# maxim2266/csvplus

Measured on AMD Instinct MI355X. Metric: joined rows/sec (IndexOn build + chained Join, 1e8-row 3-col orders), higher is better.
Workload: dtype u32; 1 GPU; BASELINE configs[3]: orders(1e8 x {cust_id,prod_id,qty}).Join(UniqueIndexOn customers.id 1e7).Join(UniqueIndexOn products.prod_id 1e5); rows=100000000, customers=10000000, products=100000, rows_this_rank=100000000, exchange=none (1 GPU), output=sorted positions

## Files before the change

### csvplus_amd/csrc/capi.hip

```cpp
#include <algorithm>
#include <map>
#include <mutex>
#include <new>

#include "cph_internal.hpp"
#include "codec_device.hpp"

namespace cph {

constexpr size_t kGuardBytes = 256;
constexpr uint8_t kGuardByte = 0xA5;

Status DevicePool::alloc(size_t bytes, void** out) {
    std::lock_guard<std::recursive_mutex> lk(mu_);
    const size_t want = (bytes + (guard ? kGuardBytes : 0) + 255) & ~(size_t)255;
    int best = -1;
    for (int i = 0; i < (int)free_.size(); i++) {
        if (free_[i].cap >= want && free_[i].cap <= want * 2 + (1u << 20)) {
            if (best < 0 || free_[i].cap < free_[best].cap) best = i;
        }
    }
    Block b;
    bool from_slab = false;
    for (size_t i = 0; i < slab_free_.size(); i++)
// ... 349 lines not shown
}

Status validate_cols(const cph_strcol* cols, int32_t ncols) {
    if (!cols || ncols <= 0) return {CPH_ERR_INVALID, "no key columns"};
    if (ncols > kMaxKeyCols) return {CPH_ERR_INVALID, "too many key columns"};
    for (int c = 0; c < ncols; c++) {
        if (cols[c].fixed_width == 0 && cols[c].offset_bits != 32 && cols[c].offset_bits != 64)
            return {CPH_ERR_INVALID, "offset_bits must be 32 or 64"};
        if (cols[c].mem != CPH_MEM_HOST && cols[c].mem != CPH_MEM_DEVICE) return {CPH_ERR_INVALID, "bad mem"};
        if (cols[c].nrows != cols[0].nrows) return {CPH_ERR_INVALID, "key columns differ in row count"};
        if (cols[c].nrows && !cols[c].offsets && cols[c].fixed_width == 0) return {CPH_ERR_INVALID, "offsets is NULL"};
        if (cols[c].nrows && cols[c].fixed_width && !cols[c].data) return {CPH_ERR_INVALID, "data is NULL"};
    }
    if (cols[0].nrows > 0xFFFFFFFFull) return {CPH_ERR_TOO_MANY_ROWS, "more than 2^32-1 rows"};
    return {};
}

Status stage_cols(cph_ctx* ctx, const cph_strcol* cols, int32_t ncols, std::vector<DevBuf>* storage,
                         DevCol* out) {
    for (int c = 0; c < ncols; c++) {
        DevCol d;
        d.nrows = cols[c].nrows;
        d.offset_bits = cols[c].offset_bits;
        d.fixed_width = cols[c].fixed_width;
        if (cols[c].mem == CPH_MEM_DEVICE || cols[c].nrows == 0) {
            d.data = cols[c].data;
            d.offsets = cols[c].offsets;
            if (!d.data) {
                if (!ctx->safe_words) {
                    CPH_TRY(ctx->safe_words.alloc(&ctx->pool, 64));
                    CPH_HIP_TRY(hipMemsetAsync(ctx->safe_words.get(), 0, 64, ctx->stream));
                }
                d.data = ctx->safe_words.as<uint8_t>();
            }
        } else if (cols[c].fixed_width) {
            const size_t bytes = (size_t)cols[c].nrows * cols[c].fixed_width;
            DevBuf bd;
            CPH_TRY(bd.alloc(&ctx->pool, bytes + 8));
            CPH_HIP_TRY(hipMemcpyAsync(bd.get(), cols[c].data, bytes, hipMemcpyHostToDevice, ctx->stream));
            d.data = bd.as<uint8_t>();
            d.offsets = nullptr;
            storage->push_back(std::move(bd));
        } else {
            const size_t obytes = (size_t)(cols[c].nrows + 1) * (size_t)(cols[c].offset_bits / 8);
            const uint64_t first = cols[c].offset_bits == 32 ? ((const uint32_t*)cols[c].offsets)[0]
                                                             : ((const uint64_t*)cols[c].offsets)[0];
            const uint64_t last = cols[c].offset_bits == 32 ? ((const uint32_t*)cols[c].offsets)[cols[c].nrows]
                                                            : ((const uint64_t*)cols[c].offsets)[cols[c].nrows];
            if (last < first) return {CPH_ERR_INVALID, "offsets are not monotonic"};
            DevBuf bo, bd;
            CPH_TRY(bo.alloc(&ctx->pool, obytes));
            CPH_TRY(bd.alloc(&ctx->pool, (size_t)last + 8));
            CPH_HIP_TRY(hipMemcpyAsync(bo.get(), cols[c].offsets, obytes, hipMemcpyHostToDevice, ctx->stream));
            if (last) CPH_HIP_TRY(hipMemcpyAsync(bd.get(), cols[c].data, (size_t)last, hipMemcpyHostToDevice, ctx->stream));
            d.data = bd.as<uint8_t>();
            d.offsets = bo.get();
            storage->push_back(std::move(bo));
            storage->push_back(std::move(bd));
        }
        out[c] = d;
    }
    return {};
}

Status check_row_sources(const cph_strcol* cols, const cph_rowsel* sel, int32_t ncols, uint64_t first_row, uint64_t nrows, bool exact) {
    for (int c = 0; c < ncols; c++) {
        CPH_TRY(validate_cols(cols + c, 1));
        const bool ident = !sel || !sel[c].ids;
        if (ident && nrows && (exact ? cols[c].nrows != nrows : cols[c].nrows < first_row + nrows))
            return {CPH_ERR_INVALID, exact ? "a column without row ids must have nrows rows"
                                           : "a column without row ids must have at least first_row + nrows rows"};
        if (!ident && sel[c].bits != 32 && sel[c].bits != 64) return {CPH_ERR_INVALID, "row id bits must be 32 or 64"};
    }
    return {};
}

Status stage_row_sources(cph_ctx* ctx, const cph_strcol* cols, const cph_rowsel* sel, const int* order, int32_t ncols, uint64_t first_row,
                         uint64_t n, std::vector<DevBuf>* staged, ColsArg* arg, ColIds* ids) {
    for (int k = 0; k < ncols; k++) {
        const int c = order ? order[k] : k;
        CPH_TRY(stage_cols(ctx, cols + c, 1, staged, &arg->c[k]));
        if (!sel || !sel[c].ids || !n) continue;
        RowIds& r = ids->ids[k];
        r.bits = sel[c].bits;
        r.base = sel[c].base;
        r.ptr = sel[c].ids;
        if (cols[c].mem == CPH_MEM_HOST) {
            const size_t w = (size_t)(sel[c].bits / 8);
            staged->emplace_back();
            CPH_TRY(staged->back().alloc(&ctx->pool, n * w));
            CPH_HIP_TRY(hipMemcpyAsync(staged->back().get(), static_cast<const uint8_t*>(sel[c].ids) + first_row * w, n * w,
                                       hipMemcpyHostToDevice, ctx->stream));
            r.ptr = reinterpret_cast<const void*>((uintptr_t)staged->back().get() - (uintptr_t)(first_row * w));
        }
    }
    return {};
}

Status deliver(cph_ctx* ctx, ResultOwner* owner, const ResultPart* parts, int nparts, int32_t out_mem) {
    auto show = [](const ResultPart& p, const void* v) { memcpy(p.pub, &v, sizeof v); };
    auto padded = [](const ResultPart& p) { return (p.bytes + 15) & ~(size_t)15; };
    uint8_t* h = nullptr;
    if (out_mem == CPH_MEM_HOST) {
        size_t need = 16;
        for (int i = 0; i < nparts; i++) need += padded(parts[i]);
        CPH_HIP_TRY(hipHostMalloc(&owner->h_block, need, hipHostMallocDefault));
        h = static_cast<uint8_t*>(owner->h_block);
    }
    for (int i = 0; i < nparts; i++) {
        const ResultPart& p = parts[i];
        const void* src = p.src ? p.src : p.dev->get();
        if (h && p.bytes) CPH_HIP_TRY(hipMemcpyAsync(h, src, p.bytes, hipMemcpyDeviceToHost, ctx->stream));
        show(p, h ? h : src);
        if (h) h += padded(p);
    }
    CPH_HIP_TRY(hipStreamSynchronize(ctx->stream));
    if (h)
        for (int i = 0; i < nparts; i++) parts[i].dev->reset();
    return {};
}

static int32_t fail(cph_ctx* ctx, const Status& s) {
    if (ctx) ctx->err = s.msg;
    return s.code;
}

static Status enter(cph_ctx* ctx) {
    if (!ctx) return {CPH_ERR_INVALID, "ctx is NULL"};
    CPH_HIP_TRY(hipSetDevice(ctx->device));
    return {};
}

struct BuildJob {
    cph_index* ix = nullptr;
    int32_t nkeycols = 0;
    std::vector<DevBuf> staged;
    DevCol dcols[kMaxKeyCols];
    DevBuf stats_dev;
    const void* sample_host = nullptr;
    size_t scratch_off = 0;
    GroupSpec spec;
    bool small = false;
    SmallBufs sbufs;
    bool presplit = false;
    bool sampled = false;
    bool no_sample = false;
    bool unique = false;
    bool no_direct = false;
    bool side = false;
    bool spec_split = false;
    bool exact_split = false;
    bool no_split = false;
    uint32_t* miss = nullptr;
    uint32_t* cs_over = nullptr;
    DevBuf cs_codes;
};

static Status build_phase1(cph_ctx* ctx, const cph_strcol* keycols, int32_t nkeycols, BuildJob* job) {
    CPH_TRY(validate_cols(keycols, nkeycols));
    cph_index* ix = job->ix;
    ix->ctx = ctx;
    ix->nrows = keycols[0].nrows;
    ix->table_rows = ix->nrows;
    ix->nkeycols = nkeycols;
    job->nkeycols = nkeycols;
    CPH_TRY(stage_cols(ctx, keycols, nkeycols, &job->staged, job->dcols));
    job->small = small_build_applies(ctx, job->dcols, nkeycols, ix->nrows);
    if (!job->small && !job->no_split && nkeycols == 1 && !job->dcols[0].fixed_width && ix->nrows >= (1ull << 22)) {
        CPH_TRY(codec_try_split(ctx, job->dcols, 1, ix->nrows, nullptr, &ix->codec, !job->exact_split, &job->spec_split));
        job->presplit = ix->codec.has_split();
    }
    job->sampled = !job->small && !job->presplit && !job->no_sample && codec_sample_applies(ctx, job->dcols, nkeycols, ix->nrows);
    if (job->sampled) CPH_TRY(codec_sample_launch(ctx, job->dcols[0], ix->nrows, &job->sample_host));
    else if (!job->small && !job->presplit) CPH_TRY(codec_stats_launch(ctx, job->dcols, nkeycols, &job->stats_dev));
    return {};
}

static Status build_phase2(cph_ctx* ctx, BuildJob* job, const void* stats_host);
static Status job_arm_miss(cph_ctx* ctx, BuildJob* job) {
    job->miss = host_word(ctx);
    return job->miss ? Status{} : Status{CPH_ERR_HIP, "no pinned host memory for the report words of a build"};
}
static Status build_encode_sort(cph_ctx* ctx, BuildJob* job);

static size_t job_readback_bytes(const BuildJob& j) {
    return j.small ? sizeof(SmallResult) : (j.presplit || j.sampled) ? 0 : sizeof(ColStats) * (size_t)j.nkeycols;
}

static void build_run(cph_ctx* ctx, std::vector<BuildJob>& jobs, std::vector<Status>& status) {
    const size_t nj = jobs.size();
    auto fail_all = [&](const Status& s) {
        for (size_t i = 0; i < nj; i++)
            if (status[i].ok()) status[i] = s;
    };
    size_t total = 0;
    bool any_general = false;
    for (size_t i = 0; i < nj; i++) {
        jobs[i].scratch_off = total;
        total += job_readback_bytes(jobs[i]);
        total = (total + 63) & ~(size_t)63;
        if (status[i].ok() && !jobs[i].small) any_general = true;
    }
    Status s = ensure_pinned_scratch(ctx, total > 64 ? total : 64);
    if (!s.ok()) return fail_all(s);
    uint8_t* h = static_cast<uint8_t*>(ctx->pinned_scratch);
    for (size_t i = 0; i < nj; i++) {
        if (!status[i].ok()) continue;
        if (jobs[i].small) {
            SideStream on_side(ctx, jobs[i].side);
            status[i] = small_build_launch(ctx, jobs[i].dcols, jobs[i].nkeycols, jobs[i].ix->nrows, &jobs[i].sbufs,
                                           reinterpret_cast<SmallResult*>(h + jobs[i].scratch_off));
            continue;
        }
        if (jobs[i].presplit || jobs[i].sampled) continue;
        hipError_t e = hipMemcpyAsync(h + jobs[i].scratch_off, jobs[i].stats_dev.get(), job_readback_bytes(jobs[i]),
                                      hipMemcpyDeviceToHost, jobs[i].side ? ctx->side_stream : ctx->stream);
        if (e != hipSuccess) status[i] = {CPH_ERR_HIP, std::string("statistics read-back: ") + hipGetErrorString(e)};
    }
    bool any_side = false;
    for (size_t i = 0; i < nj; i++) any_side = any_side || jobs[i].side;
    auto sync_streams = [&]() {
        return hipStreamSynchronize(ctx->stream) == hipSuccess && (!any_side || hipStreamSynchronize(ctx->side_stream) == hipSuccess);
    };
    if (!sync_streams()) return fail_all({CPH_ERR_HIP, "hipStreamSynchronize failed"});
    ctx->pool.flush_deferred();
    std::vector<std::vector<uint8_t>> stats_host(nj);
    std::vector<size_t> retry;
    for (size_t i = 0; i < nj; i++) {
        if (!status[i].ok()) continue;
        if (jobs[i].small) {
            const SmallResult res = *reinterpret_cast<const SmallResult*>(h + jobs[i].scratch_off);
            bool not_small = false;
            status[i] = small_build_finish(ctx, jobs[i].ix, jobs[i].nkeycols, &jobs[i].sbufs, &res, &not_small);
            jobs[i].sbufs = SmallBufs{};
            if (status[i].ok() && not_small) retry.push_back(i);
            else if (status[i].ok()) index_plan_table(jobs[i].ix);
            continue;
        }
        if (jobs[i].sampled) {
            const uint8_t* sh = static_cast<const uint8_t*>(jobs[i].sample_host);
            stats_host[i].assign(sh, sh + codec_sample_bytes());
        } else if (!jobs[i].presplit) {
            stats_host[i].assign(h + jobs[i].scratch_off, h + jobs[i].scratch_off + job_readback_bytes(jobs[i]));
        }
    }
    for (size_t i = 0; i < nj; i++)
        if (status[i].ok() && !jobs[i].small) {
            SideStream on_side(ctx, jobs[i].side);
            status[i] = build_phase2(ctx, &jobs[i], stats_host[i].data());
        }
    std::vector<size_t> resplit;
    std::vector<size_t> resort;
    if (any_general) {
        s = ensure_pinned_scratch(ctx, 2 * sizeof(uint32_t) * nj + 64);
        if (!s.ok()) return fail_all(s);
        uint32_t* fd = static_cast<uint32_t*>(ctx->pinned_scratch);
        uint32_t* sm = fd + nj;
        for (size_t i = 0; i < nj; i++) {
            if (!status[i].ok() || jobs[i].small) continue;
            hipStream_t js = jobs[i].side ? ctx->side_stream : ctx->stream;
            fd[i] = 0xFFFFFFFFu;
            sm[i] = 0;
            if (!jobs[i].ix->first_dup_dev) continue;
            hipError_t e = hipMemcpyAsync(&fd[i], jobs[i].ix->first_dup_dev.get(), sizeof(uint32_t), hipMemcpyDeviceToHost, js);
            if (e != hipSuccess) status[i] = {CPH_ERR_HIP, std::string("first-duplicate read-back: ") + hipGetErrorString(e)};
        }
        if (!sync_streams()) return fail_all({CPH_ERR_HIP, "hipStreamSynchronize failed"});
        ctx->pool.flush_deferred();
        for (size_t i = 0; i < nj; i++) {
            if (!status[i].ok() || jobs[i].small) continue;
            cph_index* ix = jobs[i].ix;
            if (jobs[i].miss) sm[i] = *(volatile uint32_t*)jobs[i].miss;
            if (sm[i]) { jobs[i].cs_codes.reset(); jobs[i].cs_over = nullptr; resplit.push_back(i); continue; }
            if (jobs[i].cs_over && *(volatile uint32_t*)jobs[i].cs_over) { resort.push_back(i); continue; }
            jobs[i].cs_codes.reset();
            ix->first_dup = fd[i] != 0xFFFFFFFFu ? (uint64_t)fd[i] : UINT64_MAX;
            ix->first_dup_dev.reset();
            index_plan_table(ix);
        }
    }
    for (size_t i : resort) {
        BuildJob& j = jobs[i];
        cph_index* ix = j.ix;
        const uint64_t n = ix->nrows;
        uint32_t* over = j.cs_over;
        j.cs_over = nullptr;
        ix->sorted_codes.reset(); ix->perm.reset(); ix->first_dup_dev.reset();
        DevBuf kb, va, vb;
        Status r = kb.alloc(&ctx->pool, n * sizeof(uint32_t));
        if (r.ok()) r = va.alloc(&ctx->pool, n * sizeof(uint32_t));
        bool sorted_now = false;
        {
            CountedSortPlan first;
            int wb = counted_sort_plan(ctx, n, ix->codec.word_states[0], &first) ? (int)first.wbits : 0;
            for (int attempt = 0; attempt < 2 && r.ok() && !sorted_now && wb > 0; attempt++) {
                wb -= 2;
                CountedSortPlan csp;
                if (!counted_sort_plan(ctx, n, ix->codec.word_states[0], &csp, wb) || (int)csp.wbits != wb) break;
                r = ix->first_dup_dev.alloc(&ctx->pool, sizeof(uint32_t));
                if (r.ok()) r = counted_sort(ctx, csp, j.cs_codes.as<uint32_t>(), n, ix->codec.word_states[0], va.as<uint32_t>(), kb.as<uint32_t>(),
                                             ix->first_dup_dev.as<uint32_t>(), over);
                if (r.ok() && hipStreamSynchronize(ctx->stream) != hipSuccess) r = {CPH_ERR_HIP, "hipStreamSynchronize failed"};
                if (r.ok() && *(volatile uint32_t*)over == 0) {
                    ix->sorted_codes = std::move(kb);
                    ix->perm = std::move(va);
                    ix->sort_passes = 0;
                    r = index_first_dup_read(ctx, ix);
                    sorted_now = true;
                } else {
                    ix->first_dup_dev.reset();
                }
            }
        }
        if (sorted_now) {
            j.cs_codes.reset();
            if (r.ok()) index_plan_table(ix);
            status[i] = r;
            continue;
        }
        if (r.ok()) r = vb.alloc(&ctx->pool, n * sizeof(uint32_t));
        uint32_t *kout = nullptr, *vout = nullptr;
        int passes = 0;
        if (r.ok()) r = radix_sort_pairs<uint32_t>(ctx, j.cs_codes.as<uint32_t>(), kb.as<uint32_t>(), va.as<uint32_t>(), vb.as<uint32_t>(), true, n,
                                                   ix->codec.word_bits[0], &kout, &vout, &passes);
        if (r.ok()) {
            ix->sorted_codes = std::move(kout == j.cs_codes.as<uint32_t>() ? j.cs_codes : kb);
            ix->perm = std::move(vout == va.as<uint32_t>() ? va : vb);
            ix->sort_passes = passes;
            r = index_first_dup_launch(ctx, ix);
        }
        if (r.ok()) r = index_first_dup_read(ctx, ix);
        j.cs_codes.reset();
        if (r.ok()) index_plan_table(ix);
        status[i] = r;
    }
    for (size_t i : resplit) {
        std::vector<BuildJob> one;
        one.push_back(std::move(jobs[i]));
        std::vector<Status> st1(1);
        BuildJob& j = one[0];
        j.side = false;
        const bool again_exact = j.spec_split;
        j.spec_split = false;
        j.exact_split = again_exact;
        j.no_split = !again_exact;
        j.no_sample = true;
        j.sampled = false;
        j.no_direct = true;
        j.presplit = false;
        j.miss = nullptr;
        cph_index* ix = j.ix;
        ix->codec = CodecHost{};
        ix->codec_dev.reset(); ix->sorted_codes.reset(); ix->perm.reset(); ix->first_dup_dev.reset(); ix->ranktab.reset();
        if (again_exact) {
            ctx->n_split_respec++;
            st1[0] = codec_try_split(ctx, j.dcols, 1, ix->nrows, nullptr, &ix->codec, false, nullptr);
            j.presplit = st1[0].ok() && ix->codec.has_split();
        }
        if (st1[0].ok() && !j.presplit) st1[0] = codec_stats_launch(ctx, j.dcols, j.nkeycols, &j.stats_dev);
        if (st1[0].ok()) build_run(ctx, one, st1);
        status[i] = st1[0];
        jobs[i] = std::move(one[0]);
    }
    for (size_t i : retry) {
        std::vector<BuildJob> one;
        one.push_back(std::move(jobs[i]));
        std::vector<Status> st1(1);
        one[0].small = false;
        one[0].side = false;
        st1[0] = codec_stats_launch(ctx, one[0].dcols, one[0].nkeycols, &one[0].stats_dev);
        if (st1[0].ok()) build_run(ctx, one, st1);
        status[i] = st1[0];
        jobs[i] = std::move(one[0]);
    }
}

static Status sort_words_lsd(cph_ctx* ctx, cph_index* ix, const uint64_t* all, int nw, const int* bits, uint64_t n, DevBuf& va,
                             DevBuf& vb) {
    DevBuf ka, kb;
    CPH_TRY(ka.alloc(&ctx->pool, n * sizeof(uint64_t)));
    CPH_TRY(kb.alloc(&ctx->pool, n * sizeof(uint64_t)));
    uint32_t* vcur = va.as<uint32_t>();
    uint32_t* vother = vb.as<uint32_t>();
    uint64_t* kout = ka.as<uint64_t>();
    bool first = true;
    int passes = 0;
    ix->sort_passes = 0;
    for (int w = nw - 1; w >= 0; w--) {
        const uint64_t* word = all + (uint64_t)w * n;
        if (first) {
            if (n) CPH_HIP_TRY(hipMemcpyAsync(ka.get(), word, n * sizeof(uint64_t), hipMemcpyDeviceToDevice, ctx->stream));
        } else {
            CPH_TRY(gather_u64(ctx, word, vcur, ka.as<uint64_t>(), n));
        }
        uint32_t* vout;
        CPH_TRY(radix_sort_pairs<uint64_t>(ctx, ka.as<uint64_t>(), kb.as<uint64_t>(), vcur, vother, first, n, bits[w], &kout, &vout,
                                           &passes));
        ix->sort_passes += passes;
        if (vout != vcur) { vother = vcur; vcur = vout; }
        first = false;
    }
    DevBuf sorted;
    CPH_TRY(sorted.alloc(&ctx->pool, (size_t)nw * n * sizeof(uint64_t)));
    if (n) CPH_HIP_TRY(hipMemcpyAsync(sorted.get(), kout, n * sizeof(uint64_t), hipMemcpyDeviceToDevice, ctx->stream));
    for (int w = 1; w < nw; w++) CPH_TRY(gather_u64(ctx, all + (uint64_t)w * n, vcur, sorted.as<uint64_t>() + (uint64_t)w * n, n));
    ix->sorted_codes = std::move(sorted);
    ix->perm = std::move(vcur == va.as<uint32_t>() ? va : vb);
    return {};
}

static DevCol window_col(const DevCol* cols, const cph_key_window& w, int s) {
    DevCol v = cols[w.seg_col[s]];
    v.skip = w.seg_skip[s];
    v.take = w.seg_take[s];
    return v;
}

static Status build_multi_window(cph_ctx* ctx, BuildJob* job, const std::vector<ColStats>& raw) {
    cph_index* ix = job->ix;
    const uint64_t n = ix->nrows;
    std::vector<cph_key_window>& W = ix->windows;
    W.clear();
    W.emplace_back();
    uint32_t room = kMaxKeyBytes;
    for (int c = 0; c < job->nkeycols; c++) {
        uint32_t left = raw[(size_t)c].maxlen, skip = 0;
        do {
            if (room == 0 || W.back().nseg == kMaxKeyCols) {
                W.emplace_back();
                room = kMaxKeyBytes;
            }
            cph_key_window& w = W.back();
            const uint32_t t = left < room ? left : room;
            w.seg_col[w.nseg] = c;
            w.seg_skip[w.nseg] = skip;
            w.seg_take[w.nseg] = t == left ? 0xFFFFFFFFu : t;
            w.nseg++;
            skip += t;
            left -= t;
            room -= t;
        } while (left > 0);
    }
    int total_words = 0;
    for (auto& w : W) {
        DevCol v[kMaxKeyCols];
        for (int s = 0; s < w.nseg; s++) v[s] = window_col(job->dcols, w, s);
        std::vector<ColStats> st;
        CPH_TRY(codec_collect_stats(ctx, v, w.nseg, &st));
        CPH_TRY(codec_build(st, &w.codec));
        w.codec.key32 = false;
        CPH_TRY(codec_upload(ctx, w.codec, &w.codec_dev));
        w.word_base = total_words;
        total_words += w.codec.nwords;
    }
    ix->codec = W[0].codec;
    DevBuf all, va, vb;
    CPH_TRY(all.alloc(&ctx->pool, (size_t)total_words * n * sizeof(uint64_t)));
    CPH_TRY(va.alloc(&ctx->pool, n * sizeof(uint32_t)));
    CPH_TRY(vb.alloc(&ctx->pool, n * sizeof(uint32_t)));
    std::vector<int> bits((size_t)total_words);
    for (auto& w : W) {
        DevCol v[kMaxKeyCols];
        for (int s = 0; s < w.nseg; s++) v[s] = window_col(job->dcols, w, s);
        CPH_TRY(codec_encode_build(ctx, w.codec, w.codec_dev, v, n, all.as<uint64_t>() + (uint64_t)w.word_base * n));
        for (int k = 0; k < w.codec.nwords; k++) bits[(size_t)(w.word_base + k)] = w.codec.word_bits[k];
    }
    CPH_TRY(sort_words_lsd(ctx, ix, all.as<uint64_t>(), total_words, bits.data(), n, va, vb));
    return index_first_dup_launch(ctx, ix);
}

static Status build_phase2(cph_ctx* ctx, BuildJob* job, const void* stats_host) {
    cph_index* ix = job->ix;
    const uint64_t n = ix->nrows;
    const int32_t nkeycols = job->nkeycols;
    const DevCol* dcols = job->dcols;
    if (job->presplit) {
        CPH_TRY(job_arm_miss(ctx, job));
        CPH_TRY(codec_upload(ctx, ix->codec, &ix->codec_dev));
        return build_encode_sort(ctx, job);
    }
    std::vector<ColStats> stats;
    if (job->sampled) {
        codec_sample_finish(dcols[0], stats_host, &stats);
        CPH_TRY(codec_build(stats, &ix->codec));
        if (codec_sample_checked(ix->codec, dcols)) {
            CPH_TRY(job_arm_miss(ctx, job));
            CPH_TRY(codec_upload(ctx, ix->codec, &ix->codec_dev));
            return build_encode_sort(ctx, job);
        }
        job->sampled = false;
        ix->codec = CodecHost{};
        CPH_TRY(codec_collect_stats(ctx, dcols, nkeycols, &stats));
    } else {
        codec_stats_finish(dcols, nkeycols, stats_host, &stats);
    }
    uint64_t positions = 0;
    for (const auto& s : stats) positions += s.maxlen;
    if (positions > (uint64_t)kMaxKeyBytes) return build_multi_window(ctx, job, stats);
    CPH_TRY(codec_build(stats, &ix->codec));
    if (!job->no_split) CPH_TRY(codec_try_split(ctx, dcols, nkeycols, n, &stats, &ix->codec));
    if (ix->codec.has_split()) {
        CPH_TRY(job_arm_miss(ctx, job));
    } else {
        CPH_TRY(codec_try_groups(ctx, dcols, nkeycols, n, &ix->codec, &job->spec));
    }
    CPH_TRY(codec_upload(ctx, ix->codec, &ix->codec_dev));
    return build_encode_sort(ctx, job);
}

static Status build_encode_sort(cph_ctx* ctx, BuildJob* job) {
    cph_index* ix = job->ix;
    const uint64_t n = ix->nrows;
    const DevCol* dcols = job->dcols;
    const CodecHost& cd = ix->codec;

    DevBuf va, vb;
    CPH_TRY(va.alloc(&ctx->pool, n * sizeof(uint32_t)));
    CPH_TRY(vb.alloc(&ctx->pool, n * sizeof(uint32_t)));
    int passes = 0;

    if (cd.nwords == 1) {
        const size_t kb_ = cd.key32 ? sizeof(uint32_t) : sizeof(uint64_t);
        DevBuf ka, kb, counts;
        CPH_TRY(ka.alloc(&ctx->pool, n * kb_));
        CPH_TRY(kb.alloc(&ctx->pool, n * kb_));
        const RadixPlan plan = radix_plan(ctx, n, cd.word_bits[0]);
        EncodeHist eh;
        const uint64_t states = cd.word_states[0];
        const bool direct = job->unique && !job->no_direct && ctx->direct_sort != 0 && cd.key32 && !job->spec.active && n >= (1ull << 16) &&
                            states >= n && states <= 2 * n && states < 0xFFFFFFFFull;
        if (direct) {
            if (!job->miss) {
                CPH_TRY(job_arm_miss(ctx, job));
            }
            if (states == n && ctx->direct_sort == 3) {
                CPH_HIP_TRY(hipMemsetAsync(va.get(), 0xFF, n * sizeof(uint32_t), ctx->stream));
                eh.slots = va.as<uint32_t>();
                eh.slot_states = (uint32_t)states;
            }
            DevBuf rt;
            uint64_t rt_blocks = 0;
            if (ctx->direct_ranktab && ctx->direct_sort == 1 && states != n && states <= (1ull << 30)) {
                rt_blocks = ranktab_blocks(states);
                if (!rt.alloc(&ctx->pool, rt_blocks * 8).ok()) rt_blocks = 0;
            }
            void* rtp = rt_blocks ? rt.get() : nullptr;
            ArithPlan ap;
            codec_arith_plan(cd, &ap);
            const DevCol& kc = dcols[0];
            if (ctx->direct_sort == 1 && ctx->direct_fused_encode && job->nkeycols == 1 && ap.enabled && ap.keylen == 8 && kc.fixed_width == 8 &&
                !kc.segmented() && ((uintptr_t)kc.data & 15) == 0) {
                CPH_TRY(direct_sort_windows_keys(ctx, reinterpret_cast<const uint64_t*>(kc.data), ap, n, states, va.as<uint32_t>(), ka.as<uint32_t>(),
                                                 job->miss, rtp, rt_blocks));
                ix->sorted_codes = std::move(ka);
                ix->perm = std::move(va);
                ix->sort_passes = 0;
                if (rtp) ix->ranktab = std::move(rt);
                return {};
            }
            CPH_TRY(codec_encode_build(ctx, cd, ix->codec_dev, dcols, n, ka.get(), &eh, nullptr, job->miss));
            if (eh.scattered) CPH_TRY(direct_sort_finish_full(ctx, va.as<uint32_t>(), n, ka.as<uint32_t>(), job->miss));
            else {
                bool rt_written = false;
                CPH_TRY(direct_sort_distinct(ctx, ka.as<uint32_t>(), n, states, va.as<uint32_t>(), ka.as<uint32_t>(), job->miss, rtp, rt_blocks, &rt_written));
                if (rt_written) ix->ranktab = std::move(rt);
            }
            ix->sorted_codes = std::move(ka);
            ix->perm = std::move(va);
            ix->sort_passes = 0;
            return {};
        }
        CountedSortPlan csp;
        if (cd.key32 && !job->spec.active && counted_sort_plan(ctx, n, states, &csp)) {
            uint32_t* over = host_word(ctx);
            if (!over) return {CPH_ERR_HIP, "no pinned host memory for the report words of a build"};
            vb.reset();
            CountedSort cs;
            CPH_TRY(cs.begin(ctx, csp, n));
            CPH_TRY(codec_encode_build(ctx, cd, ix->codec_dev, dcols, n, ka.get(), &eh, &job->spec, job->miss));
            CPH_TRY(ix->first_dup_dev.alloc(&ctx->pool, sizeof(uint32_t)));
            CPH_TRY(cs.run(ctx, ka.as<uint32_t>(), n, states, va.as<uint32_t>(), kb.as<uint32_t>(), ix->first_dup_dev.as<uint32_t>(), over, false));
            job->cs_over = over;
            job->cs_codes = std::move(ka);
            ix->sorted_codes = std::move(kb);
            ix->perm = std::move(va);
            ix->sort_passes = 0;
            return {};
        }
        if (plan.npass > 0) {
            CPH_TRY(counts.alloc(&ctx->pool, plan.count_words() * sizeof(uint32_t)));
            eh.tile_rows = plan.tile;
            eh.digit_mask = (1u << plan.nb0) - 1u;
            eh.bins = 1u << plan.rbits;
            eh.counts = counts.as<uint32_t>();
        }
        CPH_TRY(codec_encode_build(ctx, cd, ix->codec_dev, dcols, n, ka.get(), &eh, &job->spec, job->miss));
        if (job->spec.active) {
            uint32_t miss = 0;
            CPH_TRY(read_device_value(ctx, job->spec.miss.as<uint32_t>(), &miss));
            job->spec.active = false;
            if (miss) {
                const int bits_before = cd.word_bits[0];
                CPH_TRY(codec_groups_complete(ctx, dcols, job->nkeycols, n, miss, &job->spec, &ix->codec));
                CPH_TRY(codec_upload(ctx, ix->codec, &ix->codec_dev));
                if (cd.nwords != 1 || cd.word_bits[0] != bits_before || radix_plan(ctx, n, cd.word_bits[0]).npass != plan.npass) {
                    ka.reset(); kb.reset(); counts.reset(); va.reset(); vb.reset();
                    return build_encode_sort(ctx, job);
                }
                CPH_TRY(codec_encode_build(ctx, cd, ix->codec_dev, dcols, n, ka.get(), &eh, nullptr));
            }
        }
        uint32_t* vout;
        if (cd.key32) {
            uint32_t* kout;
            CPH_TRY(radix_sort_pairs<uint32_t>(ctx, ka.as<uint32_t>(), kb.as<uint32_t>(), va.as<uint32_t>(), vb.as<uint32_t>(),
                                               true, n, cd.word_bits[0], &kout, &vout, &passes, eh.counts, eh.done));
            ix->sorted_codes = std::move(kout == ka.as<uint32_t>() ? ka : kb);
        } else {
            uint64_t* kout;
            CPH_TRY(radix_sort_pairs<uint64_t>(ctx, ka.as<uint64_t>(), kb.as<uint64_t>(), va.as<uint32_t>(), vb.as<uint32_t>(),
                                               true, n, cd.word_bits[0], &kout, &vout, &passes, eh.counts, eh.done));
            ix->sorted_codes = std::move(kout == ka.as<uint64_t>() ? ka : kb);
        }
        ix->sort_passes = passes;
        ix->perm = std::move(vout == va.as<uint32_t>() ? va : vb);
    } else {
        DevBuf all;
        CPH_TRY(all.alloc(&ctx->pool, (size_t)cd.nwords * n * sizeof(uint64_t)));
        CPH_TRY(codec_encode_build(ctx, cd, ix->codec_dev, dcols, n, all.get(), nullptr, nullptr, job->miss));
        CPH_TRY(sort_words_lsd(ctx, ix, all.as<uint64_t>(), cd.nwords, cd.word_bits, n, va, vb));
    }

    CPH_TRY(index_first_dup_launch(ctx, ix));
    return {};
}

static Status index_build_impl(cph_ctx* ctx, const cph_strcol* keycols, int32_t nkeycols, cph_index* ix, bool unique) {
    if (nkeycols == 1 && keycols && keycols[0].mem == CPH_MEM_HOST && validate_cols(keycols, nkeycols).ok()) {
        bool taken = false;
        CPH_TRY(build_from_host_codes(ctx, keycols, nkeycols, ix, unique, &taken));
        if (taken) return {};
    }
    std::vector<BuildJob> jobs(1);
    std::vector<Status> st(1);
    jobs[0].ix = ix;
    jobs[0].unique = unique;
    st[0] = build_phase1(ctx, keycols, nkeycols, &jobs[0]);
    if (st[0].ok()) build_run(ctx, jobs, st);
    return st[0];
}

}

using namespace cph;

extern "C" {

CPH_API const char* cph_version(void) { return "csvplus_hip 0.1 (gfx950)"; }

CPH_API int32_t cph_ctx_create(int32_t device_id, cph_ctx** out) {
    if (!out) return CPH_ERR_INVALID;
    *out = nullptr;
    int count = 0;
    hipError_t e = hipGetDeviceCount(&count);
    if (e != hipSuccess || count <= 0) {
        (void)hipGetLastError();
        return CPH_ERR_NO_DEVICE;
    }
    if (device_id < 0 || device_id >= count) return CPH_ERR_NO_DEVICE;
    if (hipSetDevice(device_id) != hipSuccess) return CPH_ERR_NO_DEVICE;
    cph_ctx* ctx = new (std::nothrow) cph_ctx();
    if (!ctx) return CPH_ERR_NOMEM;
    ctx->device = device_id;
    if (hipStreamCreateWithFlags(&ctx->stream, hipStreamNonBlocking) != hipSuccess) {
        delete ctx;
        return CPH_ERR_HIP;
    }
    ctx->own_stream = true;
    warm_keycodec();
    warm_radix_sort();
    warm_probe();
    warm_chain();
    warm_materialize();
    warm_csv_ingest();
    warm_index_ops();
    warm_small_build();
    warm_window_sort();
    warm_counted_sort();
    (void)ensure_pinned_scratch(ctx, 1 << 16);
    void* ring = nullptr;
    (void)pinned_upload(ctx, 64, &ring);
    (void)host_word(ctx);
    *out = ctx;
    return CPH_OK;
}

CPH_API void cph_ctx_destroy(cph_ctx* ctx) {
    if (!ctx) return;
    (void)hipSetDevice(ctx->device);
    (void)hipStreamSynchronize(ctx->stream);
    if (ctx->pinned_scratch) (void)hipHostFree(ctx->pinned_scratch);
    if (ctx->upload_ring) (void)hipHostFree(ctx->upload_ring);
    if (ctx->host_words) (void)hipHostFree(ctx->host_words);
    for (void* p : ctx->pinned_user) (void)hipHostFree(p);
    for (auto& b : ctx->pinned_user_free) (void)hipHostFree(b.first);
    for (auto& b : ctx->pinned_cache) (void)hipHostFree(b.first);
    for (auto& p : ctx->prof_pending) { (void)hipEventDestroy(p.start); (void)hipEventDestroy(p.stop); }
    for (hipEvent_t e : ctx->prof_free_events) (void)hipEventDestroy(e);
    hipStream_t own = ctx->own_stream ? ctx->stream : nullptr;
    if (ctx->side_stream) {
        (void)hipStreamSynchronize(ctx->side_stream);
        (void)hipStreamDestroy(ctx->side_stream);
    }
    if (ctx->side_fork) (void)hipEventDestroy(ctx->side_fork);
    for (auto& sc : ctx->scan) sc.words.reset();
    for (auto& sc : ctx->self_clean) { sc.sum.reset(); sc.sample.reset(); sc.win.reset(); }
    host_pool_destroy(ctx);
    ctx->pool.trim();
    if (own) (void)hipStreamDestroy(own);
    delete ctx;
}

CPH_API int32_t cph_ctx_set_option(cph_ctx* ctx, const char* name, int64_t value) {
    if (!ctx || !name) return CPH_ERR_INVALID;
    const std::string k(name);
    if (k == "chain_debug") ctx->chain_debug = (int)value;
    else if (k == "sort_threads") ctx->sort_threads = (int)value;
    else if (k == "sort_rbits") ctx->sort_rbits = (int)value;
    else if (k == "sort_digit_stream") ctx->sort_digit_stream = value != 0;
    else if (k == "sort_xcd_tiles") ctx->sort_xcd_tiles = value != 0;
    else if (k == "codec_debug") ctx->codec_debug = (int)value;
    else if (k == "join_hash") ctx->join_hash = value != 0;
    else if (k == "stream_role_streams") ctx->stream_role_streams = value != 0;
    else if (k == "stream_zero_copy_out") ctx->stream_zero_copy_out = value != 0;
    else if (k == "chain_nt_streams") ctx->chain_nt_streams = value < 0 || value > 2 ? 0 : (int)value;
    else if (k == "chain_rank_lds") ctx->chain_rank_lds = value != 0;
    else if (k == "chain_rows4") ctx->chain_rows4 = value < 0 || value > 2 ? 1 : (int)value;
    else if (k == "codec_split") ctx->codec_split = value != 0;
    else if (k == "split_speculative") ctx->split_speculative = value != 0;
    else if (k == "scan_lookback") ctx->scan_lookback = value != 0;
    else if (k == "build_side_stream") ctx->build_side_stream = value != 0;
    else if (k == "stats_sample") ctx->stats_sample = value != 0;
    else if (k == "host_build") ctx->host_build = value != 0;
    else if (k == "host_threads") { ctx->host_threads = value < 0 || value > 256 ? 0 : (int)value; host_pool_destroy(ctx); }
    else if (k == "host_split") ctx->host_split = value < 0 || value > 2 ? 1 : (int)value;
    else if (k == "host_numa") ctx->host_numa = value != 0;
    else if (k == "sample_lean") ctx->sample_lean = value != 0;
    else if (k == "hash_partitioned") ctx->hash_partitioned = value < 0 || value > 2 ? 1 : (int)value;
    else if (k == "host_split_threads") { ctx->host_split_threads = value < 0 || value > 256 ? 0 : (int)value; host_pool_destroy(ctx); }
    else if (k == "counted_sort") ctx->counted_sort = value != 0;
    else if (k == "csv_fast") ctx->csv_fast = value != 0;
    else if (k == "csv_onepass_debug") ctx->csv_onepass_debug = (int)value;
    else if (k == "csv_onepass") ctx->csv_onepass = value < 0 ? 0 : value > (1 << 20) ? (1 << 20) : (int)value;
    else if (k == "direct_sort") ctx->direct_sort = value < 0 || value > 4 ? 1 : (int)value;
    else if (k == "chain_arith") ctx->chain_arith = value != 0;
    else if (k == "chain_identity") ctx->chain_identity = value != 0;
    else if (k == "chain_prejoin") ctx->chain_prejoin = value != 0;
    else if (k == "direct_fused_encode") ctx->direct_fused_encode = value != 0;
    else if (k == "direct_ranktab") ctx->direct_ranktab = value != 0;
    else if (k == "hash_load_pct") ctx->hash_load_pct = value < 25 ? 25 : value > 90 ? 90 : (int)value;
    else if (k == "probe_hash_rows") ctx->probe_hash_rows = value == 4 ? 4 : 2;
    else if (k == "small_build_rows") ctx->small_build_rows = value < 0 ? 0 : value > (1 << 20) ? (1 << 20) : (int)value;
    else if (k == "plan_threads") ctx->plan_threads = (int)value;
    else if (k == "gstats_threads") ctx->gstats_threads = (int)value;
    else if (k == "speculative_groups") ctx->speculative_groups = value < 0 || value > 2 ? 1 : (int)value;
    else if (k == "pool_guard") ctx->pool.guard = value != 0;
    else if (k == "pool_reserve_mb") {
        if (value <= 0) return fail_with(ctx, {CPH_ERR_INVALID, "pool_reserve_mb must be positive"});
        if (hipSetDevice(ctx->device) != hipSuccess) return fail_with(ctx, {CPH_ERR_HIP, "hipSetDevice failed"});
        Status rs = ctx->pool.reserve((size_t)value << 20);
        if (!rs.ok()) return fail_with(ctx, rs);
    }
    else if (k == "pool_guard_check") {
        ctx->pool.check_live();
        if (ctx->pool.guard_violations) {
            char b[64];
            snprintf(b, sizeof b, " (%llu blocks)", (unsigned long long)ctx->pool.guard_violations);
            return fail_with(ctx, {CPH_ERR_INVALID, ctx->pool.first_violation + b});
        }
    }
    else return fail_with(ctx, {CPH_ERR_INVALID, "unknown option: " + k});
    return CPH_OK;
}

CPH_API const char* cph_last_error(const cph_ctx* ctx) { return ctx ? ctx->err.c_str() : "ctx is NULL"; }

CPH_API int32_t cph_ctx_set_stream(cph_ctx* ctx, void* hip_stream) {
    Status s = enter(ctx);
    if (!s.ok()) return fail(ctx, s);
    (void)hipStreamSynchronize(ctx->stream);
    if (ctx->side_stream) (void)hipStreamSynchronize(ctx->side_stream);
    for (auto& sc : ctx->scan) { sc.words.reset(); sc.tiles = 0; sc.tickets = 0; sc.epoch = 0; }
    if (hip_stream) {
        if (ctx->own_stream) (void)hipStreamDestroy(ctx->stream);
        ctx->stream = reinterpret_cast<hipStream_t>(hip_stream);
        ctx->own_stream = false;
    } else if (!ctx->own_stream) {
        if (hipStreamCreateWithFlags(&ctx->stream, hipStreamNonBlocking) != hipSuccess)
            return fail(ctx, {CPH_ERR_HIP, "hipStreamCreate failed"});
        ctx->own_stream = true;
    }
    return CPH_OK;
}

CPH_API int32_t cph_ctx_synchronize(cph_ctx* ctx) {
    Status s = enter(ctx);
    if (!s.ok()) return fail(ctx, s);
    hipError_t e = hipStreamSynchronize(ctx->stream);
    if (e != hipSuccess) return fail(ctx, {CPH_ERR_HIP, std::string("hipStreamSynchronize: ") + hipGetErrorString(e)});
    return CPH_OK;
}

CPH_API int32_t cph_ctx_profile(cph_ctx* ctx, int32_t enable) {
    Status s = enter(ctx);
    if (!s.ok()) return fail(ctx, s);
    ctx->profiling = enable != 0;
    ctx->prof_only.clear();
    return CPH_OK;
}

CPH_API int32_t cph_ctx_profile_only(cph_ctx* ctx, const char* kernel_name) {
    Status s = enter(ctx);
    if (!s.ok()) return fail(ctx, s);
    ctx->profiling = kernel_name != nullptr;
    ctx->prof_only = kernel_name ? kernel_name : "";
    return CPH_OK;
}

CPH_API int32_t cph_ctx_profile_read(cph_ctx* ctx, cph_kernel_stat* out, int32_t cap, int32_t* n, int32_t reset) {
    Status s = enter(ctx);
    if (!s.ok()) return fail(ctx, s);
    if (!n || (cap > 0 && !out)) return fail(ctx, {CPH_ERR_INVALID, "bad argument"});
    hipError_t e = hipStreamSynchronize(ctx->stream);
    if (e != hipSuccess) return fail(ctx, {CPH_ERR_HIP, std::string("hipStreamSynchronize: ") + hipGetErrorString(e)});
    for (auto& p : ctx->prof_pending) {
        float ms = 0;
        if (hipEventElapsedTime(&ms, p.start, p.stop) == hipSuccess) {
            ProfStat& st = ctx->prof_stats[(size_t)p.name_idx];
            st.launches++;
            st.total_ms += ms;
            st.bytes += p.bytes;
        } else {
            (void)hipGetLastError();
        }
        ctx->prof_free_events.push_back(p.start);
        ctx->prof_free_events.push_back(p.stop);
    }
    ctx->prof_pending.clear();
    const int32_t total = (int32_t)ctx->prof_stats.size();
    *n = total;
    for (int32_t i = 0; i < total && i < cap; i++) {
        const ProfStat& st = ctx->prof_stats[(size_t)i];
        memset(&out[i], 0, sizeof out[i]);
        snprintf(out[i].name, sizeof out[i].name, "%s", st.name.c_str());
        out[i].launches = st.launches;
        out[i].total_ms = st.total_ms;
        out[i].algo_bytes = st.bytes;
    }
    if (reset) ctx->prof_stats.clear();
    return CPH_OK;
}

CPH_API int32_t cph_pinned_alloc(cph_ctx* ctx, size_t bytes, void** out) {
    Status s = enter(ctx);
    if (!s.ok()) return fail(ctx, s);
    if (!out) return fail(ctx, {CPH_ERR_INVALID, "out is NULL"});
    void* p = nullptr;
    constexpr size_t kRecycleMax = 4u << 20;
    size_t cap = bytes ? bytes : 1;
    if (cap <= kRecycleMax) {
        size_t c2 = 4096;
        while (c2 < cap) c2 <<= 1;
        cap = c2;
        for (size_t i = 0; i < ctx->pinned_user_free.size(); i++)
            if (ctx->pinned_user_free[i].second == cap) {
                p = ctx->pinned_user_free[i].first;
                ctx->pinned_user_free.erase(ctx->pinned_user_free.begin() + (long)i);
                break;
            }
    }
    if (!p) {
        hipError_t e = hipHostMalloc(&p, cap, hipHostMallocDefault);
        if (e != hipSuccess) {
            (void)hipGetLastError();
            for (auto& b : ctx->pinned_user_free) (void)hipHostFree(b.first);
            ctx->pinned_user_free.clear();
            e = hipHostMalloc(&p, cap, hipHostMallocDefault);
        }
        if (e != hipSuccess) return fail(ctx, {CPH_ERR_NOMEM, std::string("hipHostMalloc: ") + hipGetErrorString(e)});
    }
    ctx->pinned_user.push_back(p);
    if (cap <= kRecycleMax) ctx->pinned_user_cap.push_back({p, cap});
    *out = p;
    return CPH_OK;
}

CPH_API int32_t cph_pinned_free(cph_ctx* ctx, void* p) {
    Status s = enter(ctx);
    if (!s.ok()) return fail(ctx, s);
    auto it = std::find(ctx->pinned_user.begin(), ctx->pinned_user.end(), p);
    if (it == ctx->pinned_user.end()) return fail(ctx, {CPH_ERR_INVALID, "not a cph_pinned_alloc block"});
    ctx->pinned_user.erase(it);
    for (size_t i = 0; i < ctx->pinned_user_cap.size(); i++)
        if (ctx->pinned_user_cap[i].first == p) {
            const size_t cap = ctx->pinned_user_cap[i].second;
            ctx->pinned_user_cap.erase(ctx->pinned_user_cap.begin() + (long)i);
            if (ctx->pinned_user_free.size() < 32) {
                ctx->pinned_user_free.push_back({p, cap});
                return CPH_OK;
            }
            break;
        }
    (void)hipHostFree(p);
    return CPH_OK;
}

CPH_API int32_t cph_index_build(cph_ctx* ctx, const cph_strcol* keycols, int32_t nkeycols, int32_t unique,
                                cph_index** out, uint64_t* first_dup_pos) {
    Status s = enter(ctx);
    if (!s.ok()) return fail(ctx, s);
    if (!out) return fail(ctx, {CPH_ERR_INVALID, "out is NULL"});
    *out = nullptr;
    if (first_dup_pos) *first_dup_pos = UINT64_MAX;
    cph_index* ix = new (std::nothrow) cph_index();
    if (!ix) return fail(ctx, {CPH_ERR_NOMEM, "out of host memory"});
    s = index_build_impl(ctx, keycols, nkeycols, ix, unique != 0);
    if (!s.ok()) {
        delete ix;
        return fail(ctx, s);
    }
    if (first_dup_pos) *first_dup_pos = ix->first_dup;
    *out = ix;
    if (unique && ix->first_dup != UINT64_MAX) {
        char b[128];
        snprintf(b, sizeof b, "duplicate value while creating unique index (sorted position %llu)",
                 (unsigned long long)ix->first_dup);
        return fail(ctx, {CPH_ERR_DUPLICATE, b});
    }
    return CPH_OK;
}

CPH_API int32_t cph_index_build_many(cph_ctx* ctx, const cph_index_spec* specs, int32_t nspecs, cph_index** out,
                                     uint64_t* first_dup_pos, int32_t* status) {
    Status s = enter(ctx);
    if (!s.ok()) return fail(ctx, s);
    if (!specs || !out || nspecs < 1 || nspecs > 64) return fail(ctx, {CPH_ERR_INVALID, "bad cph_index_build_many arguments"});
    std::vector<BuildJob> jobs((size_t)nspecs);
    std::vector<Status> st((size_t)nspecs);
    if (!host_words_reserve(ctx, (uint32_t)nspecs * (uint32_t)(codec_sample_bytes() / 4 + 16)))
        return fail(ctx, {CPH_ERR_INVALID, "cph_index_build_many: the batch needs more report words than the ctx holds"});
    bool two_streams = nspecs >= 2 && ctx->build_side_stream != 0;
    if (two_streams && !ctx->side_stream && hipStreamCreateWithFlags(&ctx->side_stream, hipStreamNonBlocking) != hipSuccess) {
        (void)hipGetLastError();
        ctx->side_stream = nullptr;
        two_streams = false;
    }
    struct DeferGuard {
        cph_ctx* c;
        ~DeferGuard() {
            if (!c) return;
            (void)hipStreamSynchronize(c->stream);
            (void)hipStreamSynchronize(c->side_stream);
            c->pool.end_defer();
        }
    } defer{two_streams ? ctx : nullptr};
    if (two_streams) {
        hipError_t fe = ctx->side_fork ? hipSuccess : hipEventCreateWithFlags(&ctx->side_fork, hipEventDisableTiming);
        if (fe == hipSuccess) fe = hipEventRecord(ctx->side_fork, ctx->stream);
        if (fe == hipSuccess) fe = hipStreamWaitEvent(ctx->side_stream, ctx->side_fork, 0);
        if (fe != hipSuccess) {
            (void)hipGetLastError();
            two_streams = false;
            defer.c = nullptr;
        }
    }
    if (two_streams) ctx->pool.begin_defer();
    for (int i = 0; i < nspecs; i++) {
        out[i] = nullptr;
        if (first_dup_pos) first_dup_pos[i] = UINT64_MAX;
        jobs[i].ix = new (std::nothrow) cph_index();
        jobs[i].side = two_streams && (i & 1);
        jobs[i].unique = specs[i].unique != 0;
        SideStream on_side(ctx, jobs[i].side);
        if (!jobs[i].ix) st[i] = {CPH_ERR_NOMEM, "out of host memory"};
        else st[i] = build_phase1(ctx, specs[i].keycols, specs[i].nkeycols, &jobs[i]);
    }
    build_run(ctx, jobs, st);
    int32_t rc = CPH_OK;
    std::string msg;
    for (int i = 0; i < nspecs; i++) {
        cph_index* ix = jobs[i].ix;
        if (st[i].ok() && specs[i].unique && ix->first_dup != UINT64_MAX) {
            char b[160];
            snprintf(b, sizeof b, "index %d: duplicate value while creating unique index (sorted position %llu)", i,
                     (unsigned long long)ix->first_dup);
            st[i] = {CPH_ERR_DUPLICATE, b};
        }
        const bool keep = st[i].ok() || st[i].code == CPH_ERR_DUPLICATE;
        if (keep) {
            out[i] = ix;
            if (first_dup_pos) first_dup_pos[i] = ix->first_dup;
        } else {
            delete ix;
        }
        if (status) status[i] = st[i].code;
        if (!st[i].ok() && rc == CPH_OK) { rc = st[i].code; msg = st[i].msg; }
    }
    if (rc != CPH_OK) return fail(ctx, {rc, msg});
    return CPH_OK;
}

CPH_API void cph_index_destroy(cph_index* ix) {
    if (!ix) return;
    if (ix->ctx) (void)hipSetDevice(ix->ctx->device);
    if (ix->perm_host) {
        if (ix->ctx) pinned_cache_put(ix->ctx, ix->perm_host, ix->perm_host_cap);
        else (void)hipHostFree(ix->perm_host);
    }
    delete ix;
}

CPH_API uint64_t cph_index_nrows(const cph_index* ix) { return ix ? ix->nrows : 0; }
CPH_API int32_t cph_index_nkeycols(const cph_index* ix) { return ix ? ix->nkeycols : 0; }

CPH_API int32_t cph_index_perm(cph_index* ix, int32_t mem, const uint32_t** perm, uint64_t* n) {
    if (!ix || !perm) return CPH_ERR_INVALID;
    cph_ctx* ctx = ix->ctx;
    Status s = enter(ctx);
    if (!s.ok()) return fail(ctx, s);
    if (n) *n = ix->nrows;
    if (mem == CPH_MEM_DEVICE) {
        *perm = ix->perm.as<uint32_t>();
        return CPH_OK;
    }
    if (!ix->perm_host) {
        const size_t bytes = (size_t)ix->nrows * sizeof(uint32_t);
        void* p = nullptr;
        size_t cap = 0;
        s = pinned_cache_get(ctx, bytes, &p, &cap);
        if (!s.ok()) return fail(ctx, s);
        if (bytes) {
            hipError_t e = hipMemcpyAsync(p, ix->perm.get(), bytes, hipMemcpyDeviceToHost, ctx->stream);
            if (e == hipSuccess) e = hipStreamSynchronize(ctx->stream);
            if (e != hipSuccess) {
                (void)hipHostFree(p);
                return fail(ctx, {CPH_ERR_HIP, std::string("perm read-back: ") + hipGetErrorString(e)});
            }
        }
        ix->perm_host = static_cast<uint32_t*>(p);
        ix->perm_host_cap = cap;
    }
    *perm = ix->perm_host;
    return CPH_OK;
}

CPH_API int32_t cph_join_probe(cph_ctx* ctx, const cph_index* ix, const cph_strcol* probecols, int32_t nprobecols,
                               const void* row_sel, int32_t sel_bits, uint64_t sel_base, uint64_t nsel,
                               uint64_t probe_base, int32_t want_pairs, int32_t out_mem, cph_matches** out) {
    Status s = enter(ctx);
    if (!s.ok()) return fail(ctx, s);
    if (!ix || !out) return fail(ctx, {CPH_ERR_INVALID, "index/out is NULL"});
    *out = nullptr;
    if (nprobecols > ix->nkeycols) return fail(ctx, {CPH_ERR_TOO_MANY_COLS, "too many source columns in Join()"});
    s = validate_cols(probecols, nprobecols);
    if (!s.ok()) return fail(ctx, s);
    if (out_mem != CPH_MEM_HOST && out_mem != CPH_MEM_DEVICE) return fail(ctx, {CPH_ERR_INVALID, "bad out_mem"});
    if (row_sel && sel_bits != 32 && sel_bits != 64) return fail(ctx, {CPH_ERR_INVALID, "sel_bits must be 32 or 64"});
    if (row_sel && nsel > 0xFFFFFFFFull) return fail(ctx, {CPH_ERR_TOO_MANY_ROWS, "more than 2^32-1 selected rows"});

    cph_matches_impl* m = new (std::nothrow) cph_matches_impl();
    if (!m) return fail(ctx, {CPH_ERR_NOMEM, "out of host memory"});
    m->ctx = ctx;
    auto run = [&]() -> Status {
        std::vector<DevBuf> staged;
        DevCol dcols[kMaxKeyCols];
        CPH_TRY(stage_cols(ctx, probecols, nprobecols, &staged, dcols));
        RowSel dsel;
        dsel.ptr = row_sel;
        dsel.bits = sel_bits;
        dsel.base = sel_base;
        DevBuf selbuf;
        const bool cols_on_host = probecols[0].mem == CPH_MEM_HOST;
        if (row_sel && cols_on_host && nsel) {
            const size_t sb = nsel * (size_t)(sel_bits / 8);
            CPH_TRY(selbuf.alloc(&ctx->pool, sb));
            CPH_HIP_TRY(hipMemcpyAsync(selbuf.get(), row_sel, sb, hipMemcpyHostToDevice, ctx->stream));
            dsel.ptr = selbuf.get();
        }
        const uint64_t nprobe = row_sel ? nsel : probecols[0].nrows;
        ProbeOut po;
        CPH_TRY(probe_run(ctx, ix, dcols, nprobecols, dsel, nprobe, probe_base, want_pairs != 0, &po));
        m->pub.nprobe = nprobe;
        m->pub.nmatches = po.nmatches;
        m->pub.mem = out_mem;
        const bool pairs = want_pairs && po.nmatches;
        if (out_mem == CPH_MEM_DEVICE) {
            m->d_lo = std::move(po.lo);
            m->d_cnt = std::move(po.cnt);
            m->d_pidx = std::move(po.pidx);
            m->d_brow = std::move(po.brow);
            m->pub.lo = m->d_lo.as<uint32_t>();
            m->pub.cnt = m->d_cnt.as<uint32_t>();
            m->pub.probe_idx = pairs ? m->d_pidx.as<uint64_t>() : nullptr;
            m->pub.build_row = pairs ? m->d_brow.as<uint32_t>() : nullptr;
            CPH_HIP_TRY(hipStreamSynchronize(ctx->stream));
        } else {
            auto a16 = [](size_t x) { return (x + 15) & ~(size_t)15; };
            const size_t b_lo = a16(nprobe * sizeof(uint32_t));
            const size_t b_pi = pairs ? a16(po.nmatches * sizeof(uint64_t)) : 0;
            const size_t b_br = pairs ? a16(po.nmatches * sizeof(uint32_t)) : 0;
            const size_t total = 2 * b_lo + b_pi + b_br + 16;
            CPH_TRY(pinned_cache_get(ctx, result_block_bytes(total), &m->h_block, &m->h_cap));
            uint8_t* h = static_cast<uint8_t*>(m->h_block);
            uint8_t* h_pidx = h;
            uint8_t* h_lo = h + b_pi;
            uint8_t* h_cnt = h_lo + b_lo;
            uint8_t* h_brow = h_cnt + b_lo;
            if (nprobe) {
                CPH_HIP_TRY(hipMemcpyAsync(h_lo, po.lo.get(), nprobe * sizeof(uint32_t), hipMemcpyDeviceToHost, ctx->stream));
                CPH_HIP_TRY(hipMemcpyAsync(h_cnt, po.cnt.get(), nprobe * sizeof(uint32_t), hipMemcpyDeviceToHost, ctx->stream));
            }
            if (pairs) {
                CPH_HIP_TRY(hipMemcpyAsync(h_pidx, po.pidx.get(), po.nmatches * sizeof(uint64_t), hipMemcpyDeviceToHost, ctx->stream));
                CPH_HIP_TRY(hipMemcpyAsync(h_brow, po.brow.get(), po.nmatches * sizeof(uint32_t), hipMemcpyDeviceToHost, ctx->stream));
            }
            CPH_HIP_TRY(hipStreamSynchronize(ctx->stream));
            m->pub.lo = reinterpret_cast<const uint32_t*>(h_lo);
            m->pub.cnt = reinterpret_cast<const uint32_t*>(h_cnt);
            m->pub.probe_idx = pairs ? reinterpret_cast<const uint64_t*>(h_pidx) : nullptr;
            m->pub.build_row = pairs ? reinterpret_cast<const uint32_t*>(h_brow) : nullptr;
        }
        return {};
    };
    s = run();
    if (!s.ok()) {
        (void)hipStreamSynchronize(ctx->stream);
        if (m->h_block) pinned_cache_put(ctx, m->h_block, m->h_cap);
        delete m;
// ... 270 lines not shown
```

### csvplus_amd/csrc/codec_device.hpp

```cpp
#pragma once

#include "cph_internal.hpp"
#include "device_utils.hpp"

namespace cph {

__device__ __forceinline__ uint64_t find_first_byte(const uint8_t* data, uint64_t begin, uint64_t len, uint32_t d) {
    const uint64_t dv = 0x0101010101010101ull * (uint64_t)(d & 0xFFu);
    for (uint64_t j = 0; 8 * j < len; j++) {
        const uint64_t x = load_value_chunk(data, begin, len, (int)j) ^ dv;
        const uint64_t t = (x - 0x0101010101010101ull) & ~x & 0x8080808080808080ull;
        if (t) {
            const uint64_t pos = 8 * j + (uint64_t)((__ffsll((long long)t) - 1) >> 3);
            return pos < len ? pos : len;
        }
    }
    return len;
}

__device__ __forceinline__ void value_span_whole(const DevCol& col, uint64_t row, uint64_t* begin, uint64_t* len);
__device__ __forceinline__ void value_span(const DevCol& col, uint64_t row, uint64_t* begin, uint64_t* len) {
    value_span_whole(col, row, begin, len);
    if (col.split) {
        const uint64_t b = *begin, l = *len;
// ... 218 lines not shown
        uint32_t b[R], e[R];
#pragma unroll
        for (int k = 0; k < R; k++) {
            b[k] = NT ? __builtin_nontemporal_load(&off[wr.rel[k]]) : off[wr.rel[k]];
            e[k] = NT ? __builtin_nontemporal_load(&off[wr.rel[k] + 1]) : off[wr.rel[k] + 1];
        }
#pragma unroll
        for (int k = 0; k < R; k++) {
            sp->x[k] = b[k];
            sp->len[k] = e[k] - b[k];
        }
    } else if constexpr (sizeof(B) == 8) {
        const uint64_t* off = reinterpret_cast<const uint64_t*>(c.offsets) + wr.rbase;
        uint64_t b[R], e[R];
#pragma unroll
        for (int k = 0; k < R; k++) {
            b[k] = off[wr.rel[k]];
            e[k] = off[wr.rel[k] + 1];
        }
#pragma unroll
        for (int k = 0; k < R; k++) {
            sp->x[k] = b[k];
            const uint64_t l = e[k] - b[k];
            sp->len[k] = l > 0xFFFFFFFFull ? 0xFFFFFFFFu : (uint32_t)l;
        }
    } else {
#pragma unroll
        for (int k = 0; k < R; k++) { sp->x[k] = 0; sp->len[k] = 0; }
    }
}
template <int R, class B>
__device__ __forceinline__ void gather_spans(const DevCol& c, const uint32_t (&row)[R], WaveSpans<R, B>* sp) {
    const uint64_t p = (uint64_t)(uintptr_t)c.data;
    sp->base8 = (const uint8_t*)(uintptr_t)(p & ~7ull);
    sp->delta = (uint32_t)(p & 7ull);
    if (c.fixed_width) {
#pragma unroll
        for (int k = 0; k < R; k++) {
            sp->x[k] = (B)row[k] * (B)c.fixed_width;
            sp->len[k] = c.fixed_width;
        }
        return;
    }
    if (c.offset_bits == 32) {
        const uint32_t* off = reinterpret_cast<const uint32_t*>(c.offsets);
        uint32_t b[R], e[R];
#pragma unroll
        for (int k = 0; k < R; k++) {
            b[k] = off[row[k]];
            e[k] = off[(uint64_t)row[k] + 1];
        }
#pragma unroll
        for (int k = 0; k < R; k++) {
            sp->x[k] = b[k];
            sp->len[k] = e[k] - b[k];
        }
    } else if constexpr (sizeof(B) == 8) {
        const uint64_t* off = reinterpret_cast<const uint64_t*>(c.offsets);
        uint64_t b[R], e[R];
#pragma unroll
        for (int k = 0; k < R; k++) {
            b[k] = off[row[k]];
            e[k] = off[(uint64_t)row[k] + 1];
        }
#pragma unroll
        for (int k = 0; k < R; k++) {
            sp->x[k] = b[k];
            const uint64_t l = e[k] - b[k];
            sp->len[k] = l > 0xFFFFFFFFull ? 0xFFFFFFFFu : (uint32_t)l;
        }
    } else {
#pragma unroll
        for (int k = 0; k < R; k++) { sp->x[k] = 0; sp->len[k] = 0; }
    }
}
inline bool col_is_narrow(const DevCol& c) { return c.fixed_width ? c.fixed_width <= 0xFFFFu : c.offset_bits == 32; }

template <int R, class W, class B, bool FIXED>
__device__ __forceinline__ void encode_position(const CPH_LDS W* lp, int b, uint32_t pos, const WaveSpans<R, B>& sp, const uint64_t (&cur)[R],
                                                W (&acc)[R], W (&bad)[R]) {
#pragma unroll
    for (int k = 0; k < R; k++) {
        const uint32_t half = b < 4 ? (uint32_t)cur[k] : (uint32_t)(cur[k] >> 32);
        const uint32_t byte = (half >> (8 * (b & 3))) & 0xFFu;
        const uint32_t sym = FIXED ? byte + 1u : (pos < sp.len[k] ? byte + 1u : 0u);
        const W v = lp[b * kLutStride + sym];
        if constexpr (sizeof(W) == 4) {
            acc[k] = __builtin_elementwise_add_sat(acc[k], v);
        } else {
            bad[k] |= v;
            acc[k] += v;
        }
    }
}

template <int R, class W, class B, class CW, bool LONG>
__device__ __forceinline__ void encode_rows(const CodecView& cv, const WaveSpans<R, B>& sp, const uint64_t (&c0)[R],
                                            const uint64_t (&c1)[R], CW (&code)[R], uint32_t* okmask, bool fixed = false) {
    const int maxlen = cv.hdr->col_maxlen[0];
    const CPH_LDS W* lutw = (const CPH_LDS W*)cv.lutw;
    W acc[R], bad[R];
#pragma unroll
    for (int k = 0; k < R; k++) { acc[k] = 0; bad[k] = 0; }
    const int nchunks = (maxlen + 7) >> 3;
#pragma unroll 1
    for (int j = 0; j < nchunks; j++) {
        uint64_t cur[R];
        if (j == 0) {
#pragma unroll
            for (int k = 0; k < R; k++) cur[k] = c0[k];
        } else if (LONG && j == 1) {
#pragma unroll
            for (int k = 0; k < R; k++) cur[k] = c1[k];
        } else {
#pragma unroll
            for (int k = 0; k < R; k++) cur[k] = sp.chunk(k, (uint32_t)j);
        }
        const int qn = maxlen - 8 * j < 8 ? maxlen - 8 * j : 8;
        const CPH_LDS W* lp = lutw + (8 * j) * kLutStride;
        if (fixed) {
#pragma unroll
            for (int b = 0; b < 8; b++)
                if (b < qn) encode_position<R, W, B, true>(lp, b, (uint32_t)(8 * j + b), sp, cur, acc, bad);
        } else {
#pragma unroll
            for (int b = 0; b < 8; b++)
                if (b < qn) encode_position<R, W, B, false>(lp, b, (uint32_t)(8 * j + b), sp, cur, acc, bad);
        }
    }
    uint32_t m = *okmask;
#pragma unroll
    for (int k = 0; k < R; k++) {
        code[k] = (CW)acc[k];
        const W flag = sizeof(W) == 4 ? acc[k] : bad[k];
        const bool good = sp.len[k] <= (uint32_t)maxlen && !(flag >> (sizeof(W) * 8 - 1));
        if (!good) m &= ~(1u << k);
    }
    *okmask = m;
}

struct ArithPlan {
    uint32_t enabled;
    uint32_t mul24;
    uint32_t keylen;
    uint32_t keep[2];
    uint32_t lo[2];
    uint32_t rngc[2];
    uint32_t wa[2], wb[2];
    uint32_t ma[2];
    uint32_t s1;
};

void codec_arith_plan(const CodecHost& codec, ArithPlan* ap);

template <int R, class CW>
__device__ __forceinline__ void encode_rows_arith(const ArithPlan& ap, const uint64_t (&c0)[R], CW (&code)[R], uint32_t* okmask) {
    uint32_t m = *okmask;
    uint32_t zl[R], zh[R];
#pragma unroll
    for (int k = 0; k < R; k++) {
        const uint32_t xl = (uint32_t)c0[k], xh = (uint32_t)(c0[k] >> 32);
        zl[k] = xl - ap.lo[0];
        zh[k] = xh - ap.lo[1];
        const uint32_t tl = zl[k] + ap.rngc[0], th = zh[k] + ap.rngc[1];
        const uint32_t bad = ((xl | zl[k] | tl) | (xh | zh[k] | th)) & 0x80808080u;
        if (bad) m &= ~(1u << k);
    }
    if (ap.mul24) {
#pragma unroll
        for (int k = 0; k < R; k++) {
            const uint32_t pa0 = __builtin_amdgcn_udot4(zl[k], ap.wa[0], 0u, false);
            const uint32_t pa1 = __builtin_amdgcn_udot4(zh[k], ap.wa[1], 0u, false);
            const uint32_t w0 = __builtin_amdgcn_udot4(zl[k], ap.wb[0], __umul24(pa0, ap.ma[0]), false);
            code[k] = (CW)__builtin_amdgcn_udot4(zh[k], ap.wb[1], __umul24(pa1, ap.ma[1]) + __umul24(w0, ap.s1), false);
        }
    } else {
#pragma unroll
        for (int k = 0; k < R; k++) {
            const uint32_t pa0 = __builtin_amdgcn_udot4(zl[k], ap.wa[0], 0u, false);
            const uint32_t pa1 = __builtin_amdgcn_udot4(zh[k], ap.wa[1], 0u, false);
            const uint32_t w0 = __builtin_amdgcn_udot4(zl[k], ap.wb[0], pa0 * ap.ma[0], false);
            code[k] = (CW)__builtin_amdgcn_udot4(zh[k], ap.wb[1], pa1 * ap.ma[1] + w0 * ap.s1, false);
        }
    }
    *okmask = m;
}

template <bool LONGV = true>
struct ValueHeadT {
    uint64_t begin = 0, len = 0, c0 = 0, c1 = 0, c2 = 0;
    __device__ __forceinline__ void span(const DevCol& col, uint64_t row) { value_span(col, row, &begin, &len); }
    __device__ __forceinline__ void chunks(const DevCol& col) {
        c0 = len > 0 ? load_value_chunk(col.data, begin, len, 0) : 0;
        c1 = len > 8 ? load_value_chunk(col.data, begin, len, 1) : 0;
        c2 = len > 16 ? load_value_chunk(col.data, begin, len, 2) : 0;
    }
    __device__ __forceinline__ void chunks_nobranch(const DevCol& col) {
        const uint64_t p = (uint64_t)(uintptr_t)col.data;
        const uint8_t* base8 = (const uint8_t*)(uintptr_t)(p & ~7ull);
        const uint32_t delta = (uint32_t)(p & 7ull);
        const uint32_t l32 = len > 0xFFFFFFFFull ? 0xFFFFFFFFu : (uint32_t)len;
        const uint64_t a = load_chunk_nobranch<uint64_t>(base8, delta, begin, l32, 0);
        const uint64_t b = load_chunk_nobranch<uint64_t>(base8, delta, begin, l32, 1);
        const uint64_t c = load_chunk_nobranch<uint64_t>(base8, delta, begin, l32, 2);
        c0 = l32 > 0 ? a : 0;
        c1 = l32 > 8 ? b : 0;
        c2 = l32 > 16 ? c : 0;
    }
    __device__ __forceinline__ void load(const DevCol& col, uint64_t row) {
        span(col, row);
        chunks(col);
    }
    __device__ __forceinline__ uint64_t chunk(const DevCol& col, int j) const {
        if constexpr (LONGV) {
            if (8ull * (uint64_t)j >= len) return 0;
            return j == 0 ? c0 : j == 1 ? c1 : j == 2 ? c2 : load_value_chunk(col.data, begin, len, j);
        } else {
            return j == 0 ? c0 : j == 1 ? c1 : j == 2 ? c2 : 0;
        }
    }
    __device__ __forceinline__ uint32_t sym(const DevCol& col, int q) const {
        const uint32_t b = ((uint32_t)(chunk(col, q >> 3) >> (8 * (q & 7))) & 0xFFu) + 1u;
        return (uint64_t)q < len ? b : 0u;
    }
    __device__ __forceinline__ uint64_t window(const DevCol& col, int q) const {
        const int sh = (q & 7) * 8;
        const uint64_t lo = chunk(col, q >> 3);
        if (sh == 0) return lo;
        return (lo >> sh) | (chunk(col, (q >> 3) + 1) << (64 - sh));
    }
    __device__ __forceinline__ uint64_t raw(const DevCol& col, int q, int span) const {
        const uint64_t nvalid = len > (uint64_t)q ? (len - (uint64_t)q < (uint64_t)span ? len - (uint64_t)q : (uint64_t)span) : 0;
        return group_raw(window(col, q), nvalid);
    }
    template <int J>
    __device__ __forceinline__ uint64_t ck() const {
        if constexpr (J == 0) return c0;
        else if constexpr (J == 1) return c1;
        else if constexpr (J == 2) return c2;
        else return 0;
    }
    template <int J>
    __device__ __forceinline__ uint32_t sym_j(int q) const {
        const uint32_t b = ((uint32_t)(ck<J>() >> (8 * (q & 7))) & 0xFFu) + 1u;
        return (uint64_t)q < len ? b : 0u;
    }
    template <int J>
    __device__ __forceinline__ uint64_t window_j(int q) const {
        const int sh = (q & 7) * 8;
        return sh == 0 ? ck<J>() : (ck<J>() >> sh) | (ck<J + 1>() << (64 - sh));
    }
    template <int J>
    __device__ __forceinline__ uint64_t raw_j(int q, int span) const {
        const uint32_t l32 = len > 0xFFFFFFFFull ? 0xFFFFFFFFu : (uint32_t)len;
        const uint32_t left = l32 > (uint32_t)q ? l32 - (uint32_t)q : 0u;
        return group_raw(window_j<J>(q), (uint64_t)(left < (uint32_t)span ? left : (uint32_t)span));
    }
};
using ValueHead = ValueHeadT<true>;

template <class Emit>
__device__ __forceinline__ bool encode_key_groups(const CodecView& cv, const ColsArg& cols, int ncols_used, uint64_t row,
                                                  Emit&& emit) {
    const int p_end = cv.hdr->col_start[ncols_used];
    uint64_t acc = 0;
    bool valid = true;
    for (int c = 0; c < ncols_used; c++) {
        const DevCol& col = cols.c[c];
        uint64_t begin, len;
        value_span(col, row, &begin, &len);
        const int maxlen = cv.hdr->col_maxlen[c];
        const int p0 = cv.hdr->col_start[c];
        if (len > (uint64_t)maxlen) valid = false;
        ValueHead v;
        v.begin = begin;
        v.len = len;
        v.chunks(col);
        for (int q = 0; q < maxlen; q++) {
            const int p = p0 + q;
            const uint32_t kind = cv.unit[p];
            uint64_t r = 0;
            if (kind == kUnitWide) {
                int rank = -1;
                if (len <= (uint64_t)kWideBytes) {
                    uint64_t w[4];
                    wide_words(col.data, begin, len, w);
                    rank = wide_lookup(cv, w[0], w[1], w[2], w[3], (uint32_t)len);
                }
                if (rank < 0) valid = false;
                r = rank < 0 ? 0ull : (uint64_t)rank;
            } else if (kind == kUnitHead) {
                int span = 1;
                while (span < kGroupSpan && q + span < maxlen && cv.unit[p + span] == kUnitAbsorbed) span++;
                const uint64_t joint = v.raw(col, q, span);
                const CPH_LDS uint64_t* d = cv.dict + cv.dict_off[p];
                const CPH_LDS uint16_t* ht = cv.hash + cv.hash_off[p];
                const int bits = cv.hash_bits[p];
                const uint32_t mask = (1u << bits) - 1u;
                uint32_t sl = bits ? group_slot(joint, bits) : 0u;
                bool found = false;
                for (;;) {
                    const uint32_t e = ht[sl];
                    if (e == 0) break;
                    if (d[e - 1] == joint) { r = (uint64_t)(e - 1); found = true; break; }
                    sl = (sl + 1) & mask;
                }
// ... 56 lines not shown
```

### csvplus_amd/csrc/cph_internal.hpp

```cpp
#pragma once

#include <hip/hip_runtime.h>

#include <cstdint>
#include <cstdio>
#include <cstring>
#include <mutex>
#include <string>
#include <utility>
#include <vector>

#include "../../include/csvplus_hip.h"

namespace cph {

constexpr int kMaxKeyBytes = 128;
constexpr int kMaxKeyCols  = CPH_MAX_KEY_COLS;
constexpr int kLutStride   = 257;
constexpr uint16_t kLutInvalid = 0xFFFF;
constexpr int kMaxWords    = 20;

struct Status {
    int32_t code = CPH_OK;
    std::string msg;
// ... 102 lines not shown
CPH_HD2 inline uint32_t wide_rotl(uint32_t v, int r) { return (v << r) | (v >> (32 - r)); }
CPH_HD2 inline void wide_fold(uint64_t w0, uint64_t w1, uint64_t w2, uint64_t w3, uint32_t len, uint32_t* x, uint32_t* y) {
    *x = (uint32_t)w0 ^ wide_rotl((uint32_t)w1, 9) ^ wide_rotl((uint32_t)w2, 18) ^ wide_rotl((uint32_t)w3, 27) ^ (len * 0x01000193u);
    *y = (uint32_t)(w0 >> 32) ^ wide_rotl((uint32_t)(w1 >> 32), 7) ^ wide_rotl((uint32_t)(w2 >> 32), 14) ^ wide_rotl((uint32_t)(w3 >> 32), 21);
}
CPH_HD2 inline uint32_t wide_hash_lo(uint64_t w0, uint64_t w1, uint64_t w2, uint64_t w3, uint32_t len) {
    uint32_t x, y;
    wide_fold(w0, w1, w2, w3, len, &x, &y);
    uint32_t h1 = (x * 0x9E3779B1u) ^ (y * 0x85EBCA6Bu);
    h1 ^= h1 >> 15;
    return h1;
}
CPH_HD2 inline uint64_t wide_hash(uint64_t w0, uint64_t w1, uint64_t w2, uint64_t w3, uint32_t len) {
    uint32_t x, y;
    wide_fold(w0, w1, w2, w3, len, &x, &y);
    const uint32_t h1 = wide_hash_lo(w0, w1, w2, w3, len);
    uint32_t h2 = (x * 0xCC9E2D51u + wide_rotl(y, 13)) * 0x1B873593u;
    h2 ^= h2 >> 16;
    h2 *= 0xC2B2AE35u;
    h2 ^= h2 >> 13;
    const uint64_t h = (uint64_t)h1 | ((uint64_t)h2 << 32);
    return h ? h : 1ull;
}

struct CodecHost {
    int32_t ncols = 0;
    int32_t npos = 0;
    int32_t nwords = 1;
    bool    key32 = false;
    int32_t col_start[kMaxKeyCols + 1] = {0};
    int32_t col_maxlen[kMaxKeyCols] = {0};
    int32_t col_minlen[kMaxKeyCols] = {0};
    int32_t word_bits[kMaxWords] = {0};
    uint64_t word_states[kMaxWords] = {0};
    std::vector<uint16_t> radix;
    std::vector<uint64_t> mult;
    std::vector<int32_t>  word_of;
    std::vector<uint16_t> lut;
    std::vector<uint8_t>  unit;
    std::vector<int32_t>  dict_off;
    std::vector<int32_t>  dict_len;
    std::vector<uint64_t> dict;
    bool has_groups() const { return !unit.empty(); }
    int32_t split_col = -1;
    uint8_t split_byte = 0;
    bool spec_checked = false;
    int32_t split_maxlen = 0;
    std::vector<WideKey> wdict;
    std::vector<uint16_t> wide_disp, wide_slots;
    bool has_split() const { return split_col >= 0; }
    int32_t virtual_cols(int32_t real_cols) const { return real_cols + (has_split() && split_col < real_cols ? 1 : 0); }
};
constexpr int kGroupSpan = 7;
constexpr int kGroupDictMax = 4096;
enum : uint8_t { kUnitPos = 0, kUnitHead = 1, kUnitAbsorbed = 2, kUnitWide = 3 };

struct CodecDevHeader {
    int32_t ncols;
    int32_t npos;
    int32_t nwords;
    int32_t key32;
    int32_t col_start[kMaxKeyCols + 1];
    int32_t col_maxlen[kMaxKeyCols];
    int32_t mult_off;
    int32_t wordof_off;
    int32_t lut_off;
    int32_t total_bytes;
    int32_t lutw_off;
    int32_t lutw_bits;
    int32_t ngroups;
    int32_t unit_off;
    int32_t dictoff_off;
    int32_t dictlen_off;
    int32_t dict_off;
    int32_t hashoff_off;
    int32_t hashbits_off;
    int32_t hash_off;
    int32_t wide_pos;
    int32_t wide_n;
    int32_t wide_off;
    int32_t wide_hash_off;
    int32_t wide_hash_bits;
    int32_t split_vcol;
    int32_t split_byte;
    int32_t wide_disp_off;
    int32_t wide_disp_bits;
    int32_t pad_[3];
};
#if defined(__HIPCC__)
#define CPH_HD __host__ __device__
#else
#define CPH_HD
#endif
CPH_HD inline uint32_t group_slot(uint64_t raw, int bits) { return (uint32_t)((raw * 0x9E3779B97F4A7C15ull) >> (64 - bits)); }
CPH_HD inline uint64_t group_raw(uint64_t window, uint64_t nvalid) {
    return (window & ((1ull << (8 * nvalid)) - 1ull)) | (nvalid << 56);
}
CPH_HD inline uint64_t group_order_key(uint64_t raw, int span) {
    const int nvalid = (int)(raw >> 56);
    uint64_t k = 0;
    for (int i = 0; i < span && i < nvalid; i++) k |= (((raw >> (8 * i)) & 0xFFull) + 1ull) << (9 * (kGroupSpan - 1 - i));
    return k;
}

}

namespace cph {
struct ProfPending { int name_idx; hipEvent_t start, stop; double bytes; };
struct ProfStat { std::string name; uint64_t launches = 0; double total_ms = 0, bytes = 0; };
}

struct cph_ctx {
    int device = 0;
    hipStream_t stream = nullptr;
    bool own_stream = false;
    std::string err;
    cph::DevicePool pool;
    void* pinned_scratch = nullptr;
    size_t pinned_scratch_bytes = 0;
    void* upload_ring = nullptr;
    size_t upload_cap = 0, upload_pos = 0;
    std::vector<void*> pinned_user;
    std::vector<std::pair<void*, size_t>> pinned_user_free;
    std::vector<std::pair<void*, size_t>> pinned_user_cap;
    std::vector<std::pair<void*, size_t>> pinned_cache;
    uint32_t* host_words = nullptr;
    uint32_t host_words_pos = 0;
    struct SelfClean {
        cph::DevBuf sum;
        cph::DevBuf sample;
        cph::DevBuf win;
        uint64_t win_words = 0;
    } self_clean[2];
    cph::DevBuf safe_words;
    int cus = 0;
    int chain_debug = 0;
    int sort_threads = 0, sort_rbits = 0;
    int sort_digit_stream = 1;
    int sort_xcd_tiles = 1;
    int small_build_rows = 8192;
    int stream_role_streams = 0;
    int stream_zero_copy_out = 0;
    int chain_nt_streams = 0;
    int chain_arith = 1;
    int chain_identity = 1;
    int chain_rows4 = 1;
    int chain_rank_lds = 1;
    int probe_hash_rows = 2;
    int join_hash = 1;
    int codec_debug = 0;
    uint64_t n_split_respec = 0;
    int hash_load_pct = 50;
    int direct_fused_encode = 1;
    int direct_ranktab = 1;
    int chain_prejoin = 1;
    int split_speculative = 1;
    int codec_split = 1;
    int scan_lookback = 1;
    struct ScanState {
        cph::DevBuf words;
        uint64_t tiles = 0, epoch = 0;
        uint32_t tickets = 0;
    } scan[2];
    int csv_fast = 1;
    int csv_onepass = 1;
    int csv_onepass_debug = 0;
    int sample_lean = 1;
    int hash_partitioned = 1;
    int counted_sort = 1;
    int direct_sort = 1;
    int stats_sample = 1;
    int host_build = 1;
    int host_threads = 0;
    void* host_pool = nullptr;
    int host_split = 1;
    int host_split_threads = 0;
    void* host_pool_wide = nullptr;
    int host_numa = 0;
    int build_side_stream = 1;
    hipStream_t side_stream = nullptr;
    hipEvent_t side_fork = nullptr;
    int stream_slot = 0;
    hipStream_t swapped_main = nullptr;
    hipStream_t other_stream() const { return stream_slot ? swapped_main : side_stream; }
    int plan_threads = 0, gstats_threads = 0;
    int speculative_groups = 1;
    struct KernelCfg { const void* fn; size_t lds; int blocks_per_cu; };
    std::vector<KernelCfg> kernel_cfg;
    bool profiling = false;
    std::string prof_only;
    std::vector<cph::ProfPending> prof_pending;
    std::vector<cph::ProfStat> prof_stats;
    std::vector<hipEvent_t> prof_free_events;
};

namespace cph {
constexpr uint32_t kHostWords = 65536;
uint32_t* host_word(cph_ctx* ctx, uint32_t n = 1);
bool host_words_reserve(cph_ctx* ctx, uint32_t n);
Status self_clean_block(cph_ctx* ctx, cph::DevBuf* b, size_t bytes);
struct SideStream {
    cph_ctx* ctx;
    hipStream_t saved;
    SideStream(cph_ctx* c, bool on) : ctx(on ? c : nullptr), saved(c->stream) {
        if (ctx) {
            ctx->swapped_main = saved;
            ctx->stream = ctx->side_stream;
            ctx->stream_slot = 1;
        }
    }
    ~SideStream() {
        if (ctx) {
            ctx->stream = saved;
            ctx->stream_slot = 0;
            ctx->swapped_main = nullptr;
        }
    }
    SideStream(const SideStream&) = delete;
    SideStream& operator=(const SideStream&) = delete;
};
}

struct cph_key_window {
    cph::CodecHost codec;
    cph::DevBuf codec_dev;
    int32_t nseg = 0;
    int32_t seg_col[CPH_MAX_KEY_COLS] = {0};
    uint32_t seg_skip[CPH_MAX_KEY_COLS] = {0}, seg_take[CPH_MAX_KEY_COLS] = {0};
    int32_t word_base = 0;
};

struct cph_index {
    cph_ctx* ctx = nullptr;
    uint64_t nrows = 0;
    uint64_t table_rows = 0;
    int32_t nkeycols = 0;
    cph::CodecHost codec;
    cph::DevBuf codec_dev;
    std::vector<cph_key_window> windows;
    int32_t total_words() const {
        if (windows.empty()) return codec.nwords;
        int32_t t = 0;
        for (const auto& w : windows) t += w.codec.nwords;
        return t;
    }
    cph::DevBuf sorted_codes;
    cph::DevBuf perm;
    cph::DevBuf table;
    cph::DevBuf rowtab;
    cph::DevBuf ranktab;
    uint64_t table_entries = 0;
    cph::DevBuf hash;
    uint32_t hash_sectors = 0;
    uint32_t hash_slice_mask = 0;
    int32_t hash_mode = 0;
    bool accel_failed = false;
    std::mutex accel_mu;
    hipEvent_t accel_ready = nullptr;
    ~cph_index() {
        if (accel_ready) (void)hipEventDestroy(accel_ready);
    }
    int32_t sort_passes = 0;
    bool small_built = false;
    bool host_coded = false;
    uint64_t first_dup = UINT64_MAX;
    uint32_t* perm_host = nullptr;
    size_t perm_host_cap = 0;
    cph::DevBuf first_dup_dev;
};

struct cph_chain_impl {
    cph_chain pub;
    cph_ctx* ctx = nullptr;
    cph::DevBuf d_stream;
    cph::DevBuf d_rows[CPH_MAX_CHAIN];
    void* h_block = nullptr;
    size_t h_cap = 0;
};

struct cph_matches_impl {
    cph_matches pub;
    cph_ctx* ctx = nullptr;
    cph::DevBuf d_lo, d_cnt, d_pidx, d_brow;
    void* h_block = nullptr;
    size_t h_cap = 0;
};

namespace cph {

struct DevCol {
    const uint8_t* data = nullptr;
    const void* offsets = nullptr;
    uint64_t nrows = 0;
    int32_t offset_bits = 32;
    uint32_t fixed_width = 0;
    uint32_t skip = 0, take = 0xFFFFFFFFu;
    bool segmented() const { return skip != 0 || take != 0xFFFFFFFFu; }
    uint16_t split = 0;
    uint16_t part = 0;
};
struct ColsArg {
    DevCol c[kMaxKeyCols];
};
struct RowIds {
    const void* ptr = nullptr;
    int32_t bits = 32;
    uint64_t base = 0;
    uint64_t* stash = nullptr;
};
struct ColIds {
    RowIds ids[kMaxKeyCols];
};
int codec_virtual_cols(const CodecHost& codec, const DevCol* real, int nreal, DevCol* out);
bool codec_wide_perfect_hash(CodecHost* codec);

struct ColStats {
    uint32_t minlen, maxlen;
    uint32_t mask[kMaxKeyBytes][8];
};
Status codec_collect_stats(cph_ctx* ctx, const DevCol* cols, int32_t ncols, std::vector<ColStats>* out);
Status codec_stats_launch(cph_ctx* ctx, const DevCol* cols, int32_t ncols, DevBuf* dev_stats);
void codec_stats_finish(const DevCol* cols, int32_t ncols, const void* host_copy, std::vector<ColStats>* out);
Status codec_build(const std::vector<ColStats>& stats, CodecHost* codec);
bool codec_sample_applies(const cph_ctx* ctx, const DevCol* cols, int32_t ncols, uint64_t n);
size_t codec_sample_bytes();
Status codec_sample_launch(cph_ctx* ctx, const DevCol& col, uint64_t n, const void** host_copy);
void codec_sample_finish(const DevCol& col, const void* host_copy, std::vector<ColStats>* out);
bool codec_sample_checked(const CodecHost& codec, const DevCol* cols);
struct GroupChoice { int t, p0, span; double saved; uint32_t count; uint32_t tab; };
struct GroupSpec {
    bool active = false;
    DevBuf slots, counts, miss;
    std::vector<GroupChoice> chosen;
    CodecHost plain;
};
Status codec_try_groups(cph_ctx* ctx, const DevCol* cols, int32_t ncols, uint64_t n, CodecHost* codec, GroupSpec* spec = nullptr);
constexpr uint32_t kSpecGiveUp = 1u << 16;
Status codec_groups_complete(cph_ctx* ctx, const DevCol* cols, int32_t ncols, uint64_t n, uint32_t missed, GroupSpec* spec, CodecHost* codec);
Status codec_upload(cph_ctx* ctx, const CodecHost& codec, DevBuf* dev);
int codec_premultiplied_bits(const CodecHost& codec);
struct EncodeHist {
    uint32_t tile_rows = 0;
    uint32_t digit_mask = 0;
    uint32_t bins = 0;
    uint32_t* counts = nullptr;
    bool done = false;
    uint32_t* slots = nullptr;
    uint32_t slot_states = 0;
    bool scattered = false;
};
Status codec_encode_build(cph_ctx* ctx, const CodecHost& codec, const DevBuf& codec_dev, const DevCol* cols,
                          uint64_t n, void* out_codes, const EncodeHist* hist = nullptr, const GroupSpec* spec = nullptr,
                          uint32_t* miss = nullptr);
Status codec_try_split(cph_ctx* ctx, const DevCol* cols, int32_t ncols, uint64_t n, const std::vector<ColStats>* stats, CodecHost* codec,
                       bool speculate = false, bool* speculated = nullptr);
Status codec_split_from_host(cph_ctx* ctx, const cph_host::HostCol& hc, uint64_t n, cph_host::BlockPool& pool, CodecHost* codec);
bool codec_encode_values_host(const CodecHost& codec, const cph_strval* values, int32_t nvalues,
                              uint64_t* q_exact, int32_t* nq, uint64_t* qlo, uint64_t* qhi);

struct RadixPlan {
    int npass = 0, threads = 256, rbits = 8;
    uint32_t tile = 4096, ntiles = 0;
    int nb0 = 0;
    size_t count_words() const { return ((size_t)1 << rbits) * ntiles; }
};
RadixPlan radix_plan(const cph_ctx* ctx, uint64_t n, int bits);
template <class K>
Status radix_sort_pairs(cph_ctx* ctx, K* keys_a, K* keys_b, uint32_t* vals_a, uint32_t* vals_b, bool vals_iota,
                        uint64_t n, int bits, K** keys_out, uint32_t** vals_out, int* passes,
                        uint32_t* counts = nullptr, bool first_hist_done = false);
struct CountedSortPlan {
    uint32_t wbits = 0, k2 = 0, nb1 = 0, nwt = 0;
    bool two = false;
};
bool counted_sort_plan(const cph_ctx* ctx, uint64_t n, uint64_t states, CountedSortPlan* p, int max_wbits = 31, uint64_t min_rows = 1ull << 21);
struct CountedSort {
    CountedSortPlan p;
    DevBuf words, ent1, ent2;
    uint32_t* counts = nullptr;
    Status begin(cph_ctx* ctx, const CountedSortPlan& plan, uint64_t n);
    Status partition(cph_ctx* ctx, const uint32_t* codes, uint64_t n, uint64_t states, uint32_t* over_host, bool hist_done);
    const uint64_t* entries() const { return p.two ? ent2.as<uint64_t>() : ent1.as<uint64_t>(); }
    const uint32_t* flag() const { return counts + p.nwt; }
    const uint32_t* wbase() const { return counts + p.nwt + 1; }
    Status run(cph_ctx* ctx, const uint32_t* codes, uint64_t n, uint64_t states, uint32_t* perm_out, uint32_t* sorted_out, uint32_t* first_dup_dev,
               uint32_t* over_host, bool hist_done);
};
Status counted_sort(cph_ctx* ctx, const CountedSortPlan& p, const uint32_t* codes, uint64_t n, uint64_t states, uint32_t* perm_out,
                    uint32_t* sorted_out, uint32_t* first_dup_dev, uint32_t* over_host);
void warm_counted_sort();
Status direct_sort_distinct(cph_ctx* ctx, const uint32_t* codes, uint64_t n, uint64_t states, uint32_t* perm_out, uint32_t* sorted_out,
                            uint32_t* flag, void* ranktab = nullptr, uint64_t rank_blocks = 0, bool* ranktab_written = nullptr);
struct ArithPlan;
Status direct_sort_windows_keys(cph_ctx* ctx, const uint64_t* keys, const ArithPlan& ap, uint64_t n, uint64_t states, uint32_t* perm_out,
                                uint32_t* sorted_out, uint32_t* flag, void* ranktab = nullptr, uint64_t rank_blocks = 0);
Status direct_sort_windows(cph_ctx* ctx, const uint32_t* codes, uint64_t n, uint64_t states, uint32_t* perm_out, uint32_t* sorted_out,
                           uint32_t* flag, void* ranktab = nullptr, uint64_t rank_blocks = 0);
struct WindowSort {
    Status begin(cph_ctx* ctx, uint64_t n, uint64_t states);
    Status add(cph_ctx* ctx, const uint32_t* codes, uint64_t row0, uint64_t m, uint32_t* flag, const uint64_t* keys = nullptr, const ArithPlan* ap = nullptr);
    Status finish(cph_ctx* ctx, uint32_t* perm_out, uint32_t* sorted_out, uint32_t* flag, void* ranktab = nullptr, uint64_t rank_blocks = 0);
    ~WindowSort();
    WindowSort() = default;
    WindowSort(const WindowSort&) = delete;
    WindowSort& operator=(const WindowSort&) = delete;
    uint64_t n = 0, states = 0, nb1 = 0, nwin_total = 0;
    uint32_t nb2 = 1, shift1 = 0;
    bool two = false, started = false, finished = false;
    DevBuf ent1, ent2;
    DevBuf* words = nullptr;
    uint32_t *cur1 = nullptr, *cur2 = nullptr;
};
Status direct_sort_finish_full(cph_ctx* ctx, const uint32_t* slots, uint64_t n, uint32_t* sorted_out, uint32_t* flag);
Status exclusive_scan_u32(cph_ctx* ctx, uint32_t* data, uint64_t n);
Status exclusive_scan_u32_total(cph_ctx* ctx, uint32_t* data, uint64_t n, uint32_t* total_out);
Status exclusive_scan_u64(cph_ctx* ctx, uint64_t* data, uint64_t n, uint64_t* total_out);
Status gather_u64(cph_ctx* ctx, const uint64_t* src, const uint32_t* idx, uint64_t* dst, uint64_t n);
Status fill_iota_u32(cph_ctx* ctx, uint32_t* dst, uint64_t n);

Status index_first_dup_launch(cph_ctx* ctx, cph_index* ix);
Status index_first_dup_read(cph_ctx* ctx, cph_index* ix);
void index_plan_table(cph_index* ix);
Status index_ensure_table(cph_ctx* ctx, const cph_index* ix);
Status index_ensure_rowtab(cph_ctx* ctx, const cph_index* ix);
Status index_ensure_ranktab(cph_ctx* ctx, const cph_index* ix);
inline uint64_t ranktab_blocks(uint64_t table_entries) { return ((table_entries + 31) / 32 + 1) & ~1ull; }
Status index_ensure_hash(cph_ctx* ctx, const cph_index* ix);
bool index_wants_hash(const cph_index* ix);
struct ProbeOut {
    DevBuf lo, cnt, pidx, brow;
    uint64_t nprobe = 0, nmatches = 0;
};
struct RowSel {
    const void* ptr = nullptr;
    int32_t bits = 32;
    uint64_t base = 0;
};
Status probe_run(cph_ctx* ctx, const cph_index* ix, const DevCol* cols, int32_t ncols, RowSel sel,
                 uint64_t nprobe, uint64_t probe_base, bool want_pairs, ProbeOut* out, bool positions = false);
Status index_find_device(cph_ctx* ctx, const cph_index* ix, const uint64_t* q_exact, int32_t nq, uint64_t qlo,
                         uint64_t qhi, uint64_t* lower, uint64_t* upper);
Status index_find_many_device(cph_ctx* ctx, const cph_index* ix, const uint64_t* queries, size_t stride, uint64_t nkeys,
                              uint64_t* lower, uint64_t* upper);

void index_desc_serialize(const cph_index* ix, std::vector<uint8_t>* out);
size_t index_desc_header_bytes();
bool index_desc_size(const uint8_t* p, size_t n, size_t* need);
bool index_desc_parse(const uint8_t* p, size_t n, cph_index* ix);
Status index_adopt_payload(cph_ctx* ctx, cph_index* ix);
size_t index_code_bytes(const cph_index* ix);

struct ChainStep {
    const cph_index* index = nullptr;
    DevCol cols[kMaxKeyCols];
    int32_t ncols = 0;
    int32_t source = 0;
};
struct ChainOut {
    DevBuf stream_row;
    DevBuf build_row[CPH_MAX_CHAIN];
    uint64_t nrows = 0;
    int32_t nsteps = 0;
    bool identity = false;
};
Status chain_run(cph_ctx* ctx, const ChainStep* steps, int nsteps, uint64_t probe_base, ChainOut* out, bool positions = false);
bool chain_fast_path_ok(const ChainStep* steps, int nsteps);
Status chain_enqueue_dense(cph_ctx* ctx, const ChainStep* steps, int nsteps, uint64_t nprobe, uint64_t probe_base,
                           uint32_t* const* d_rows, uint64_t* d_masks, uint32_t* d_counts, uint64_t* d_total, bool positions = false);
Status chain_enqueue_codes(cph_ctx* ctx, const cph_index* const* idx, const uint32_t* const* d_codes, int nsteps, uint64_t nprobe,
                           uint32_t* const* d_rows, uint64_t* d_masks, uint32_t* d_counts, uint64_t* d_total, bool positions);
uint64_t chain_dense_mask_words(uint64_t nprobe);
uint64_t chain_dense_count_words(uint64_t nprobe);

void warm_keycodec();
void warm_radix_sort();
void warm_probe();
void warm_chain();
void warm_materialize();
void warm_csv_ingest();
void warm_index_ops();
void warm_small_build();
void warm_window_sort();
Status build_from_host_codes(cph_ctx* ctx, const cph_strcol* keycols, int32_t nkeycols, cph_index* ix, bool unique, bool* taken);
void host_pool_destroy(cph_ctx* ctx);

constexpr int kSmallMaxPos = 64;
enum : uint32_t { kSmallBuilt = 0, kSmallNotSmall = 1, kSmallPending = 0xFFFFFFFFu };
struct SmallResult {
    uint32_t status;
    uint32_t first_dup;
    uint32_t bits, key32, passes;
    uint32_t minlen[kMaxKeyCols], maxlen[kMaxKeyCols];
    uint32_t mask[kSmallMaxPos][8];
    uint64_t t[10];
    uint64_t codec_check;
};
CPH_HD inline uint64_t small_codec_check(uint64_t h, uint64_t radix, uint64_t mult) {
    h = (h ^ radix) * 0x9E3779B97F4A7C15ull;
    return (h ^ mult) * 0xC2B2AE3D27D4EB4Full + 1;
}
struct SmallBufs {
    DevBuf ka, kb, va, vb, sorted, perm;
};
bool small_build_applies(const cph_ctx* ctx, const DevCol* cols, int32_t ncols, uint64_t n);
Status small_build_launch(cph_ctx* ctx, const DevCol* cols, int32_t ncols, uint64_t n, SmallBufs* bufs, SmallResult* res);
Status small_build_finish(cph_ctx* ctx, cph_index* ix, int32_t ncols, SmallBufs* bufs, const SmallResult* res, bool* not_small);

Status ensure_pinned_scratch(cph_ctx* ctx, size_t bytes);
Status pinned_cache_get(cph_ctx* ctx, size_t bytes, void** out, size_t* cap);
void pinned_cache_put(cph_ctx* ctx, void* p, size_t cap);
Status pinned_upload(cph_ctx* ctx, size_t bytes, void** out);
Status validate_cols(const cph_strcol* cols, int32_t ncols);
Status stage_cols(cph_ctx* ctx, const cph_strcol* cols, int32_t ncols, std::vector<DevBuf>* storage, DevCol* out);
Status check_row_sources(const cph_strcol* cols, const cph_rowsel* sel, int32_t ncols, uint64_t first_row, uint64_t nrows, bool exact);
Status stage_row_sources(cph_ctx* ctx, const cph_strcol* cols, const cph_rowsel* sel, const int* order, int32_t ncols, uint64_t first_row,
                         uint64_t n, std::vector<DevBuf>* staged, ColsArg* arg, ColIds* ids);

inline int32_t fail_with(cph_ctx* ctx, const Status& s) {
    if (ctx) ctx->err = s.msg;
    return s.code;
}

struct ResultOwner {
    cph_ctx* ctx = nullptr;
    void* h_block = nullptr;
    ResultOwner() = default;
    ResultOwner(const ResultOwner&) = delete;
    ResultOwner& operator=(const ResultOwner&) = delete;
    ~ResultOwner() {
        if (h_block) (void)hipHostFree(h_block);
    }
};
struct ResultPart {
    DevBuf* dev;
    size_t bytes;
    void* pub;
    const void* src = nullptr;
};
Status deliver(cph_ctx* ctx, ResultOwner* owner, const ResultPart* parts, int nparts, int32_t out_mem);

template <class Impl, class Pub>
int32_t finish_call(cph_ctx* ctx, Impl* r, const Status& s, Pub** out) {
    if (!s.ok()) {
        (void)hipStreamSynchronize(ctx->stream);
        delete r;
        return fail_with(ctx, s);
    }
    *out = &r->pub;
    return CPH_OK;
}
template <class Impl, class Pub>
void release_result(Pub* pub) {
    if (!pub) return;
    auto* r = reinterpret_cast<Impl*>(pub);
    if (r->own.ctx) (void)hipSetDevice(r->own.ctx->device);
    delete r;
}

template <class T>
Status read_device_value(cph_ctx* ctx, const T* dev, T* host) {
    CPH_TRY(ensure_pinned_scratch(ctx, sizeof(T)));
    CPH_HIP_TRY(hipMemcpyAsync(ctx->pinned_scratch, dev, sizeof(T), hipMemcpyDeviceToHost, ctx->stream));
    CPH_HIP_TRY(hipStreamSynchronize(ctx->stream));
    memcpy(host, ctx->pinned_scratch, sizeof(T));
    return {};
}

Status kernel_setup(cph_ctx* ctx, const void* fn, int threads, size_t lds, int* blocks_per_cu);
Status device_cus(cph_ctx* ctx, int* cus);

inline unsigned grid_for_items(uint64_t n, unsigned cap = 8192) {
    uint64_t b = (n + 255) / 256;
    if (b > cap) b = cap;
    return (unsigned)(b ? b : 1);
}

class ProfScope {
public:
    ProfScope(cph_ctx* ctx, const char* name, double bytes);
// ... 10 lines not shown
```

### csvplus_amd/csrc/keycodec.hip

```cpp
#include <algorithm>
#include <cmath>
#include <mutex>

#include "codec_device.hpp"
#include "host_encode_kernels.hpp"

namespace cph {

constexpr int kStatsThreads = 256;
constexpr int kStatsRows = 8;

template <class B, bool SEG>
__global__ __launch_bounds__(kStatsThreads) void k_col_stats(DevCol col, uint32_t* __restrict__ g_minmax,
                                                            uint32_t* __restrict__ g_mask) {
    __shared__ __attribute__((aligned(16))) uint8_t s_flag[kMaxKeyBytes * 256];
    __shared__ uint32_t s_min, s_max;
    {
        uint4* z = reinterpret_cast<uint4*>(s_flag);
        for (int i = threadIdx.x; i < kMaxKeyBytes * 256 / 16; i += kStatsThreads) z[i] = make_uint4(0, 0, 0, 0);
    }
    if (threadIdx.x == 0) { s_min = 0xFFFFFFFFu; s_max = 0; }
    __syncthreads();

    uint32_t mn = 0xFFFFFFFFu, mx = 0;
// ... 895 lines not shown
            s_flag[q * 256u + byte] = 1;
            if (v.find(0x0101010101010101ull * (uint64_t)byte) == q) atomicAdd(&s_cnt[byte], 1u);
        }
    }
    mx = wave_max(mx);
    mn = wave_min(mn);
    if (lane_id() == 0) { atomicMax(&s_max, mx); atomicMin(&s_min, mn); }
    lds_atomics_barrier();
    for (int i = threadIdx.x; i < 256; i += kSplitThreads)
        if (s_cnt[i]) atomicAdd(&out->cnt[i], s_cnt[i]);
    for (int i = threadIdx.x; i < kSplitMaxValue * 8; i += kSplitThreads) {
        const uint32_t* f = reinterpret_cast<const uint32_t*>(s_flag + 32 * i);
        uint32_t bits = 0;
#pragma unroll
        for (int x = 0; x < 8; x++) {
            const uint32_t q = f[x];
            bits |= ((q & 1u) | ((q >> 7) & 2u) | ((q >> 14) & 4u) | ((q >> 21) & 8u)) << (4 * x);
        }
        uint32_t* gm = &out->mask[0][0] + i;
        if (bits && (__hip_atomic_load(gm, __ATOMIC_RELAXED, __HIP_MEMORY_SCOPE_AGENT) & bits) != bits) atomicOr(gm, bits);
    }
    if (threadIdx.x == 0) { atomicMax(&out->maxlen, s_max); atomicMax(&out->minlen_inv, ~s_min); }
    if (host_out) {
        __shared__ uint32_t s_last;
        uint32_t* ticket = reinterpret_cast<uint32_t*>(out + 1);
        __threadfence();
        __syncthreads();
        if (threadIdx.x == 0) s_last = atomicAdd(ticket, 1u) == gridDim.x - 1u ? 1u : 0u;
        __syncthreads();
        if (s_last) {
            uint32_t* src = reinterpret_cast<uint32_t*>(out);
            uint32_t* dst = reinterpret_cast<uint32_t*>(host_out);
            for (uint32_t i = threadIdx.x; i < (uint32_t)(sizeof(SplitSample) / 4); i += kSplitThreads) dst[i] = atomicExch(&src[i], 0u);
            if (threadIdx.x == 0) atomicExch(ticket, 0u);
            __threadfence_system();
        }
    }
}

template <class OUT, int NCH, bool PLAIN32 = false>
__global__ __launch_bounds__(kSplitThreads) void k_encode_split(DevCol col, const uint8_t* __restrict__ g_codec, uint64_t n,
                                                               OUT* __restrict__ out, uint32_t tile_rows, uint32_t ntiles,
                                                               uint32_t* __restrict__ counts, uint32_t digit_mask, uint32_t bins,
                                                               int codec_bytes, uint32_t* __restrict__ miss, OUT inv, uint32_t vmax) {
    extern __shared__ __attribute__((aligned(16))) uint8_t smem[];
    const CodecView cv = codec_load_to_lds(g_codec, smem);
    const uint64_t dv = 0x0101010101010101ull * (uint64_t)((uint32_t)cv.hdr->split_byte & 0xFFu);
    const int vp = cv.hdr->split_vcol;
    const int ps = cv.hdr->col_start[vp + 1];
    const uint32_t smaxlen = (uint32_t)cv.hdr->col_maxlen[vp + 1];
    const OUT pmult = (OUT)cv.mult[cv.hdr->wide_pos];
    CPH_LDS OUT* s_lutw = (CPH_LDS OUT*)(smem + codec_bytes);
    uint32_t* s_hist = reinterpret_cast<uint32_t*>(smem + codec_bytes + (size_t)smaxlen * kLutStride * sizeof(OUT));
    for (uint32_t i = threadIdx.x; i < smaxlen * (uint32_t)kLutStride; i += kSplitThreads) {
        const uint32_t r = cv.lut[(uint32_t)ps * kLutStride + i];
        s_lutw[i] = r == kLutInvalid ? inv : (OUT)r * (OUT)cv.mult[ps + (int)(i / kLutStride)];
    }
    __syncthreads();
    const uint32_t hmask = (1u << cv.hdr->wide_hash_bits) - 1u, dmask = (1u << cv.hdr->wide_disp_bits) - 1u;
    const uint32_t per_xcd = (ntiles + 7) / 8, xcd = blockIdx.x & 7u;
    const uint32_t t_end = (xcd + 1) * per_xcd < ntiles ? (xcd + 1) * per_xcd : ntiles;
    uint32_t missed = 0;
    for (uint32_t tile = xcd * per_xcd + (blockIdx.x >> 3); tile < t_end; tile += gridDim.x >> 3) {
        if (counts) {
            for (uint32_t x = threadIdx.x; x < bins; x += kSplitThreads) s_hist[x] = 0;
            __syncthreads();
        }
        const uint64_t tile_end = (uint64_t)(tile + 1) * tile_rows < n ? (uint64_t)(tile + 1) * tile_rows : n;
        for (uint64_t base = (uint64_t)tile * tile_rows; base < tile_end; base += (uint64_t)kSplitThreads * kSplitRows) {
            ValueRegs<NCH> v[kSplitRows];
            {
                uint64_t b[kSplitRows], l[kSplitRows];
                if constexpr (PLAIN32) {
                    const uint32_t* __restrict__ offs = reinterpret_cast<const uint32_t*>(col.offsets);
                    uint32_t o0[kSplitRows], o1[kSplitRows];
#pragma unroll
                    for (int k = 0; k < kSplitRows; k++) {
                        const uint64_t i = base + (uint64_t)k * kSplitThreads + threadIdx.x;
                        const uint64_t r = i < n ? i : n - 1;
                        o0[k] = offs[r];
                        o1[k] = offs[r + 1];
                    }
#pragma unroll
                    for (int k = 0; k < kSplitRows; k++) v[k].load32(col, o0[k], o1[k] - o0[k]);
                } else {
#pragma unroll
                    for (int k = 0; k < kSplitRows; k++) {
                        const uint64_t i = base + (uint64_t)k * kSplitThreads + threadIdx.x;
                        value_span_whole(col, i < n ? i : n - 1, &b[k], &l[k]);
                    }
#pragma unroll
                    for (int k = 0; k < kSplitRows; k++) v[k].load(col, b[k], l[k]);
                }
            }
            uint32_t plen[kSplitRows], slen[kSplitRows], hh[kSplitRows], disp[kSplitRows], e[kSplitRows];
            uint64_t w[kSplitRows][4];
#pragma unroll
            for (int k = 0; k < kSplitRows; k++) {
                split_lengths(v[k], dv, &plen[k], &slen[k]);
                v[k].head_words(plen[k] < (uint32_t)kWideBytes ? plen[k] : (uint32_t)kWideBytes, w[k]);
                hh[k] = wide_hash_lo(w[k][0], w[k][1], w[k][2], w[k][3], plen[k]);
            }
#pragma unroll
            for (int k = 0; k < kSplitRows; k++) disp[k] = cv.wide_disp[hh[k] & dmask];
#pragma unroll
            for (int k = 0; k < kSplitRows; k++) e[k] = cv.wide_hash[((hh[k] >> 16) + disp[k]) & hmask];
            bool hit[kSplitRows];
#pragma unroll
            for (int k = 0; k < kSplitRows; k++) {
                const CPH_LDS WideKey* key = cv.wide + (e[k] ? e[k] - 1 : 0);
                const uint32_t klen = key->len;
                const uint64_t k0 = key->w[0], k1 = key->w[1], k2 = key->w[2];
                uint64_t diff = (k0 ^ w[k][0]) | (k1 ^ w[k][1]) | (k2 ^ w[k][2]);
                if constexpr (NCH > 3) diff |= key->w[3] ^ w[k][3];
                hit[k] = (e[k] != 0) & (klen == plen[k]) & (diff == 0);
            }
            OUT acc[kSplitRows];
            uint64_t w0[kSplitRows], w1[kSplitRows];
#pragma unroll
            for (int k = 0; k < kSplitRows; k++) {
                const bool ok = hit[k] && v[k].len <= vmax && plen[k] <= (uint32_t)kWideBytes && slen[k] <= smaxlen;
                if (!ok && base + (uint64_t)k * kSplitThreads + threadIdx.x < tile_end) missed = 1;
                acc[k] = (OUT)(hit[k] ? e[k] - 1 : 0u) * pmult;
                v[k].window(plen[k], &w0[k], &w1[k]);
            }
            for (uint32_t q = 0; q < smaxlen; q++) {
                const CPH_LDS OUT* lp = s_lutw + q * (uint32_t)kLutStride;
#pragma unroll
                for (int k = 0; k < kSplitRows; k++) {
                    const uint64_t src = q < 8u ? w0[k] : w1[k];
                    const uint32_t sym = q < slen[k] ? ((uint32_t)(src >> (8u * (q & 7u))) & 0xFFu) + 1u : 0u;
                    acc[k] += lp[sym];
                }
            }
#pragma unroll
            for (int k = 0; k < kSplitRows; k++) {
                const uint64_t i = base + (uint64_t)k * kSplitThreads + threadIdx.x;
                if (i < tile_end) {
                    if (inv && acc[k] >= inv) missed = 1;
                    out[i] = acc[k];
                    if (counts) atomicAdd(&s_hist[(uint32_t)acc[k] & digit_mask], 1u);
                }
            }
        }
        if (counts) {
            lds_atomics_barrier();
            for (uint32_t x = threadIdx.x; x < bins; x += kSplitThreads) counts[(uint64_t)x * ntiles + tile] = s_hist[x];
            __syncthreads();
        }
    }
    if (__ballot(missed) && lane_id() == 0) *miss = 1u;
}

__global__ __launch_bounds__(kSplitThreads) void k_sample_fixed8(DevCol col, uint64_t step, uint64_t n, SplitSample* __restrict__ out,
                                                                SplitSample* __restrict__ host_out) {
    __shared__ uint32_t s_mask[8 * 8];
    __shared__ uint32_t s_last;
    const uint32_t W = col.fixed_width;
    if (threadIdx.x < 64) s_mask[threadIdx.x] = 0;
    __syncthreads();
    const uint64_t stride = (uint64_t)gridDim.x * kSplitThreads;
    for (uint64_t i = (uint64_t)blockIdx.x * kSplitThreads + threadIdx.x; i < n; i += stride) {
        uint64_t b, l;
        value_span_whole(col, i * step, &b, &l);
        ValueRegs<1> v;
        v.load(col, b, l);
        for (uint32_t q = 0; q < W; q++) {
            const uint32_t byte = (uint32_t)(v.c[0] >> (8u * q)) & 0xFFu, bit = 1u << (byte & 31u);
            uint32_t* w = &s_mask[q * 8u + (byte >> 5)];
            if (!(*(volatile uint32_t*)w & bit)) atomicOr(w, bit);
        }
    }
    lds_atomics_barrier();
    if (threadIdx.x < 64) {
        const uint32_t bits = s_mask[threadIdx.x];
        uint32_t* gm = &out->mask[0][0] + threadIdx.x;
        if (bits && (__hip_atomic_load(gm, __ATOMIC_RELAXED, __HIP_MEMORY_SCOPE_AGENT) & bits) != bits) atomicOr(gm, bits);
    }
    uint32_t* ticket = reinterpret_cast<uint32_t*>(out + 1);
    __threadfence();
    __syncthreads();
    if (threadIdx.x == 0) s_last = atomicAdd(ticket, 1u) == gridDim.x - 1u ? 1u : 0u;
    __syncthreads();
    if (s_last) {
        uint32_t* src = &out->mask[0][0];
        uint32_t* dst = &host_out->mask[0][0];
        for (uint32_t i = threadIdx.x; i < (uint32_t)(kSplitMaxValue * 8); i += kSplitThreads) dst[i] = i < 64u ? atomicExch(&src[i], 0u) : 0u;
        if (threadIdx.x == 0) {
            host_out->maxlen = W;
            host_out->minlen_inv = ~W;
            atomicExch(ticket, 0u);
        }
        __threadfence_system();
    }
}

int codec_virtual_cols(const CodecHost& cd, const DevCol* real, int nreal, DevCol* out) {
    int nv = 0;
    for (int c = 0; c < nreal; c++) {
        if (cd.has_split() && c == cd.split_col) {
            DevCol a = real[c], b = real[c];
            a.split = b.split = (uint16_t)(0x100u | cd.split_byte);
            a.part = 0;
            b.part = 1;
            out[nv++] = a;
            out[nv++] = b;
        } else {
            out[nv++] = real[c];
        }
    }
    return nv;
}

bool codec_wide_perfect_hash(CodecHost* codec) {
    CodecHost& cd = *codec;
    const size_t n = cd.wdict.size();
    cd.wide_disp.clear();
    cd.wide_slots.clear();
    if (n == 0 || n > (size_t)kWideDictMax) return false;
    std::vector<uint32_t> h(n);
    for (size_t i = 0; i < n; i++) h[i] = wide_hash_lo(cd.wdict[i].w[0], cd.wdict[i].w[1], cd.wdict[i].w[2], cd.wdict[i].w[3], cd.wdict[i].len);
    size_t nslots = 4;
    while (nslots < 2 * n) nslots <<= 1;
    for (int attempt = 0; attempt < 3; attempt++, nslots <<= 1) {
        const size_t nbuckets = nslots / 4 > 0 ? nslots / 4 : 1;
        std::vector<std::vector<uint32_t>> bucket(nbuckets);
        for (size_t i = 0; i < n; i++) bucket[h[i] & (nbuckets - 1)].push_back((uint32_t)i);
        std::vector<size_t> order(nbuckets);
        for (size_t b = 0; b < nbuckets; b++) order[b] = b;
        std::sort(order.begin(), order.end(), [&](size_t a, size_t b) { return bucket[a].size() > bucket[b].size(); });
        std::vector<uint16_t> slots(nslots, 0), disp(nbuckets, 0);
        bool ok = true;
        for (size_t b : order) {
            if (bucket[b].empty()) break;
            bool placed = false;
            for (uint32_t d = 0; d < 65536u && !placed; d++) {
                std::vector<uint32_t> at;
                bool free_ = true;
                for (uint32_t i : bucket[b]) {
                    const uint32_t sl = ((h[i] >> 16) + d) & (uint32_t)(nslots - 1);
                    if (slots[sl] || std::find(at.begin(), at.end(), sl) != at.end()) { free_ = false; break; }
                    at.push_back(sl);
                }
                if (!free_) continue;
                for (size_t j = 0; j < at.size(); j++) slots[at[j]] = (uint16_t)(bucket[b][j] + 1);
                disp[b] = (uint16_t)d;
                placed = true;
            }
            if (!placed) { ok = false; break; }
        }
        if (ok) {
            cd.wide_disp = std::move(disp);
            cd.wide_slots = std::move(slots);
            return true;
        }
    }
    return false;
}

static bool wide_less(const WideKey& a, const WideKey& b) {
    const uint32_t m = a.len < b.len ? a.len : b.len;
    for (uint32_t i = 0; i < m; i++) {
        const uint8_t x = (uint8_t)(a.w[i >> 3] >> (8 * (i & 7))), y = (uint8_t)(b.w[i >> 3] >> (8 * (i & 7)));
        if (x != y) return x < y;
    }
    return a.len < b.len;
}

static double codec_sort_cost(const CodecHost& c) {
    if (c.nwords == 1) return (double)((c.word_bits[0] + 7) / 8) * (c.key32 ? 8.0 : 12.0);
    double cost = 0;
    for (int w = 0; w < c.nwords; w++) cost += (double)((c.word_bits[w] + 7) / 8) * 12.0 + 16.0;
    return cost;
}
static double radix_bits(const ColStats& st, uint32_t q) {
    int cnt = q >= st.minlen ? 1 : 0;
    for (int w = 0; w < 8; w++) cnt += __builtin_popcount(st.mask[q][w]);
    return std::log2((double)(cnt > 1 ? cnt : 1));
}

template <int NCH>
static void launch_split_stats(cph_ctx* ctx, const DevCol& col, const SplitCands& cands, uint64_t step, uint64_t rows, SplitSlot* slots, SplitStats* out) {
    uint64_t nblk = (rows + (uint64_t)kSplitThreads * kSplitRows - 1) / ((uint64_t)kSplitThreads * kSplitRows);
    if (nblk > 2048) nblk = 2048;
    if (nblk < 1) nblk = 1;
    hipLaunchKernelGGL((k_split_stats<NCH>), dim3((unsigned)nblk, cands.n), dim3(kSplitThreads), 0, ctx->stream, col, cands, step, rows, slots, out);
}
static double bits_sort_cost(double bits) {
    if (bits <= 32.0) return std::ceil(bits / 8.0) * 8.0;
    if (bits <= 63.0) return std::ceil(bits / 8.0) * 12.0;
    const double words = std::ceil(bits / 63.0);
    return std::ceil(bits / 8.0) * 12.0 + 16.0 * words;
}

static int split_pick(const cph_ctx* ctx, int c, const std::vector<int>& cand, const std::vector<SplitStats>& hs, uint64_t step, double most,
                      double plain_bits) {
    auto split_bits = [&](const SplitStats& st) {
        double bits = std::log2((double)(st.count > 1 ? st.count : 1));
        ColStats tmp{};
        tmp.minlen = ~st.smin_inv;
        memcpy(tmp.mask, st.mask, sizeof st.mask);
        for (uint32_t q = 0; q < st.smax && q < (uint32_t)kSplitMaxSuffix; q++) bits += radix_bits(tmp, q);
        return bits;
    };
    int best = -1;
    double best_bits = 1e30;
    for (size_t k = 0; k < cand.size(); k++) {
        const SplitStats& st = hs[k];
        if (st.flags || st.count == 0 || st.count > (uint32_t)kWideDictMax / (step > 1 ? 2 : 1) || st.smax > (uint32_t)kSplitMaxSuffix) continue;
        const double bits = split_bits(st);
        if (ctx->codec_debug) fprintf(stderr, "codec_try_split: column %d, byte 0x%02x: %u prefixes, suffix %u..%u bytes, %.1f bits (plain %.1f)\n", c, cand[k], st.count, ~st.smin_inv, st.smax, bits, most);
        if (bits < best_bits) { best_bits = bits; best = (int)k; }
    }
    if (best < 0 || bits_sort_cost(plain_bits - most + best_bits) >= bits_sort_cost(plain_bits)) return -1;
    return best;
}

static std::vector<int> split_candidates(const SplitSample& hsm, uint64_t nsel) {
    std::vector<int> cand;
    for (int b = 0; b < 256; b++)
        if ((double)hsm.cnt[b] >= 0.99 * (double)nsel) cand.push_back(b);
    auto alnum = [](int b) { return (b >= '0' && b <= '9') || (b >= 'a' && b <= 'z') || (b >= 'A' && b <= 'Z'); };
    std::sort(cand.begin(), cand.end(), [&](int a, int b) { return alnum(a) != alnum(b) ? !alnum(a) : hsm.cnt[a] > hsm.cnt[b]; });
    if (cand.size() > 8) cand.resize(8);
    return cand;
}

static Status split_assemble(const cph_ctx* ctx, int c, int ncols, const std::vector<ColStats>* stats, uint32_t d, const SplitStats& st,
                             std::vector<WideKey>* dict_io, double plain_bits, CodecHost* out, bool* usable) {
    *usable = false;
    std::vector<WideKey>& dict = *dict_io;
    const uint32_t pmin = ~st.pmin_inv, smin = ~st.smin_inv;
    std::sort(dict.begin(), dict.end(), wide_less);

    std::vector<ColStats> vstats;
    for (int k = 0; k < ncols; k++) {
        if (k != c) { vstats.push_back((*stats)[(size_t)k]); continue; }
        ColStats pre{}, suf{};
        pre.minlen = pmin;
        pre.maxlen = st.pmax;
        for (uint32_t q = 0; q < st.pmax; q++) pre.mask[q][0] = 1u;
        suf.minlen = smin;
        suf.maxlen = st.smax;
        memcpy(suf.mask, st.mask, sizeof st.mask);
        vstats.push_back(pre);
        vstats.push_back(suf);
    }
    uint64_t positions = 0;
    for (const auto& v : vstats) positions += v.maxlen;
    if (positions > (uint64_t)kMaxKeyBytes || st.pmax == 0) return {};
    CodecHost trial;
    CPH_TRY(codec_build(vstats, &trial));
    const int p0 = trial.col_start[c];
    trial.unit.assign((size_t)trial.npos, kUnitPos);
    trial.dict_off.assign((size_t)trial.npos, 0);
    trial.dict_len.assign((size_t)trial.npos, 0);
    trial.unit[(size_t)p0] = kUnitWide;
    trial.radix[(size_t)p0] = (uint16_t)dict.size();
    for (int sym = 0; sym < kLutStride; sym++) trial.lut[(size_t)p0 * kLutStride + (size_t)sym] = kLutInvalid;
    for (uint32_t i = 1; i < st.pmax; i++) {
        trial.unit[(size_t)p0 + i] = kUnitAbsorbed;
        trial.radix[(size_t)p0 + i] = 1;
        for (int sym = 0; sym < kLutStride; sym++) trial.lut[((size_t)p0 + i) * kLutStride + (size_t)sym] = 0;
    }
    trial.split_col = c;
    trial.split_byte = (uint8_t)d;
    trial.split_maxlen = (int32_t)st.vmax;
    trial.wdict = std::move(dict);
    if (!codec_wide_perfect_hash(&trial)) return {};
    CPH_TRY(codec_split_words(&trial));
    if (ctx->codec_debug)
        fprintf(stderr, "codec_try_split: column %d cut at 0x%02x: %zu prefixes (<= %u bytes), suffix %u..%u bytes: %d word(s), %d bits, sort cost %.0f (plain: %.1f bits%s)\n",
                c, d, trial.wdict.size(), st.pmax, smin, st.smax, trial.nwords, trial.word_bits[0], codec_sort_cost(trial), plain_bits,
                stats ? "" : " by the sample");
    *out = std::move(trial);
    *usable = true;
    return {};
}

bool codec_sample_applies(const cph_ctx* ctx, const DevCol* cols, int32_t ncols, uint64_t n) {
    return ctx->stats_sample != 0 && ncols == 1 && cols[0].fixed_width >= 1 && cols[0].fixed_width <= (uint32_t)kSplitMaxValue &&
           !cols[0].segmented() && n >= (1ull << 20);
}
size_t codec_sample_bytes() { return sizeof(SplitSample); }
Status codec_sample_launch(cph_ctx* ctx, const DevCol& col, uint64_t n, const void** host_copy) {
    const uint64_t step = n >> 16;
    const uint64_t nsel = (n + step - 1) / step;
    DevBuf& acc = ctx->self_clean[ctx->stream_slot].sample;
    CPH_TRY(self_clean_block(ctx, &acc, sizeof(SplitSample) + 16));
    uint32_t* hw = host_word(ctx, (uint32_t)(sizeof(SplitSample) / 4));
    if (!hw) return {CPH_ERR_HIP, "no pinned host memory for the sample's statistics"};
    ProfScope ps(ctx, "k_split_count", 0);
    uint64_t nblk = (nsel + kSplitThreads - 1) / kSplitThreads;
    if (nblk > 1024) nblk = 1024;
    if (col.fixed_width <= 8 && ctx->sample_lean)
        hipLaunchKernelGGL(k_sample_fixed8, dim3((unsigned)nblk), dim3(kSplitThreads), 0, ctx->stream, col, step, nsel, acc.as<SplitSample>(),
                           reinterpret_cast<SplitSample*>(hw));
    else
        hipLaunchKernelGGL(k_split_count, dim3((unsigned)nblk), dim3(kSplitThreads), 0, ctx->stream, col, step, nsel, acc.as<SplitSample>(),
                           reinterpret_cast<SplitSample*>(hw));
    if (hipGetLastError() != hipSuccess) {
        acc.reset();
        return {CPH_ERR_HIP, "k_split_count launch failed"};
    }
    *host_copy = hw;
    return {};
}
void codec_sample_finish(const DevCol& col, const void* host_copy, std::vector<ColStats>* out) {
    const SplitSample* sm = static_cast<const SplitSample*>(host_copy);
    out->assign(1, ColStats{});
    ColStats& st = (*out)[0];
    st.minlen = st.maxlen = col.fixed_width;
    static_assert(sizeof(sm->mask) <= sizeof(st.mask), "the sample's positions must fit ColStats");
    memcpy(st.mask, sm->mask, sizeof sm->mask);
}
bool codec_sample_checked(const CodecHost& cd, const DevCol* cols) {
    return !cd.has_split() && !cd.has_groups() && cd.ncols == 1 && cd.nwords == 1 && codec_premultiplied_bits(cd) != 0 && !cols[0].segmented();
}

Status codec_try_split(cph_ctx* ctx, const DevCol* cols, int32_t ncols, uint64_t n, const std::vector<ColStats>* stats, CodecHost* codec,
                       bool speculate, bool* speculated) {
    if (speculated) *speculated = false;
    if (!ctx->codec_split || n < (1ull << 16) || ncols >= kMaxKeyCols) return {};
    if (stats && (codec->key32 || codec->has_groups())) return {};
    if (!stats && ncols != 1) return {};
    int c = -1;
    double most = 0, plain_bits = 0;
    if (stats) {
        for (int k = 0; k < ncols; k++) {
            double bits = 0;
            for (uint32_t q = 0; q < (*stats)[(size_t)k].maxlen; q++) bits += radix_bits((*stats)[(size_t)k], q);
            plain_bits += bits;
            if (cols[k].fixed_width || cols[k].segmented() || (*stats)[(size_t)k].maxlen > (uint32_t)kSplitMaxValue || (*stats)[(size_t)k].maxlen < 4) continue;
            if (bits > most) { most = bits; c = k; }
        }
        if (c < 0 || most < 24.0) return {};
    } else {
        if (cols[0].fixed_width || cols[0].segmented()) return {};
        c = 0;
    }
    const DevCol& col = cols[c];
    const uint64_t step = n > (1ull << 19) ? n >> 18 : 1;
    const uint64_t nsel = (n + step - 1) / step;

    DevBuf sample;
    CPH_TRY(sample.alloc(&ctx->pool, sizeof(SplitSample)));
    CPH_HIP_TRY(hipMemsetAsync(sample.get(), 0, sizeof(SplitSample), ctx->stream));
    {
        ProfScope ps(ctx, "k_split_count", 0);
        uint64_t nblk = (nsel + kSplitThreads - 1) / kSplitThreads;
        if (nblk > 1024) nblk = 1024;
        hipLaunchKernelGGL(k_split_count, dim3((unsigned)nblk), dim3(kSplitThreads), 0, ctx->stream, col, step, nsel, sample.as<SplitSample>(), (SplitSample*)nullptr);
        CPH_HIP_TRY(hipGetLastError());
    }
    CPH_TRY(ensure_pinned_scratch(ctx, sizeof(SplitSample)));
    CPH_HIP_TRY(hipMemcpyAsync(ctx->pinned_scratch, sample.get(), sizeof(SplitSample), hipMemcpyDeviceToHost, ctx->stream));
    CPH_HIP_TRY(hipStreamSynchronize(ctx->stream));
    std::vector<SplitSample> hsv(1);
    SplitSample& hsm = hsv[0];
    memcpy(&hsm, ctx->pinned_scratch, sizeof hsm);
    if (hsm.maxlen > (uint32_t)kSplitMaxValue || hsm.maxlen < 4) return {};
    if (!stats) {
        ColStats tmp{};
        tmp.minlen = ~hsm.minlen_inv;
        memcpy(tmp.mask, hsm.mask, sizeof hsm.mask);
        for (uint32_t q = 0; q < hsm.maxlen; q++) most += radix_bits(tmp, q);
        plain_bits = most;
        if (most <= 32.0) return {};
    }
    const bool small_values = (stats ? (*stats)[(size_t)c].maxlen : hsm.maxlen) <= 24;
    const std::vector<int> cand = split_candidates(hsm, nsel);
    if (cand.empty()) return {};

    const size_t set_bytes = (size_t)kSplitSetSlots * sizeof(SplitSlot);
    DevBuf sets, sstats;
    CPH_TRY(sets.alloc(&ctx->pool, cand.size() * set_bytes));
    CPH_TRY(sstats.alloc(&ctx->pool, cand.size() * sizeof(SplitStats)));
    CPH_HIP_TRY(hipMemsetAsync(sets.get(), 0, cand.size() * set_bytes, ctx->stream));
    CPH_HIP_TRY(hipMemsetAsync(sstats.get(), 0, cand.size() * sizeof(SplitStats), ctx->stream));
    SplitCands all{};
    all.n = (uint32_t)cand.size();
    for (size_t k = 0; k < cand.size(); k++) all.d[k] = (uint8_t)cand[k];
    {
        ProfScope ps(ctx, "k_split_sample", 0);
        if (small_values) launch_split_stats<3>(ctx, col, all, step, nsel, sets.as<SplitSlot>(), sstats.as<SplitStats>());
        else launch_split_stats<5>(ctx, col, all, step, nsel, sets.as<SplitSlot>(), sstats.as<SplitStats>());
        CPH_HIP_TRY(hipGetLastError());
    }
    std::vector<SplitStats> hs(cand.size());
    CPH_TRY(ensure_pinned_scratch(ctx, cand.size() * sizeof(SplitStats)));
    CPH_HIP_TRY(hipMemcpyAsync(ctx->pinned_scratch, sstats.get(), cand.size() * sizeof(SplitStats), hipMemcpyDeviceToHost, ctx->stream));
    CPH_HIP_TRY(hipStreamSynchronize(ctx->stream));
    memcpy(hs.data(), ctx->pinned_scratch, cand.size() * sizeof(SplitStats));
    const int best = split_pick(ctx, c, cand, hs, step, most, plain_bits);
    if (best < 0) return {};

    SplitSlot* slots = sets.as<SplitSlot>() + (size_t)best * kSplitSetSlots;
    SplitStats* dstat = sstats.as<SplitStats>() + best;
    const uint32_t d = (uint32_t)cand[(size_t)best];
    const bool spec = speculate && step > 1 && ctx->split_speculative != 0;
    if (step > 1 && !spec) {
        ProfScope ps(ctx, "k_split_stats", 0);
        SplitCands one{};
        one.n = 1;
        one.d[0] = (uint8_t)d;
        if (small_values) launch_split_stats<3>(ctx, col, one, 1, n, slots, dstat);
        else launch_split_stats<5>(ctx, col, one, 1, n, slots, dstat);
        CPH_HIP_TRY(hipGetLastError());
    }
    CPH_TRY(ensure_pinned_scratch(ctx, sizeof(SplitStats) + set_bytes));
    uint8_t* hp = static_cast<uint8_t*>(ctx->pinned_scratch);
    CPH_HIP_TRY(hipMemcpyAsync(hp, dstat, sizeof(SplitStats), hipMemcpyDeviceToHost, ctx->stream));
    CPH_HIP_TRY(hipMemcpyAsync(hp + sizeof(SplitStats), slots, set_bytes, hipMemcpyDeviceToHost, ctx->stream));
    CPH_HIP_TRY(hipStreamSynchronize(ctx->stream));
    SplitStats st;
    memcpy(&st, hp, sizeof st);
    if (st.flags || st.count == 0 || st.count > (uint32_t)kWideDictMax || st.pmax > (uint32_t)kWideBytes || st.smax > (uint32_t)kSplitMaxSuffix ||
        st.vmax > (uint32_t)kSplitMaxValue)
        return {};
    std::vector<WideKey> dict;
    const SplitSlot* hsl = reinterpret_cast<const SplitSlot*>(hp + sizeof(SplitStats));
    for (int i = 0; i < kSplitSetSlots; i++)
        if (hsl[i].tag) {
            WideKey k{};
            for (int j = 0; j < 4; j++) k.w[j] = hsl[i].w[j];
            k.len = hsl[i].len;
            dict.push_back(k);
        }
    if (dict.size() != st.count) return {};
    CodecHost trial;
    bool usable = false;
    CPH_TRY(split_assemble(ctx, c, ncols, stats, d, st, &dict, plain_bits, &trial, &usable));
    if (!usable) return {};
    if (spec) {
        trial.spec_checked = true;
        if (trial.nwords != 1 || trial.word_states[0] > (trial.key32 ? (1ull << 27) : (1ull << 58)))
            return codec_try_split(ctx, cols, ncols, n, stats, codec, false, nullptr);
    }
    const double plain_cost = stats ? codec_sort_cost(*codec) : bits_sort_cost(plain_bits);
    if (codec_sort_cost(trial) < plain_cost) {
        *codec = std::move(trial);
        if (speculated) *speculated = spec;
    }
    return {};
}

Status codec_split_from_host(cph_ctx* ctx, const cph_host::HostCol& hc, uint64_t n, cph_host::BlockPool& pool, CodecHost* codec) {
    if (!ctx->codec_split || !ctx->split_speculative || hc.fixed_width || !hc.offsets || n < (1ull << 22)) return {};
    const uint64_t step = n >> 18;
    const uint64_t nsel = (n + step - 1) / step;
// ... 21 lines not shown
            const uint64_t b = bb[(i - i0) % kBatch], l = ll[(i - i0) % kBatch];
            const uint32_t l32 = l > 0xFFFFFFFFull ? 0xFFFFFFFFu : (uint32_t)l;
            loc.maxlen = l32 > loc.maxlen ? l32 : loc.maxlen;
            loc.minlen_inv = ~l32 > loc.minlen_inv ? ~l32 : loc.minlen_inv;
            uint32_t seen[8] = {0};
            const uint64_t m = l < (uint64_t)kSplitMaxValue ? l : (uint64_t)kSplitMaxValue;
            for (uint64_t q = 0; q < m; q++) {
                const uint8_t v = hc.data[b + q];
                if (!((seen[v >> 5] >> (v & 31)) & 1u)) {
                    seen[v >> 5] |= 1u << (v & 31);
                    loc.cnt[v]++;
                }
                loc.mask[q][v >> 5] |= 1u << (v & 31);
            }
        }
        std::lock_guard<std::mutex> lk(mu);
        for (int b = 0; b < 256; b++) hsm.cnt[b] += loc.cnt[b];
        hsm.maxlen = loc.maxlen > hsm.maxlen ? loc.maxlen : hsm.maxlen;
        hsm.minlen_inv = loc.minlen_inv > hsm.minlen_inv ? loc.minlen_inv : hsm.minlen_inv;
        for (int q = 0; q < kSplitMaxValue; q++)
            for (int w = 0; w < 8; w++) hsm.mask[q][w] |= loc.mask[q][w];
    }, 2048);
    if (hsm.maxlen > (uint32_t)kSplitMaxValue || hsm.maxlen < 4) return {};
    double most = 0;
    {
        ColStats tmp{};
        tmp.minlen = ~hsm.minlen_inv;
        memcpy(tmp.mask, hsm.mask, sizeof hsm.mask);
        for (uint32_t q = 0; q < hsm.maxlen; q++) most += radix_bits(tmp, q);
    }
    const double plain_bits = most;
    if (most <= 32.0) return {};
    const std::vector<int> cand = split_candidates(hsm, nsel);
    if (cand.empty()) return {};

    std::vector<SplitStats> hs(cand.size());
    std::vector<std::vector<WideKey>> dicts(cand.size());
    std::vector<std::vector<uint64_t>> dtags(cand.size());
    for (auto& x : hs) memset(&x, 0, sizeof x);
    pool.run(nsel, [&](uint64_t i0, uint64_t i1) {
        const size_t nc = cand.size();
        std::vector<SplitStats> loc(nc);
        for (auto& x : loc) memset(&x, 0, sizeof x);
        constexpr size_t kSlots = 4096;
        std::vector<uint64_t> tags(nc * kSlots, 0ull);
        std::vector<WideKey> keys(nc * kSlots);
        std::vector<uint32_t> nkeys(nc, 0);
        constexpr uint64_t kBatch = 32;
        uint64_t bb[kBatch], ll[kBatch];
        for (uint64_t i = i0; i < i1; i++) {
            if ((i - i0) % kBatch == 0) {
                const uint64_t m2 = i1 - i < kBatch ? i1 - i : kBatch;
                for (uint64_t k = 0; k < m2; k++) __builtin_prefetch(static_cast<const uint8_t*>(hc.offsets) + (i + k) * step * (uint64_t)(hc.offset_bits / 8));
                for (uint64_t k = 0; k < m2; k++) {
                    span((i + k) * step, &bb[k], &ll[k]);
                    __builtin_prefetch(hc.data + bb[k]);
                }
            }
            const uint64_t b = bb[(i - i0) % kBatch], l = ll[(i - i0) % kBatch];
            const uint8_t* p = hc.data + b;
            for (size_t k = 0; k < nc; k++) {
                SplitStats& st = loc[k];
                const void* f = l ? memchr(p, cand[k], (size_t)l) : nullptr;
                const uint64_t plen = f ? (uint64_t)((const uint8_t*)f - p) + 1 : l, slen = l - plen;
                const bool usable = l <= (uint64_t)kSplitMaxValue && plen <= (uint64_t)kWideBytes;
                if (!usable) st.flags |= 1u;
                if (slen > (uint64_t)kSplitMaxSuffix) st.flags |= 2u;
                st.rows_with += f ? 1u : 0u;
                const uint32_t pl = plen > 0xFFFFFFFFull ? 0xFFFFFFFFu : (uint32_t)plen, sl = slen > 0xFFFFFFFFull ? 0xFFFFFFFFu : (uint32_t)slen;
                const uint32_t vl = l > 0xFFFFFFFFull ? 0xFFFFFFFFu : (uint32_t)l;
                st.pmin_inv = ~pl > st.pmin_inv ? ~pl : st.pmin_inv;
                st.pmax = pl > st.pmax ? pl : st.pmax;
                st.smin_inv = ~sl > st.smin_inv ? ~sl : st.smin_inv;
                st.smax = sl > st.smax ? sl : st.smax;
                st.vmax = vl > st.vmax ? vl : st.vmax;
                if (usable && !(st.flags & 4u)) {
                    WideKey key{};
                    memcpy(key.w, p, (size_t)plen);
                    key.len = pl;
                    const uint64_t tag = wide_hash(key.w[0], key.w[1], key.w[2], key.w[3], pl);
                    uint64_t* tg = &tags[k * kSlots];
                    WideKey* ky = &keys[k * kSlots];
                    size_t h = (size_t)(tag >> 32) & (kSlots - 1);
                    while (tg[h] != 0ull && !(tg[h] == tag && ky[h].len == pl && memcmp(ky[h].w, key.w, sizeof key.w) == 0)) h = (h + 1) & (kSlots - 1);
                    if (tg[h] == 0ull) {
                        if (nkeys[k] >= (uint32_t)kWideDictMax) st.flags |= 4u;
                        else { tg[h] = tag; ky[h] = key; nkeys[k]++; }
                    }
                }
                const uint64_t lim = slen < (uint64_t)kSplitMaxSuffix ? slen : (uint64_t)kSplitMaxSuffix;
                for (uint64_t q = 0; q < lim; q++) {
                    const uint8_t v = p[plen + q];
                    st.mask[q][v >> 5] |= 1u << (v & 31);
                }
            }
        }
        std::lock_guard<std::mutex> lk(mu);
        for (size_t k = 0; k < nc; k++) {
            SplitStats& g = hs[k];
            const SplitStats& st = loc[k];
            g.flags |= st.flags;
            g.rows_with += st.rows_with;
            g.pmin_inv = st.pmin_inv > g.pmin_inv ? st.pmin_inv : g.pmin_inv;
            g.pmax = st.pmax > g.pmax ? st.pmax : g.pmax;
            g.smin_inv = st.smin_inv > g.smin_inv ? st.smin_inv : g.smin_inv;
            g.smax = st.smax > g.smax ? st.smax : g.smax;
            g.vmax = st.vmax > g.vmax ? st.vmax : g.vmax;
            for (int q = 0; q < kSplitMaxSuffix; q++)
                for (int w = 0; w < 8; w++) g.mask[q][w] |= st.mask[q][w];
            if (dtags[k].empty()) { dtags[k].assign(kSlots, 0ull); dicts[k].assign(kSlots, WideKey{}); }
            for (size_t s2 = 0; s2 < kSlots && !(g.flags & 4u); s2++) {
                const uint64_t tag = tags[k * kSlots + s2];
                if (!tag) continue;
                const WideKey& key = keys[k * kSlots + s2];
                size_t h = (size_t)(tag >> 32) & (kSlots - 1);
                while (dtags[k][h] != 0ull && !(dtags[k][h] == tag && dicts[k][h].len == key.len && memcmp(dicts[k][h].w, key.w, sizeof key.w) == 0)) h = (h + 1) & (kSlots - 1);
                if (dtags[k][h] == 0ull) {
                    if (g.count >= (uint32_t)kWideDictMax) g.flags |= 4u;
                    else { dtags[k][h] = tag; dicts[k][h] = key; g.count++; }
                }
            }
        }
    }, 2048);
    const int best = split_pick(ctx, 0, cand, hs, step, most, plain_bits);
    if (best < 0) return {};
    const SplitStats& st = hs[(size_t)best];
    if (st.flags || st.count == 0 || st.count > (uint32_t)kWideDictMax || st.pmax > (uint32_t)kWideBytes || st.smax > (uint32_t)kSplitMaxSuffix ||
        st.vmax > (uint32_t)kSplitMaxValue)
        return {};
    std::vector<WideKey> dict;
    for (size_t s2 = 0; s2 < dtags[(size_t)best].size(); s2++)
        if (dtags[(size_t)best][s2]) dict.push_back(dicts[(size_t)best][s2]);
    if (dict.size() != st.count) return {};
    CodecHost trial;
    bool usable = false;
    CPH_TRY(split_assemble(ctx, 0, 1, nullptr, (uint32_t)cand[(size_t)best], st, &dict, plain_bits, &trial, &usable));
    if (!usable) return {};
    trial.spec_checked = true;
    if (trial.nwords != 1 || !trial.key32 || trial.word_states[0] > (1ull << 27)) return {};
    if (codec_sort_cost(trial) < bits_sort_cost(plain_bits)) *codec = std::move(trial);
    return {};
}

int codec_premultiplied_bits(const CodecHost& cd) {
    if (cd.nwords != 1 || cd.npos <= 0 || cd.has_groups()) return 0;
    const int bits = cd.word_states[0] <= (1ull << 31) ? 32 : 64;
    return (size_t)cd.npos * kLutStride * (size_t)(bits / 8) <= 48 * 1024 ? bits : 0;
}

void codec_arith_plan(const CodecHost& cd, ArithPlan* ap) {
    *ap = ArithPlan{};
    if (cd.ncols != 1 || cd.nwords != 1 || cd.has_groups() || cd.npos < 1 || cd.npos > 8) return;
    if (cd.col_minlen[0] != cd.col_maxlen[0] || cd.word_states[0] > (1ull << 31)) return;
    uint32_t lo[8] = {0}, rng[8] = {0}, radix[8] = {1, 1, 1, 1, 1, 1, 1, 1};
    for (int p = 0; p < cd.npos; p++) {
        const uint16_t* lut = &cd.lut[(size_t)p * kLutStride];
        if (lut[0] != kLutInvalid) return;
        int first = -1, last = -1, count = 0;
        for (int b = 0; b < 256; b++)
            if (lut[1 + b] != kLutInvalid) { if (first < 0) first = b; last = b; count++; }
        if (first < 0 || last >= 0x80 || last - first + 1 != count || count > 255 || count != (int)cd.radix[(size_t)p]) return;
        for (int b = first; b <= last; b++)
            if (lut[1 + b] != (uint16_t)(b - first)) return;
        lo[p] = (uint32_t)first;
        rng[p] = (uint32_t)(last - first);
        radix[p] = (uint32_t)count;
    }
    ap->keylen = (uint32_t)cd.npos;
    for (int w = 0; w < 2; w++) {
        for (int i = 0; i < 4; i++) {
            const int p = 4 * w + i;
            if (p < cd.npos) ap->keep[w] |= 0xFFu << (8 * i);
            ap->lo[w] |= lo[p] << (8 * i);
            ap->rngc[w] |= (0x7Fu - rng[p]) << (8 * i);
        }
        ap->wa[w] = radix[4 * w + 1] | 1u << 8;
        ap->wb[w] = radix[4 * w + 3] << 16 | 1u << 24;
        ap->ma[w] = radix[4 * w + 2] * radix[4 * w + 3];
    }
    const uint64_t s0 = (uint64_t)radix[0] * radix[1] * radix[2] * radix[3];
    const uint64_t s1 = (uint64_t)radix[4] * radix[5] * radix[6] * radix[7];
    ap->s1 = (uint32_t)s1;
    ap->mul24 = s0 <= (1ull << 24) && s1 < (1ull << 24) ? 1u : 0u;
    ap->enabled = 1;
}

Status codec_upload(cph_ctx* ctx, const CodecHost& cd, DevBuf* dev) {
    CodecDevHeader h{};
    h.ncols = cd.ncols;
    h.npos = cd.npos;
    h.nwords = cd.nwords;
    h.key32 = cd.key32 ? 1 : 0;
    for (int c = 0; c <= cd.ncols; c++) h.col_start[c] = cd.col_start[c];
    for (int c = cd.ncols + 1; c <= kMaxKeyCols; c++) h.col_start[c] = cd.npos;
    for (int c = 0; c < cd.ncols; c++) h.col_maxlen[c] = cd.col_maxlen[c];
    auto align16 = [](size_t x) { return (x + 15) & ~(size_t)15; };
    size_t off = align16(sizeof(CodecDevHeader));
    h.mult_off = (int32_t)off;
    off = align16(off + sizeof(uint64_t) * (size_t)cd.npos);
    h.wordof_off = (int32_t)off;
    off = align16(off + (size_t)cd.npos + 1);
    const int lutw_bits = codec_premultiplied_bits(cd);
    h.lutw_bits = lutw_bits;
    if (lutw_bits) {
        h.lut_off = 0;
        h.lutw_off = (int32_t)off;
        off = align16(off + (size_t)(lutw_bits / 8) * (size_t)cd.npos * kLutStride);
    } else {
        h.lutw_off = 0;
        h.lut_off = (int32_t)off;
        off = align16(off + sizeof(uint16_t) * (size_t)cd.npos * kLutStride);
    }
    if (cd.has_groups()) {
        h.ngroups = 0;
        for (int p = 0; p < cd.npos; p++) h.ngroups += cd.unit[(size_t)p] == kUnitHead || cd.unit[(size_t)p] == kUnitWide;
        h.unit_off = (int32_t)off;
        off = align16(off + (size_t)cd.npos);
        h.dictoff_off = (int32_t)off;
        off = align16(off + sizeof(int32_t) * (size_t)cd.npos);
        h.dictlen_off = (int32_t)off;
        off = align16(off + sizeof(int32_t) * (size_t)cd.npos);
        h.dict_off = (int32_t)off;
        off = align16(off + sizeof(uint64_t) * cd.dict.size());
        h.hashoff_off = (int32_t)off;
        off = align16(off + sizeof(int32_t) * (size_t)cd.npos);
        h.hashbits_off = (int32_t)off;
        off = align16(off + sizeof(int32_t) * (size_t)cd.npos);
        h.hash_off = (int32_t)off;
        size_t slots = 0;
        for (int p = 0; p < cd.npos; p++)
            if (cd.unit[(size_t)p] == kUnitHead) slots += (size_t)1 << (bits_needed((uint64_t)cd.dict_len[(size_t)p] * 2) + 0);
        off = align16(off + sizeof(uint16_t) * slots);
    }
    h.wide_pos = -1;
    h.split_vcol = -1;
    int wide_bits = 0;
    if (cd.has_split()) {
        h.split_vcol = cd.split_col;
        h.split_byte = cd.split_byte;
        h.wide_pos = cd.col_start[cd.split_col];
        h.wide_n = (int32_t)cd.wdict.size();
        h.wide_off = (int32_t)off;
        off = align16(off + sizeof(WideKey) * cd.wdict.size());
        if (cd.wide_slots.empty() || cd.wide_disp.empty()) return {CPH_ERR_INVALID, "internal: split codec without its perfect hash"};
        wide_bits = bits_needed((uint64_t)cd.wide_slots.size());
        h.wide_hash_bits = wide_bits;
        h.wide_hash_off = (int32_t)off;
        off = align16(off + sizeof(uint16_t) * cd.wide_slots.size());
        h.wide_disp_bits = bits_needed((uint64_t)cd.wide_disp.size());
        h.wide_disp_off = (int32_t)off;
        off = align16(off + sizeof(uint16_t) * cd.wide_disp.size());
    }
    h.total_bytes = (int32_t)off;

    std::vector<uint8_t> blob(off, 0);
    memcpy(blob.data(), &h, sizeof h);
    if (cd.has_split()) {
        memcpy(blob.data() + h.wide_off, cd.wdict.data(), sizeof(WideKey) * cd.wdict.size());
        memcpy(blob.data() + h.wide_hash_off, cd.wide_slots.data(), sizeof(uint16_t) * cd.wide_slots.size());
        memcpy(blob.data() + h.wide_disp_off, cd.wide_disp.data(), sizeof(uint16_t) * cd.wide_disp.size());
    }
    if (cd.has_groups()) {
        memcpy(blob.data() + h.unit_off, cd.unit.data(), (size_t)cd.npos);
        memcpy(blob.data() + h.dictoff_off, cd.dict_off.data(), sizeof(int32_t) * (size_t)cd.npos);
        memcpy(blob.data() + h.dictlen_off, cd.dict_len.data(), sizeof(int32_t) * (size_t)cd.npos);
        memcpy(blob.data() + h.dict_off, cd.dict.data(), sizeof(uint64_t) * cd.dict.size());
        int32_t* hoff = reinterpret_cast<int32_t*>(blob.data() + h.hashoff_off);
        int32_t* hbits = reinterpret_cast<int32_t*>(blob.data() + h.hashbits_off);
        uint16_t* hash = reinterpret_cast<uint16_t*>(blob.data() + h.hash_off);
        size_t base = 0;
        for (int p = 0; p < cd.npos; p++) {
            if (cd.unit[(size_t)p] != kUnitHead) continue;
            const int bits = bits_needed((uint64_t)cd.dict_len[(size_t)p] * 2);
            const uint32_t mask = (1u << bits) - 1u;
            hoff[p] = (int32_t)base;
            hbits[p] = bits;
            for (int32_t r = 0; r < cd.dict_len[(size_t)p]; r++) {
                uint32_t sl = bits ? group_slot(cd.dict[(size_t)(cd.dict_off[(size_t)p] + r)], bits) : 0u;
                while (hash[base + sl]) sl = (sl + 1) & mask;
                hash[base + sl] = (uint16_t)(r + 1);
            }
            base += (size_t)1 << bits;
        }
    }
    if (cd.npos) {
        memcpy(blob.data() + h.mult_off, cd.mult.data(), sizeof(uint64_t) * (size_t)cd.npos);
        for (int p = 0; p < cd.npos; p++) blob[(size_t)h.wordof_off + (size_t)p] = (uint8_t)cd.word_of[(size_t)p];
        blob[(size_t)h.wordof_off + (size_t)cd.npos] = 0xFF;
        if (lutw_bits == 32) {
            uint32_t* w = reinterpret_cast<uint32_t*>(blob.data() + h.lutw_off);
            for (size_t i = 0; i < (size_t)cd.npos * kLutStride; i++) {
                const uint16_t r = cd.lut[i];
                w[i] = r == kLutInvalid ? 0x80000000u : (uint32_t)((uint64_t)r * cd.mult[i / kLutStride]);
            }
        } else if (lutw_bits == 64) {
            uint64_t* w = reinterpret_cast<uint64_t*>(blob.data() + h.lutw_off);
            for (size_t i = 0; i < (size_t)cd.npos * kLutStride; i++) {
                const uint16_t r = cd.lut[i];
                w[i] = r == kLutInvalid ? 0x8000000000000000ull : (uint64_t)r * cd.mult[i / kLutStride];
            }
        } else {
            memcpy(blob.data() + h.lut_off, cd.lut.data(), sizeof(uint16_t) * (size_t)cd.npos * kLutStride);
        }
    }
    CPH_TRY(dev->alloc(&ctx->pool, off));
    void* slot = nullptr;
    CPH_TRY(pinned_upload(ctx, off, &slot));
    memcpy(slot, blob.data(), off);
    CPH_HIP_TRY(hipMemcpyAsync(dev->get(), slot, off, hipMemcpyHostToDevice, ctx->stream));
    return {};
}

constexpr int kEncodeThreads = 256;

template <bool KEY32>
__global__ __launch_bounds__(kEncodeThreads) void k_encode_build(ColsArg cols, const uint8_t* __restrict__ g_codec,
                                                                uint64_t n, void* __restrict__ out, uint32_t* __restrict__ miss) {
    extern __shared__ __attribute__((aligned(16))) uint8_t smem[];
    const CodecView cv = codec_load_to_lds(g_codec, smem);
    const int ncols = cv.hdr->ncols;
    const uint64_t stride = (uint64_t)gridDim.x * kEncodeThreads;
    bool all_valid = true;
    for (uint64_t row = (uint64_t)blockIdx.x * kEncodeThreads + threadIdx.x; row < n; row += stride) {
        if constexpr (KEY32) {
            uint32_t code = 0;
            all_valid &= encode_key(cv, cols, ncols, row, [&](int, uint64_t v, int) { code = (uint32_t)v; });
            reinterpret_cast<uint32_t*>(out)[row] = code;
        } else {
            uint64_t* o = reinterpret_cast<uint64_t*>(out);
            if (cv.hdr->npos == 0) o[row] = 0;
            all_valid &= encode_key(cv, cols, ncols, row, [&](int word, uint64_t v, int) { o[(uint64_t)word * n + row] = v; });
        }
    }
    if (miss && !all_valid) *miss = 1u;
}

constexpr int kEncodeRows = 4;
// ... 471 lines not shown
```

### csvplus_amd/csrc/window_sort.hip

```cpp
#include "cph_internal.hpp"
#include "codec_device.hpp"
#include "device_utils.hpp"

namespace cph {

constexpr int kWpThreads = 512;
constexpr int kWpItems = 16;
constexpr int kWpTile = kWpThreads * kWpItems;
constexpr int kWpMaxBuckets = 2048;
constexpr int kWinBits = 14;
constexpr uint32_t kWinSlots = 1u << kWinBits;
constexpr uint32_t kWinEmpty = 0xFFFFFFFFu;
constexpr int kPlaceThreads = 512;

struct WpArgs {
    const uint64_t* keys;
    ArithPlan ap;
    const uint32_t* codes;
    const uint64_t* entries;
    const uint32_t* src_count;
    uint64_t n;
    uint32_t src_cap;
    uint32_t tiles_per_src;
    uint32_t shift;
    uint32_t nb;
    uint64_t* dst;
    uint32_t* dst_count;
    uint32_t states;
    uint32_t row_base;
    uint32_t* flag;
};

template <int SRC>
__global__ __launch_bounds__(kWpThreads) void k_win_partition(WpArgs a) {
    constexpr bool FROM_CODES = SRC != 0;
    extern __shared__ __attribute__((aligned(16))) uint8_t smem[];
    __shared__ uint32_t s_tmp[kWpThreads / kWave + 1];
    const uint32_t nbp = (a.nb + (uint32_t)kWpThreads - 1u) & ~((uint32_t)kWpThreads - 1u);
    uint64_t* s_ent = reinterpret_cast<uint64_t*>(smem);
    uint32_t* s_hist = reinterpret_cast<uint32_t*>(s_ent + kWpTile);
    uint32_t* s_start = s_hist + nbp;
    uint32_t* s_delta = s_start + nbp;
    const uint32_t sb = blockIdx.x / a.tiles_per_src, tl = blockIdx.x % a.tiles_per_src;
    uint64_t cnt = a.n;
    if constexpr (!FROM_CODES) {
        const uint32_t c = a.src_count[sb];
        cnt = c < a.src_cap ? c : a.src_cap;
    }
    const uint64_t t0 = (uint64_t)tl * kWpTile;
    if (t0 >= cnt) return;
    const uint32_t m = cnt - t0 < (uint64_t)kWpTile ? (uint32_t)(cnt - t0) : (uint32_t)kWpTile;
    const uint64_t src0 = FROM_CODES ? t0 : (uint64_t)sb * a.src_cap + t0;
    const uint32_t t = threadIdx.x;
    for (uint32_t i = t; i < nbp; i += kWpThreads) s_hist[i] = 0;
    __syncthreads();
    typedef unsigned int u32x4 __attribute__((ext_vector_type(4)));
    uint32_t code[kWpItems], row[kWpItems], rank[kWpItems];
    if constexpr (SRC == 2) {
        uint64_t c0[kWpItems];
        uint32_t okm = 0;
#pragma unroll
        for (int j = 0; j < kWpItems / 4; j++) {
            const uint32_t i4 = 4u * ((uint32_t)j * kWpThreads + t);
            if (i4 + 3 < m) {
                const u32x4 v0 = reinterpret_cast<const u32x4*>(a.keys + src0 + i4)[0], v1 = reinterpret_cast<const u32x4*>(a.keys + src0 + i4)[1];
                c0[4 * j] = (uint64_t)v0.x | ((uint64_t)v0.y << 32);
                c0[4 * j + 1] = (uint64_t)v0.z | ((uint64_t)v0.w << 32);
                c0[4 * j + 2] = (uint64_t)v1.x | ((uint64_t)v1.y << 32);
                c0[4 * j + 3] = (uint64_t)v1.z | ((uint64_t)v1.w << 32);
                okm |= 0xFu << (4 * j);
            } else {
#pragma unroll
                for (int c = 0; c < 4; c++) {
                    c0[4 * j + c] = i4 + c < m ? a.keys[src0 + i4 + c] : 0ull;
                    okm |= (i4 + c < m ? 1u : 0u) << (4 * j + c);
                }
            }
#pragma unroll
            for (int c = 0; c < 4; c++) row[4 * j + c] = a.row_base + (uint32_t)(t0 + i4 + c);
        }
        const uint32_t have = okm;
        encode_rows_arith<kWpItems, uint32_t>(a.ap, c0, code, &okm);
        bool bad = false;
#pragma unroll
        for (int k = 0; k < kWpItems; k++) {
            const bool ok = ((okm >> k) & 1u) && code[k] < a.states;
            bad |= ((have >> k) & 1u) && !ok;
            code[k] = ok ? code[k] : kWinEmpty;
        }
        if (__ballot(bad) && lane_id() == 0) *a.flag = 1u;
    } else if constexpr (SRC == 1) {
        const bool vec = m == (uint32_t)kWpTile && (((uintptr_t)(a.codes + src0)) & 15) == 0;
#pragma unroll
        for (int j = 0; j < kWpItems / 4; j++) {
            const uint32_t i4 = 4u * ((uint32_t)j * kWpThreads + t);
            uint32_t w[4];
            if (vec) {
                const u32x4 v = reinterpret_cast<const u32x4*>(a.codes + src0)[i4 >> 2];
                w[0] = v.x; w[1] = v.y; w[2] = v.z; w[3] = v.w;
            } else {
#pragma unroll
                for (int c = 0; c < 4; c++) w[c] = i4 + c < m ? a.codes[src0 + i4 + c] : kWinEmpty;
            }
#pragma unroll
            for (int c = 0; c < 4; c++) {
                const bool ok = i4 + c < m && w[c] < a.states;
                code[4 * j + c] = ok ? w[c] : kWinEmpty;
                row[4 * j + c] = a.row_base + (uint32_t)(t0 + i4 + c);
            }
        }
    } else {
        const bool vec = m == (uint32_t)kWpTile;
#pragma unroll
        for (int j = 0; j < kWpItems / 2; j++) {
            const uint32_t i2 = 2u * ((uint32_t)j * kWpThreads + t);
            if (vec) {
                const u32x4 v = reinterpret_cast<const u32x4*>(a.entries + src0)[i2 >> 1];
                row[2 * j] = v.x; code[2 * j] = v.y; row[2 * j + 1] = v.z; code[2 * j + 1] = v.w;
            } else {
#pragma unroll
                for (int c = 0; c < 2; c++) {
                    const uint64_t e = i2 + c < m ? a.entries[src0 + i2 + c] : ~0ull;
                    row[2 * j + c] = (uint32_t)e;
                    code[2 * j + c] = i2 + c < m ? (uint32_t)(e >> 32) : kWinEmpty;
                }
            }
        }
    }
#pragma unroll
    for (int k = 0; k < kWpItems; k++) rank[k] = code[k] != kWinEmpty ? atomicAdd(&s_hist[code[k] >> a.shift], 1u) : 0u;
    lds_atomics_barrier();
    uint32_t tot;
    {
        const uint32_t per = nbp / kWpThreads;
        uint32_t h[kWpMaxBuckets / kWpThreads], sum = 0;
#pragma unroll
        for (int k = 0; k < kWpMaxBuckets / kWpThreads; k++) {
            h[k] = (uint32_t)k < per ? s_hist[t * per + k] : 0u;
            sum += h[k];
        }
        uint32_t run = block_exclusive_sum<uint32_t, kWpThreads>(sum, s_tmp, &tot);
#pragma unroll
        for (int k = 0; k < kWpMaxBuckets / kWpThreads; k++) {
            if ((uint32_t)k < per) {
                const uint32_t b = t * per + k;
                s_start[b] = run;
                if (h[k]) s_delta[b] = atomicAdd(&a.dst_count[(uint64_t)sb * a.nb + b], h[k]) - run;
                run += h[k];
            }
        }
    }
    __syncthreads();
#pragma unroll
    for (int k = 0; k < kWpItems; k++)
        if (code[k] != kWinEmpty) s_ent[s_start[code[k] >> a.shift] + rank[k]] = ((uint64_t)code[k] << 32) | row[k];
    __syncthreads();
    const uint32_t cap = 1u << a.shift, mask = cap - 1u;
    bool over = false;
    uint64_t e[kWpItems];
    uint32_t pos[kWpItems];
#pragma unroll
    for (int k = 0; k < kWpItems; k++) {
        const uint32_t i = (uint32_t)k * kWpThreads + t;
        e[k] = s_ent[i < tot ? i : 0u];
    }
#pragma unroll
    for (int k = 0; k < kWpItems; k++) {
        const uint32_t i = (uint32_t)k * kWpThreads + t;
        pos[k] = s_delta[i < tot ? (uint32_t)(e[k] >> 32) >> a.shift : 0u] + i;
    }
#pragma unroll
    for (int k = 0; k < kWpItems; k++) {
        const uint32_t i = (uint32_t)k * kWpThreads + t;
        if (i < tot) {
            const uint32_t w = (uint32_t)(e[k] >> 32), b = w >> a.shift;
            if (pos[k] < cap) a.dst[(((uint64_t)sb * a.nb + b) << a.shift) + pos[k]] = ((uint64_t)(w & mask) << 32) | (uint32_t)e[k];
            else over = true;
        }
    }
    if (__ballot(over) && lane_id() == 0) *a.flag = 1u;
}

__global__ __launch_bounds__(1024) void k_win_offsets(const uint32_t* __restrict__ counts, uint32_t nwin, uint32_t* __restrict__ off) {
    __shared__ uint32_t s_tmp[1024 / kWave + 1];
    uint32_t carry = 0;
    for (uint32_t base = 0; base < nwin; base += 1024) {
        const uint32_t i = base + threadIdx.x;
        uint32_t v = i < nwin ? counts[i] : 0u;
        v = v < kWinSlots ? v : kWinSlots;
        uint32_t total;
        const uint32_t ex = block_exclusive_sum<uint32_t, 1024>(v, s_tmp, &total);
        if (i < nwin) off[i] = carry + ex;
        carry += total;
    }
}

__global__ __launch_bounds__(kPlaceThreads) void k_win_place(const uint64_t* __restrict__ entries, uint32_t* __restrict__ counts,
                                                            const uint32_t* __restrict__ off, uint64_t n, uint32_t* __restrict__ perm,
                                                            uint32_t* __restrict__ sorted, uint32_t* __restrict__ flag,
                                                            uint32_t* __restrict__ clear_also, uint32_t nclear, uint2* __restrict__ ranktab,
                                                            uint32_t rank_blocks) {
    extern __shared__ __attribute__((aligned(16))) uint8_t smem[];
    __shared__ uint32_t s_wcount[kPlaceThreads / kWave];
    typedef unsigned int u32x4 __attribute__((ext_vector_type(4)));
    uint32_t* win = reinterpret_cast<uint32_t*>(smem);
    const uint32_t g = blockIdx.x, t = threadIdx.x;
    const uint32_t craw = counts[g], cnt = craw < kWinSlots ? craw : kWinSlots;
    {
        u32x4 e;
        e.x = e.y = e.z = e.w = kWinEmpty;
        for (uint32_t i = t; i < kWinSlots / 4; i += kPlaceThreads) reinterpret_cast<u32x4*>(win)[i] = e;
    }
    __syncthreads();
    if (t == 0) {
        counts[g] = 0u;
        if (g < nclear) clear_also[g] = 0u;
    }
    const uint64_t* src = entries + ((uint64_t)g << kWinBits);
    for (uint32_t i = t; i < cnt; i += kPlaceThreads) {
        const uint64_t e = src[i];
        win[(uint32_t)(e >> 32) & (kWinSlots - 1u)] = (uint32_t)e;
    }
    __syncthreads();
    constexpr uint32_t kWaves = kPlaceThreads / kWave, kPerWave = kWinSlots / kWaves, kIters = kPerWave / kWave;
    const uint32_t wave = (uint32_t)wave_id(), lane = (uint32_t)lane_id();
    const uint32_t s0 = wave * kPerWave;
    uint32_t c = 0;
#pragma unroll 4
    for (uint32_t it = 0; it < kIters; it++) c += (uint32_t)__popcll(__ballot(win[s0 + it * kWave + lane] != kWinEmpty));
    if (lane == 0) s_wcount[wave] = c;
    __syncthreads();
    uint32_t before = 0, filled = 0;
#pragma unroll
    for (uint32_t w = 0; w < kWaves; w++) {
        const uint32_t x = s_wcount[w];
        before += w < wave ? x : 0u;
        filled += x;
    }
    if (t == 0 && (filled != craw)) *flag = 1u;
    uint64_t pos = (off ? (uint64_t)off[g] : ((uint64_t)g << kWinBits)) + before;
    const uint64_t lt = lanemask_lt();
    const uint32_t code0 = (g << kWinBits) + s0;
    for (uint32_t it = 0; it < kIters; it++) {
        const uint32_t v = win[s0 + it * kWave + lane];
        const uint64_t bal = __ballot(v != kWinEmpty);
        if (ranktab && lane < 2) {
            const uint32_t blk = ((code0 + it * kWave) >> 5) + lane;
            if (blk < rank_blocks)
                ranktab[blk] = make_uint2(lane ? (uint32_t)(bal >> 32) : (uint32_t)bal, (uint32_t)pos + (lane ? (uint32_t)__popc((uint32_t)bal) : 0u));
        }
        if (v != kWinEmpty) {
            const uint64_t p = pos + (uint64_t)__popcll(bal & lt);
            if (p < n) {
                perm[p] = v;
                sorted[p] = code0 + it * kWave + lane;
            }
        }
        pos += (uint64_t)__popcll(bal);
    }
}

Status WindowSort::begin(cph_ctx* ctx, uint64_t n_, uint64_t states_) {
    n = n_;
    states = states_;
    const uint64_t nwin = (states + kWinSlots - 1) >> kWinBits;
    two = nwin > (uint64_t)kWpMaxBuckets;
    int k2 = 0;
    if (two) {
        int wb = 0;
        while ((1ull << wb) < nwin) wb++;
        k2 = (wb + 1) / 2;
    }
    nb2 = 1u << k2;
    shift1 = (uint32_t)kWinBits + (uint32_t)k2;
    nb1 = two ? (states + (1ull << shift1) - 1) >> shift1 : nwin;
    if (nb1 > (uint64_t)kWpMaxBuckets) return {CPH_ERR_INVALID, "direct_sort_windows: code space too large"};
    nwin_total = two ? nb1 * nb2 : nwin;
    CPH_TRY(ent1.alloc(&ctx->pool, (nb1 << shift1) * sizeof(uint64_t)));
    if (two) CPH_TRY(ent2.alloc(&ctx->pool, (nwin_total << kWinBits) * sizeof(uint64_t)));
    const uint64_t nwords = nb1 + (two ? nwin_total : 0);
    words = &ctx->self_clean[ctx->stream_slot].win;
    CPH_TRY(self_clean_block(ctx, words, nwords * sizeof(uint32_t)));
    cur1 = words->as<uint32_t>();
    cur2 = two ? cur1 + nb1 : cur1;
    started = true;
    return {};
}
WindowSort::~WindowSort() {
    if (started && !finished && words) words->reset();
}

static size_t win_partition_lds(uint32_t nb) {
    const uint32_t nbp = (nb + (uint32_t)kWpThreads - 1u) & ~((uint32_t)kWpThreads - 1u);
    return (size_t)kWpTile * 8 + (size_t)nbp * 12;
}

Status WindowSort::add(cph_ctx* ctx, const uint32_t* codes, uint64_t row0, uint64_t m, uint32_t* flag, const uint64_t* keys, const ArithPlan* ap) {
    if (m == 0) return {};
    WpArgs a{};
    a.codes = codes;
    a.keys = keys;
    if (keys) a.ap = *ap;
    a.n = m;
    a.tiles_per_src = (uint32_t)((m + kWpTile - 1) / kWpTile);
    a.shift = shift1;
    a.nb = (uint32_t)nb1;
    a.dst = ent1.as<uint64_t>();
    a.dst_count = cur1;
    a.states = (uint32_t)states;
    a.row_base = (uint32_t)row0;
    a.flag = flag;
    const size_t lds = win_partition_lds(a.nb);
    if (keys) {
        CPH_TRY(kernel_setup(ctx, reinterpret_cast<const void*>(&k_win_partition<2>), kWpThreads, lds, nullptr));
        ProfScope ps(ctx, "k_win_partition", 16.0 * (double)m);
        hipLaunchKernelGGL(k_win_partition<2>, dim3(a.tiles_per_src), dim3(kWpThreads), lds, ctx->stream, a);
    } else {
        CPH_TRY(kernel_setup(ctx, reinterpret_cast<const void*>(&k_win_partition<1>), kWpThreads, lds, nullptr));
        ProfScope ps(ctx, "k_win_partition", 12.0 * (double)m);
        hipLaunchKernelGGL(k_win_partition<1>, dim3(a.tiles_per_src), dim3(kWpThreads), lds, ctx->stream, a);
    }
    CPH_HIP_TRY(hipGetLastError());
    return {};
}

Status WindowSort::finish(cph_ctx* ctx, uint32_t* perm_out, uint32_t* sorted_out, uint32_t* flag, void* ranktab, uint64_t rank_blocks) {
    const bool need_off = states != n;
    DevBuf offsets;
    if (need_off) CPH_TRY(offsets.alloc(&ctx->pool, nwin_total * sizeof(uint32_t)));
    uint32_t* off = offsets.as<uint32_t>();
    if (two) {
        WpArgs a{};
        a.entries = ent1.as<uint64_t>();
        a.src_count = cur1;
        a.src_cap = 1u << shift1;
        a.tiles_per_src = (a.src_cap + kWpTile - 1) / kWpTile;
        a.shift = (uint32_t)kWinBits;
        a.nb = nb2;
        a.dst = ent2.as<uint64_t>();
        a.dst_count = cur2;
        a.flag = flag;
        const size_t lds = win_partition_lds(a.nb);
        CPH_TRY(kernel_setup(ctx, reinterpret_cast<const void*>(&k_win_partition<0>), kWpThreads, lds, nullptr));
        ProfScope ps(ctx, "k_win_partition", 16.0 * (double)n);
        hipLaunchKernelGGL(k_win_partition<0>, dim3((unsigned)(nb1 * a.tiles_per_src)), dim3(kWpThreads), lds, ctx->stream, a);
        CPH_HIP_TRY(hipGetLastError());
    }
    uint32_t* counts = two ? cur2 : cur1;
    if (need_off) {
        ProfScope ps(ctx, "k_win_place", 0);
        hipLaunchKernelGGL(k_win_offsets, dim3(1), dim3(1024), 0, ctx->stream, counts, (uint32_t)nwin_total, off);
    }
    {
        const size_t lds = (size_t)kWinSlots * sizeof(uint32_t);
        CPH_TRY(kernel_setup(ctx, reinterpret_cast<const void*>(&k_win_place), kPlaceThreads, lds, nullptr));
        ProfScope ps(ctx, "k_win_place", 16.0 * (double)n);
        hipLaunchKernelGGL(k_win_place, dim3((unsigned)nwin_total), dim3(kPlaceThreads), lds, ctx->stream, two ? ent2.as<uint64_t>() : ent1.as<uint64_t>(),
                           counts, need_off ? off : nullptr, n, perm_out, sorted_out, flag, cur1, two ? (uint32_t)nb1 : 0u,
                           static_cast<uint2*>(ranktab), (uint32_t)rank_blocks);
    }
    CPH_HIP_TRY(hipGetLastError());
    finished = true;
    return {};
}

Status direct_sort_windows(cph_ctx* ctx, const uint32_t* codes, uint64_t n, uint64_t states, uint32_t* perm_out, uint32_t* sorted_out,
                           uint32_t* flag, void* ranktab, uint64_t rank_blocks) {
    if (n == 0) return {};
    WindowSort ws;
    CPH_TRY(ws.begin(ctx, n, states));
    CPH_TRY(ws.add(ctx, codes, 0, n, flag));
    return ws.finish(ctx, perm_out, sorted_out, flag, ranktab, rank_blocks);
}
Status direct_sort_windows_keys(cph_ctx* ctx, const uint64_t* keys, const ArithPlan& ap, uint64_t n, uint64_t states, uint32_t* perm_out,
                                uint32_t* sorted_out, uint32_t* flag, void* ranktab, uint64_t rank_blocks) {
    if (n == 0) return {};
    WindowSort ws;
    CPH_TRY(ws.begin(ctx, n, states));
    CPH_TRY(ws.add(ctx, nullptr, 0, n, flag, keys, &ap));
    return ws.finish(ctx, perm_out, sorted_out, flag, ranktab, rank_blocks);
}

}

namespace cph {
void warm_window_sort() {
    hipFuncAttributes a;
    (void)hipFuncGetAttributes(&a, reinterpret_cast<const void*>(&k_win_offsets));
    (void)hipGetLastError();
}
}
```

Before: 132.5 billion rows/s.

## Speculatively launch window sort from a device-computed plan before host sampling readback

When a unique single fixed-width-8 key index is built with sampling, the sample kernel now also emits a device-side SpecPlan (arith plan, state count, rank blocks), and the window-sort kernels launch right away reading that plan from device memory. This removes the host round trip between sampling and sort. The host later checks the device plan against its own codec build and either adopts the speculative perm, sorted codes and rank table, or falls back to the normal path. It costs extra allocations sized for up to 2n states, an event per job, and wasted sort work when the verdict is a mismatch. It also shrinks the partition kernel's LDS by aliasing s_start onto s_hist.

```diff
diff --git a/csvplus_amd/csrc/capi.hip b/csvplus_amd/csrc/capi.hip
--- a/csvplus_amd/csrc/capi.hip
+++ b/csvplus_amd/csrc/capi.hip
@@ -525,9 +525,23 @@
     bool exact_split = false;
     bool no_split = false;
     uint32_t* miss = nullptr;
+    bool spec_sort = false;
+    bool spec_adopted = false;
+    hipEvent_t sample_done = nullptr;
+    DevBuf spec_plan_dev, spec_perm, spec_sorted, spec_rt;
+    const SpecPlan* spec_plan_host = nullptr;
     uint32_t* cs_over = nullptr;
     DevBuf cs_codes;
 };
+
+static Status job_arm_miss(cph_ctx* ctx, BuildJob* job);
+static bool spec_sort_applies(const cph_ctx* ctx, const BuildJob& job) {
+    const DevCol& kc = job.dcols[0];
+    return ctx->direct_spec != 0 && job.sampled && job.unique && !job.no_direct && ctx->direct_sort == 1 && ctx->direct_fused_encode != 0 &&
+           ctx->sample_lean != 0 && job.nkeycols == 1 && kc.fixed_width == 8 && !kc.segmented() && ((uintptr_t)kc.data & 15) == 0 &&
+           job.ix->nrows >= (1ull << 16) && job.ix->nrows <= (1ull << 30);
+}
+static uint64_t spec_rank_blocks_room(uint64_t n) { return ranktab_blocks(2 * n < (1ull << 30) ? 2 * n : (1ull << 30)); }
 
 static Status build_phase1(cph_ctx* ctx, const cph_strcol* keycols, int32_t nkeycols, BuildJob* job) {
     CPH_TRY(validate_cols(keycols, nkeycols));
@@ -544,12 +558,37 @@
         job->presplit = ix->codec.has_split();
     }
     job->sampled = !job->small && !job->presplit && !job->no_sample && codec_sample_applies(ctx, job->dcols, nkeycols, ix->nrows);
-    if (job->sampled) CPH_TRY(codec_sample_launch(ctx, job->dcols[0], ix->nrows, &job->sample_host));
+    if (job->sampled && spec_sort_applies(ctx, *job)) {
+        CPH_TRY(job_arm_miss(ctx, job));
+        CPH_TRY(job->spec_plan_dev.alloc(&ctx->pool, sizeof(SpecPlan)));
+        CPH_TRY(codec_sample_launch(ctx, job->dcols[0], ix->nrows, &job->sample_host, job->spec_plan_dev.as<SpecPlan>(), &job->spec_plan_host,
+                                    ctx->direct_ranktab != 0));
+        if (ctx->spec_events.empty()) {
+            CPH_HIP_TRY(hipEventCreateWithFlags(&job->sample_done, hipEventDisableTiming));
+        } else {
+            job->sample_done = ctx->spec_events.back();
+            ctx->spec_events.pop_back();
+        }
+        CPH_HIP_TRY(hipEventRecord(job->sample_done, ctx->stream));
+        job->spec_sort = true;
+    } else if (job->sampled) CPH_TRY(codec_sample_launch(ctx, job->dcols[0], ix->nrows, &job->sample_host));
     else if (!job->small && !job->presplit) CPH_TRY(codec_stats_launch(ctx, job->dcols, nkeycols, &job->stats_dev));
     return {};
 }
 
+static Status build_spec_launch(cph_ctx* ctx, BuildJob* job) {
+    if (!job->spec_sort) return {};
+    const uint64_t n = job->ix->nrows;
+    CPH_TRY(job->spec_perm.alloc(&ctx->pool, n * sizeof(uint32_t)));
+    CPH_TRY(job->spec_sorted.alloc(&ctx->pool, n * sizeof(uint32_t)));
+    if (ctx->direct_ranktab) CPH_TRY(job->spec_rt.alloc(&ctx->pool, spec_rank_blocks_room(n) * 8));
+    return direct_sort_windows_spec(ctx, reinterpret_cast<const uint64_t*>(job->dcols[0].data), job->spec_plan_dev.as<SpecPlan>(), n,
+                                    job->spec_perm.as<uint32_t>(), job->spec_sorted.as<uint32_t>(), job->miss, job->spec_rt.get());
+}
+
 static Status build_phase2(cph_ctx* ctx, BuildJob* job, const void* stats_host);
+enum class SpecVerdict { adopted, not_qualified, mismatch };
+static Status build_spec_verify(cph_ctx* ctx, BuildJob* job, SpecVerdict* verdict);
 static Status job_arm_miss(cph_ctx* ctx, BuildJob* job) {
     job->miss = host_word(ctx);
     return job->miss ? Status{} : Status{CPH_ERR_HIP, "no pinned host memory for the report words of a build"};
@@ -566,6 +605,12 @@
         for (size_t i = 0; i < nj; i++)
             if (status[i].ok()) status[i] = s;
     };
+    for (size_t i = 0; i < nj; i++)
+        if (!status[i].ok() && jobs[i].sample_done) {
+            ctx->spec_events.push_back(jobs[i].sample_done);
+            jobs[i].sample_done = nullptr;
+            jobs[i].spec_sort = false;
+        }
     size_t total = 0;
     bool any_general = false;
     for (size_t i = 0; i < nj; i++) {
@@ -595,8 +640,14 @@
     auto sync_streams = [&]() {
         return hipStreamSynchronize(ctx->stream) == hipSuccess && (!any_side || hipStreamSynchronize(ctx->side_stream) == hipSuccess);
     };
-    if (!sync_streams()) return fail_all({CPH_ERR_HIP, "hipStreamSynchronize failed"});
-    ctx->pool.flush_deferred();
+    bool wait_main = false, wait_side = false, spec_main = false, spec_side = false;
+    for (size_t i = 0; i < nj; i++) {
+        if (!status[i].ok()) continue;
+        (jobs[i].spec_sort ? (jobs[i].side ? spec_side : spec_main) : (jobs[i].side ? wait_side : wait_main)) = true;
+    }
+    if ((wait_main && hipStreamSynchronize(ctx->stream) != hipSuccess) || (wait_side && hipStreamSynchronize(ctx->side_stream) != hipSuccess))
+        return fail_all({CPH_ERR_HIP, "hipStreamSynchronize failed"});
+    if ((wait_main || wait_side) && (wait_main || !spec_main) && (wait_side || !spec_side)) ctx->pool.flush_deferred();
     std::vector<std::vector<uint8_t>> stats_host(nj);
     std::vector<size_t> retry;
     for (size_t i = 0; i < nj; i++) {
@@ -610,6 +661,7 @@
             else if (status[i].ok()) index_plan_table(jobs[i].ix);
             continue;
         }
+        if (jobs[i].spec_sort) continue;
         if (jobs[i].sampled) {
             const uint8_t* sh = static_cast<const uint8_t*>(jobs[i].sample_host);
             stats_host[i].assign(sh, sh + codec_sample_bytes());
@@ -618,10 +670,27 @@
         }
     }
     for (size_t i = 0; i < nj; i++)
-        if (status[i].ok() && !jobs[i].small) {
+        if (status[i].ok() && !jobs[i].small && !jobs[i].spec_sort) {
             SideStream on_side(ctx, jobs[i].side);
             status[i] = build_phase2(ctx, &jobs[i], stats_host[i].data());
         }
+    for (size_t i = 0; i < nj; i++) {
+        if (!status[i].ok() || !jobs[i].spec_sort) continue;
+        BuildJob& j = jobs[i];
+        SideStream on_side(ctx, j.side);
+        SpecVerdict v = SpecVerdict::mismatch;
+        if (hipEventSynchronize(j.sample_done) != hipSuccess) status[i] = {CPH_ERR_HIP, "hipEventSynchronize failed"};
+        else status[i] = build_spec_verify(ctx, &j, &v);
+        ctx->spec_events.push_back(j.sample_done);
+        j.sample_done = nullptr;
+        if (!status[i].ok()) continue;
+        j.spec_adopted = v == SpecVerdict::adopted;
+        if (v != SpecVerdict::not_qualified) continue;
+        j.spec_sort = false;
+        j.miss = nullptr;
+        j.spec_plan_dev.reset(); j.spec_perm.reset(); j.spec_sorted.reset(); j.spec_rt.reset();
+        status[i] = build_phase2(ctx, &j, j.sample_host);
+    }
     std::vector<size_t> resplit;
     std::vector<size_t> resort;
     if (any_general) {
@@ -644,6 +713,7 @@
             if (!status[i].ok() || jobs[i].small) continue;
             cph_index* ix = jobs[i].ix;
             if (jobs[i].miss) sm[i] = *(volatile uint32_t*)jobs[i].miss;
+            if (jobs[i].spec_sort && !jobs[i].spec_adopted) sm[i] = 1;
             if (sm[i]) { jobs[i].cs_codes.reset(); jobs[i].cs_over = nullptr; resplit.push_back(i); continue; }
             if (jobs[i].cs_over && *(volatile uint32_t*)jobs[i].cs_over) { resort.push_back(i); continue; }
             jobs[i].cs_codes.reset();
@@ -713,6 +783,8 @@
         std::vector<Status> st1(1);
         BuildJob& j = one[0];
         j.side = false;
+        j.spec_sort = j.spec_adopted = false;
+        j.spec_plan_dev.reset(); j.spec_perm.reset(); j.spec_sorted.reset(); j.spec_rt.reset();
         const bool again_exact = j.spec_split;
         j.spec_split = false;
         j.exact_split = again_exact;
@@ -881,6 +953,39 @@
     return build_encode_sort(ctx, job);
 }
 
+static Status build_spec_verify(cph_ctx* ctx, BuildJob* job, SpecVerdict* verdict) {
+    cph_index* ix = job->ix;
+    const uint64_t n = ix->nrows;
+    SpecPlan dev;
+    memcpy(&dev, job->spec_plan_host, sizeof dev);
+    if (dev.ok == 0) {
+        *verdict = SpecVerdict::not_qualified;
+        return {};
+    }
+    *verdict = SpecVerdict::mismatch;
+    std::vector<ColStats> stats;
+    codec_sample_finish(job->dcols[0], job->sample_host, &stats);
+    CPH_TRY(codec_build(stats, &ix->codec));
+    const CodecHost& cd = ix->codec;
+    if (!codec_sample_checked(cd, job->dcols) || cd.nwords != 1 || !cd.key32) return {};
+    const uint64_t states = cd.word_states[0];
+    if (!(states >= n && states <= 2 * n && states < 0xFFFFFFFFull)) return {};
+    ArithPlan ap;
+    codec_arith_plan(cd, &ap);
+    if (!ap.enabled || ap.keylen != 8) return {};
+    const uint64_t rt_blocks = job->spec_rt && states != n && states <= (1ull << 30) ? ranktab_blocks(states) : 0;
+    if (memcmp(&ap, &dev.ap, sizeof ap) != 0 || (uint64_t)dev.states != states || (uint64_t)dev.rank_blocks != rt_blocks) return {};
+    CPH_TRY(codec_upload(ctx, cd, &ix->codec_dev));
+    ix->sorted_codes = std::move(job->spec_sorted);
+    ix->perm = std::move(job->spec_perm);
+    ix->sort_passes = 0;
+    if (rt_blocks) ix->ranktab = std::move(job->spec_rt);
+    job->spec_rt.reset();
+    job->spec_plan_dev.reset();
+    *verdict = SpecVerdict::adopted;
+    return {};
+}
+
 static Status build_encode_sort(cph_ctx* ctx, BuildJob* job) {
     cph_index* ix = job->ix;
     const uint64_t n = ix->nrows;
@@ -1019,6 +1124,7 @@
     jobs[0].ix = ix;
     jobs[0].unique = unique;
     st[0] = build_phase1(ctx, keycols, nkeycols, &jobs[0]);
+    if (st[0].ok()) st[0] = build_spec_launch(ctx, &jobs[0]);
     if (st[0].ok()) build_run(ctx, jobs, st);
     return st[0];
 }
@@ -1080,6 +1186,7 @@
     for (auto& b : ctx->pinned_cache) (void)hipHostFree(b.first);
     for (auto& p : ctx->prof_pending) { (void)hipEventDestroy(p.start); (void)hipEventDestroy(p.stop); }
     for (hipEvent_t e : ctx->prof_free_events) (void)hipEventDestroy(e);
+    for (hipEvent_t e : ctx->spec_events) (void)hipEventDestroy(e);
     hipStream_t own = ctx->own_stream ? ctx->stream : nullptr;
     if (ctx->side_stream) {
         (void)hipStreamSynchronize(ctx->side_stream);
@@ -1130,6 +1237,7 @@
     else if (k == "chain_identity") ctx->chain_identity = value != 0;
     else if (k == "chain_prejoin") ctx->chain_prejoin = value != 0;
     else if (k == "direct_fused_encode") ctx->direct_fused_encode = value != 0;
+    else if (k == "direct_spec") ctx->direct_spec = value != 0;
     else if (k == "direct_ranktab") ctx->direct_ranktab = value != 0;
     else if (k == "hash_load_pct") ctx->hash_load_pct = value < 25 ? 25 : value > 90 ? 90 : (int)value;
     else if (k == "probe_hash_rows") ctx->probe_hash_rows = value == 4 ? 4 : 2;
@@ -1320,7 +1428,7 @@
     if (!specs || !out || nspecs < 1 || nspecs > 64) return fail(ctx, {CPH_ERR_INVALID, "bad cph_index_build_many arguments"});
     std::vector<BuildJob> jobs((size_t)nspecs);
     std::vector<Status> st((size_t)nspecs);
-    if (!host_words_reserve(ctx, (uint32_t)nspecs * (uint32_t)(codec_sample_bytes() / 4 + 16)))
+    if (!host_words_reserve(ctx, (uint32_t)nspecs * (uint32_t)((codec_sample_bytes() + sizeof(SpecPlan)) / 4 + 16)))
         return fail(ctx, {CPH_ERR_INVALID, "cph_index_build_many: the batch needs more report words than the ctx holds"});
     bool two_streams = nspecs >= 2 && ctx->build_side_stream != 0;
     if (two_streams && !ctx->side_stream && hipStreamCreateWithFlags(&ctx->side_stream, hipStreamNonBlocking) != hipSuccess) {
@@ -1357,6 +1465,11 @@
         SideStream on_side(ctx, jobs[i].side);
         if (!jobs[i].ix) st[i] = {CPH_ERR_NOMEM, "out of host memory"};
         else st[i] = build_phase1(ctx, specs[i].keycols, specs[i].nkeycols, &jobs[i]);
+    }
+    for (int i = 0; i < nspecs; i++) {
+        if (!st[i].ok() || !jobs[i].spec_sort) continue;
+        SideStream on_side(ctx, jobs[i].side);
+        st[i] = build_spec_launch(ctx, &jobs[i]);
     }
     build_run(ctx, jobs, st);
     int32_t rc = CPH_OK;
diff --git a/csvplus_amd/csrc/codec_device.hpp b/csvplus_amd/csrc/codec_device.hpp
--- a/csvplus_amd/csrc/codec_device.hpp
+++ b/csvplus_amd/csrc/codec_device.hpp
@@ -394,6 +394,43 @@
 };
 
 void codec_arith_plan(const CodecHost& codec, ArithPlan* ap);
+
+__host__ __device__ inline uint64_t arith_plan_fill(const uint32_t (&first)[8], const uint32_t (&count)[8], uint32_t keylen, ArithPlan* ap) {
+    *ap = ArithPlan{};
+    uint32_t lo[8], rng[8], radix[8];
+    for (uint32_t p = 0; p < 8; p++) {
+        const bool in = p < keylen;
+        lo[p] = in ? first[p] : 0u;
+        rng[p] = in ? count[p] - 1u : 0u;
+        radix[p] = in ? count[p] : 1u;
+    }
+    ap->keylen = keylen;
+    for (int w = 0; w < 2; w++) {
+        for (int i = 0; i < 4; i++) {
+            const int p = 4 * w + i;
+            if ((uint32_t)p < keylen) ap->keep[w] |= 0xFFu << (8 * i);
+            ap->lo[w] |= lo[p] << (8 * i);
+            ap->rngc[w] |= (0x7Fu - rng[p]) << (8 * i);
+        }
+        ap->wa[w] = radix[4 * w + 1] | 1u << 8;
+        ap->wb[w] = radix[4 * w + 3] << 16 | 1u << 24;
+        ap->ma[w] = radix[4 * w + 2] * radix[4 * w + 3];
+    }
+    const uint64_t s0 = (uint64_t)radix[0] * radix[1] * radix[2] * radix[3];
+    const uint64_t s1 = (uint64_t)radix[4] * radix[5] * radix[6] * radix[7];
+    ap->s1 = (uint32_t)s1;
+    ap->mul24 = s0 <= (1ull << 24) && s1 < (1ull << 24) ? 1u : 0u;
+    ap->enabled = 1;
+    return s0 * s1;
+}
+
+struct SpecPlan {
+    ArithPlan ap;
+    uint32_t states;
+    uint32_t rank_blocks;
+    uint32_t ok;
+    uint32_t pad_;
+};
 
 template <int R, class CW>
 __device__ __forceinline__ void encode_rows_arith(const ArithPlan& ap, const uint64_t (&c0)[R], CW (&code)[R], uint32_t* okmask) {
diff --git a/csvplus_amd/csrc/cph_internal.hpp b/csvplus_amd/csrc/cph_internal.hpp
--- a/csvplus_amd/csrc/cph_internal.hpp
+++ b/csvplus_amd/csrc/cph_internal.hpp
@@ -278,6 +278,8 @@
     uint64_t n_split_respec = 0;
     int hash_load_pct = 50;
     int direct_fused_encode = 1;
+    int direct_spec = 1;
+    std::vector<hipEvent_t> spec_events;
     int direct_ranktab = 1;
     int chain_prejoin = 1;
     int split_speculative = 1;
@@ -450,7 +452,9 @@
 Status codec_build(const std::vector<ColStats>& stats, CodecHost* codec);
 bool codec_sample_applies(const cph_ctx* ctx, const DevCol* cols, int32_t ncols, uint64_t n);
 size_t codec_sample_bytes();
-Status codec_sample_launch(cph_ctx* ctx, const DevCol& col, uint64_t n, const void** host_copy);
+struct SpecPlan;
+Status codec_sample_launch(cph_ctx* ctx, const DevCol& col, uint64_t n, const void** host_copy, SpecPlan* spec_dev = nullptr,
+                           const SpecPlan** spec_host = nullptr, bool want_ranktab = false);
 void codec_sample_finish(const DevCol& col, const void* host_copy, std::vector<ColStats>* out);
 bool codec_sample_checked(const CodecHost& codec, const DevCol* cols);
 struct GroupChoice { int t, p0, span; double saved; uint32_t count; uint32_t tab; };
@@ -522,8 +526,11 @@
                                 uint32_t* sorted_out, uint32_t* flag, void* ranktab = nullptr, uint64_t rank_blocks = 0);
 Status direct_sort_windows(cph_ctx* ctx, const uint32_t* codes, uint64_t n, uint64_t states, uint32_t* perm_out, uint32_t* sorted_out,
                            uint32_t* flag, void* ranktab = nullptr, uint64_t rank_blocks = 0);
+struct SpecPlan;
+Status direct_sort_windows_spec(cph_ctx* ctx, const uint64_t* keys, const SpecPlan* plan, uint64_t n, uint32_t* perm_out, uint32_t* sorted_out,
+                                uint32_t* flag, void* ranktab);
 struct WindowSort {
-    Status begin(cph_ctx* ctx, uint64_t n, uint64_t states);
+    Status begin(cph_ctx* ctx, uint64_t n, uint64_t states, const SpecPlan* plan = nullptr);
     Status add(cph_ctx* ctx, const uint32_t* codes, uint64_t row0, uint64_t m, uint32_t* flag, const uint64_t* keys = nullptr, const ArithPlan* ap = nullptr);
     Status finish(cph_ctx* ctx, uint32_t* perm_out, uint32_t* sorted_out, uint32_t* flag, void* ranktab = nullptr, uint64_t rank_blocks = 0);
     ~WindowSort();
@@ -536,6 +543,7 @@
     DevBuf ent1, ent2;
     DevBuf* words = nullptr;
     uint32_t *cur1 = nullptr, *cur2 = nullptr;
+    const SpecPlan* plan = nullptr;
 };
 Status direct_sort_finish_full(cph_ctx* ctx, const uint32_t* slots, uint64_t n, uint32_t* sorted_out, uint32_t* flag);
 Status exclusive_scan_u32(cph_ctx* ctx, uint32_t* data, uint64_t n);
@@ -550,7 +558,7 @@
 Status index_ensure_table(cph_ctx* ctx, const cph_index* ix);
 Status index_ensure_rowtab(cph_ctx* ctx, const cph_index* ix);
 Status index_ensure_ranktab(cph_ctx* ctx, const cph_index* ix);
-inline uint64_t ranktab_blocks(uint64_t table_entries) { return ((table_entries + 31) / 32 + 1) & ~1ull; }
+__host__ __device__ inline uint64_t ranktab_blocks(uint64_t table_entries) { return ((table_entries + 31) / 32 + 1) & ~1ull; }
 Status index_ensure_hash(cph_ctx* ctx, const cph_index* ix);
 bool index_wants_hash(const cph_index* ix);
 struct ProbeOut {
diff --git a/csvplus_amd/csrc/keycodec.hip b/csvplus_amd/csrc/keycodec.hip
--- a/csvplus_amd/csrc/keycodec.hip
+++ b/csvplus_amd/csrc/keycodec.hip
@@ -1071,8 +1071,14 @@
     if (__ballot(missed) && lane_id() == 0) *miss = 1u;
 }
 
+struct SpecPlanOut {
+    SpecPlan* dev;
+    SpecPlan* host;
+    uint64_t table_rows;
+    uint32_t want_ranktab;
+};
 __global__ __launch_bounds__(kSplitThreads) void k_sample_fixed8(DevCol col, uint64_t step, uint64_t n, SplitSample* __restrict__ out,
-                                                                SplitSample* __restrict__ host_out) {
+                                                                SplitSample* __restrict__ host_out, SpecPlanOut spec) {
     __shared__ uint32_t s_mask[8 * 8];
     __shared__ uint32_t s_last;
     const uint32_t W = col.fixed_width;
@@ -1104,11 +1110,49 @@
     if (s_last) {
         uint32_t* src = &out->mask[0][0];
         uint32_t* dst = &host_out->mask[0][0];
-        for (uint32_t i = threadIdx.x; i < (uint32_t)(kSplitMaxValue * 8); i += kSplitThreads) dst[i] = i < 64u ? atomicExch(&src[i], 0u) : 0u;
+        for (uint32_t i = threadIdx.x; i < (uint32_t)(kSplitMaxValue * 8); i += kSplitThreads) {
+            const uint32_t m = i < 64u ? atomicExch(&src[i], 0u) : 0u;
+            dst[i] = m;
+            if (i < 64u) s_mask[i] = m;
+        }
         if (threadIdx.x == 0) {
             host_out->maxlen = W;
             host_out->minlen_inv = ~W;
             atomicExch(ticket, 0u);
+        }
+        if (spec.dev) {
+            __syncthreads();
+            if (threadIdx.x == 0) {
+                uint32_t first[8], count[8];
+                bool ok = W == 8u;
+#pragma unroll
+                for (int q = 0; q < 8; q++) {
+                    uint32_t cnt = 0, fst = 256u, lst = 0;
+#pragma unroll
+                    for (int w = 0; w < 8; w++) {
+                        const uint32_t m = s_mask[q * 8 + w];
+                        if (m) {
+                            cnt += (uint32_t)__popc(m);
+                            if (fst == 256u) fst = 32u * (uint32_t)w + (uint32_t)__ffs((int)m) - 1u;
+                            lst = 32u * (uint32_t)w + 31u - (uint32_t)__clz((int)m);
+                        }
+                    }
+                    ok = ok && cnt >= 1u && lst < 0x80u && lst - fst + 1u == cnt;
+                    first[q] = fst;
+                    count[q] = cnt;
+                }
+                SpecPlan sp{};
+                if (ok) {
+                    const uint64_t states = arith_plan_fill(first, count, 8u, &sp.ap);
+                    ok = states <= (1ull << 31) && states >= spec.table_rows && states <= 2 * spec.table_rows;
+                    sp.states = ok ? (uint32_t)states : 0u;
+                    if (ok && spec.want_ranktab && states != spec.table_rows && states <= (1ull << 30)) sp.rank_blocks = (uint32_t)ranktab_blocks(states);
+                }
+                if (!ok) sp.ap = ArithPlan{};
+                sp.ok = ok ? 1u : 0u;
+                *spec.dev = sp;
+                *spec.host = sp;
+            }
         }
         __threadfence_system();
     }
@@ -1302,19 +1346,30 @@
            !cols[0].segmented() && n >= (1ull << 20);
 }
 size_t codec_sample_bytes() { return sizeof(SplitSample); }
-Status codec_sample_launch(cph_ctx* ctx, const DevCol& col, uint64_t n, const void** host_copy) {
+Status codec_sample_launch(cph_ctx* ctx, const DevCol& col, uint64_t n, const void** host_copy, SpecPlan* spec_dev, const SpecPlan** spec_host,
+                           bool want_ranktab) {
     const uint64_t step = n >> 16;
     const uint64_t nsel = (n + step - 1) / step;
     DevBuf& acc = ctx->self_clean[ctx->stream_slot].sample;
     CPH_TRY(self_clean_block(ctx, &acc, sizeof(SplitSample) + 16));
-    uint32_t* hw = host_word(ctx, (uint32_t)(sizeof(SplitSample) / 4));
+    static_assert(sizeof(SplitSample) % 8 == 0 && sizeof(SpecPlan) % 8 == 0, "report words come in pairs");
+    uint32_t* hw = host_word(ctx, (uint32_t)((sizeof(SplitSample) + (spec_dev ? sizeof(SpecPlan) : 0)) / 4));
     if (!hw) return {CPH_ERR_HIP, "no pinned host memory for the sample's statistics"};
+    if (spec_dev && !(col.fixed_width == 8 && ctx->sample_lean)) return {CPH_ERR_INVALID, "internal: no speculative plan for this sample"};
+    SpecPlanOut spo{};
+    if (spec_dev) {
+        spo.dev = spec_dev;
+        spo.host = reinterpret_cast<SpecPlan*>(hw + sizeof(SplitSample) / 4);
+        spo.table_rows = n;
+        spo.want_ranktab = want_ranktab ? 1u : 0u;
+        *spec_host = spo.host;
+    }
     ProfScope ps(ctx, "k_split_count", 0);
     uint64_t nblk = (nsel + kSplitThreads - 1) / kSplitThreads;
     if (nblk > 1024) nblk = 1024;
     if (col.fixed_width <= 8 && ctx->sample_lean)
         hipLaunchKernelGGL(k_sample_fixed8, dim3((unsigned)nblk), dim3(kSplitThreads), 0, ctx->stream, col, step, nsel, acc.as<SplitSample>(),
-                           reinterpret_cast<SplitSample*>(hw));
+                           reinterpret_cast<SplitSample*>(hw), spo);
     else
         hipLaunchKernelGGL(k_split_count, dim3((unsigned)nblk), dim3(kSplitThreads), 0, ctx->stream, col, step, nsel, acc.as<SplitSample>(),
                            reinterpret_cast<SplitSample*>(hw));
@@ -1642,7 +1697,7 @@
     *ap = ArithPlan{};
     if (cd.ncols != 1 || cd.nwords != 1 || cd.has_groups() || cd.npos < 1 || cd.npos > 8) return;
     if (cd.col_minlen[0] != cd.col_maxlen[0] || cd.word_states[0] > (1ull << 31)) return;
-    uint32_t lo[8] = {0}, rng[8] = {0}, radix[8] = {1, 1, 1, 1, 1, 1, 1, 1};
+    uint32_t lo[8] = {0}, radix[8] = {1, 1, 1, 1, 1, 1, 1, 1};
     for (int p = 0; p < cd.npos; p++) {
         const uint16_t* lut = &cd.lut[(size_t)p * kLutStride];
         if (lut[0] != kLutInvalid) return;
@@ -1653,26 +1708,9 @@
         for (int b = first; b <= last; b++)
             if (lut[1 + b] != (uint16_t)(b - first)) return;
         lo[p] = (uint32_t)first;
-        rng[p] = (uint32_t)(last - first);
         radix[p] = (uint32_t)count;
     }
-    ap->keylen = (uint32_t)cd.npos;
-    for (int w = 0; w < 2; w++) {
-        for (int i = 0; i < 4; i++) {
-            const int p = 4 * w + i;
-            if (p < cd.npos) ap->keep[w] |= 0xFFu << (8 * i);
-            ap->lo[w] |= lo[p] << (8 * i);
-            ap->rngc[w] |= (0x7Fu - rng[p]) << (8 * i);
-        }
-        ap->wa[w] = radix[4 * w + 1] | 1u << 8;
-        ap->wb[w] = radix[4 * w + 3] << 16 | 1u << 24;
-        ap->ma[w] = radix[4 * w + 2] * radix[4 * w + 3];
-    }
-    const uint64_t s0 = (uint64_t)radix[0] * radix[1] * radix[2] * radix[3];
-    const uint64_t s1 = (uint64_t)radix[4] * radix[5] * radix[6] * radix[7];
-    ap->s1 = (uint32_t)s1;
-    ap->mul24 = s0 <= (1ull << 24) && s1 < (1ull << 24) ? 1u : 0u;
-    ap->enabled = 1;
+    (void)arith_plan_fill(lo, radix, (uint32_t)cd.npos, ap);
 }
 
 Status codec_upload(cph_ctx* ctx, const CodecHost& cd, DevBuf* dev) {
diff --git a/csvplus_amd/csrc/window_sort.hip b/csvplus_amd/csrc/window_sort.hip
--- a/csvplus_amd/csrc/window_sort.hip
+++ b/csvplus_amd/csrc/window_sort.hip
@@ -29,6 +29,7 @@
     uint32_t states;
     uint32_t row_base;
     uint32_t* flag;
+    const SpecPlan* plan;
 };
 
 template <int SRC>
@@ -39,8 +40,9 @@
     const uint32_t nbp = (a.nb + (uint32_t)kWpThreads - 1u) & ~((uint32_t)kWpThreads - 1u);
     uint64_t* s_ent = reinterpret_cast<uint64_t*>(smem);
     uint32_t* s_hist = reinterpret_cast<uint32_t*>(s_ent + kWpTile);
-    uint32_t* s_start = s_hist + nbp;
-    uint32_t* s_delta = s_start + nbp;
+    uint32_t* s_start = s_hist;
+    uint32_t* s_delta = s_hist + nbp;
+    if (a.plan && a.plan->ok == 0u) return;
     const uint32_t sb = blockIdx.x / a.tiles_per_src, tl = blockIdx.x % a.tiles_per_src;
     uint64_t cnt = a.n;
     if constexpr (!FROM_CODES) {
@@ -80,11 +82,13 @@
             for (int c = 0; c < 4; c++) row[4 * j + c] = a.row_base + (uint32_t)(t0 + i4 + c);
         }
         const uint32_t have = okm;
-        encode_rows_arith<kWpItems, uint32_t>(a.ap, c0, code, &okm);
+        const ArithPlan ap = a.plan ? a.plan->ap : a.ap;
+        const uint32_t states = a.plan ? a.plan->states : a.states;
+        encode_rows_arith<kWpItems, uint32_t>(ap, c0, code, &okm);
         bool bad = false;
 #pragma unroll
         for (int k = 0; k < kWpItems; k++) {
-            const bool ok = ((okm >> k) & 1u) && code[k] < a.states;
+            const bool ok = ((okm >> k) & 1u) && code[k] < states;
             bad |= ((have >> k) & 1u) && !ok;
             code[k] = ok ? code[k] : kWinEmpty;
         }
@@ -181,8 +185,10 @@
     if (__ballot(over) && lane_id() == 0) *a.flag = 1u;
 }
 
-__global__ __launch_bounds__(1024) void k_win_offsets(const uint32_t* __restrict__ counts, uint32_t nwin, uint32_t* __restrict__ off) {
+__global__ __launch_bounds__(1024) void k_win_offsets(const uint32_t* __restrict__ counts, uint32_t nwin, uint32_t* __restrict__ off,
+                                                      const SpecPlan* __restrict__ plan, uint64_t n) {
     __shared__ uint32_t s_tmp[1024 / kWave + 1];
+    if (plan && (plan->ok == 0u || (uint64_t)plan->states == n)) return;
     uint32_t carry = 0;
     for (uint32_t base = 0; base < nwin; base += 1024) {
         const uint32_t i = base + threadIdx.x;
@@ -199,12 +205,22 @@
                                                             const uint32_t* __restrict__ off, uint64_t n, uint32_t* __restrict__ perm,
                                                             uint32_t* __restrict__ sorted, uint32_t* __restrict__ flag,
                                                             uint32_t* __restrict__ clear_also, uint32_t nclear, uint2* __restrict__ ranktab,
-                                                            uint32_t rank_blocks) {
+                                                            uint32_t rank_blocks, const SpecPlan* __restrict__ plan) {
     extern __shared__ __attribute__((aligned(16))) uint8_t smem[];
     __shared__ uint32_t s_wcount[kPlaceThreads / kWave];
     typedef unsigned int u32x4 __attribute__((ext_vector_type(4)));
     uint32_t* win = reinterpret_cast<uint32_t*>(smem);
     const uint32_t g = blockIdx.x, t = threadIdx.x;
+    if (plan) {
+        if (plan->ok == 0u) return;
+        const uint32_t states = plan->states;
+        rank_blocks = plan->rank_blocks;
+        if ((uint64_t)states == n) off = nullptr;
+        if (((uint64_t)g << kWinBits) >= (uint64_t)states) {
+            if (t == 0 && g < nclear) clear_also[g] = 0u;
+            return;
+        }
+    }
     const uint32_t craw = counts[g], cnt = craw < kWinSlots ? craw : kWinSlots;
     {
         u32x4 e;
@@ -260,9 +276,10 @@
     }
 }
 
-Status WindowSort::begin(cph_ctx* ctx, uint64_t n_, uint64_t states_) {
+Status WindowSort::begin(cph_ctx* ctx, uint64_t n_, uint64_t states_, const SpecPlan* plan_) {
     n = n_;
     states = states_;
+    plan = plan_;
     const uint64_t nwin = (states + kWinSlots - 1) >> kWinBits;
     two = nwin > (uint64_t)kWpMaxBuckets;
     int k2 = 0;
@@ -292,7 +309,7 @@
 
 static size_t win_partition_lds(uint32_t nb) {
     const uint32_t nbp = (nb + (uint32_t)kWpThreads - 1u) & ~((uint32_t)kWpThreads - 1u);
-    return (size_t)kWpTile * 8 + (size_t)nbp * 12;
+    return (size_t)kWpTile * 8 + (size_t)nbp * 8;
 }
 
 Status WindowSort::add(cph_ctx* ctx, const uint32_t* codes, uint64_t row0, uint64_t m, uint32_t* flag, const uint64_t* keys, const ArithPlan* ap) {
@@ -310,6 +327,7 @@
     a.states = (uint32_t)states;
     a.row_base = (uint32_t)row0;
     a.flag = flag;
+    a.plan = plan;
     const size_t lds = win_partition_lds(a.nb);
     if (keys) {
         CPH_TRY(kernel_setup(ctx, reinterpret_cast<const void*>(&k_win_partition<2>), kWpThreads, lds, nullptr));
@@ -325,7 +343,7 @@
 }
 
 Status WindowSort::finish(cph_ctx* ctx, uint32_t* perm_out, uint32_t* sorted_out, uint32_t* flag, void* ranktab, uint64_t rank_blocks) {
-    const bool need_off = states != n;
+    const bool need_off = plan || states != n;
     DevBuf offsets;
     if (need_off) CPH_TRY(offsets.alloc(&ctx->pool, nwin_total * sizeof(uint32_t)));
     uint32_t* off = offsets.as<uint32_t>();
@@ -340,6 +358,7 @@
         a.dst = ent2.as<uint64_t>();
         a.dst_count = cur2;
         a.flag = flag;
+        a.plan = plan;
         const size_t lds = win_partition_lds(a.nb);
         CPH_TRY(kernel_setup(ctx, reinterpret_cast<const void*>(&k_win_partition<0>), kWpThreads, lds, nullptr));
         ProfScope ps(ctx, "k_win_partition", 16.0 * (double)n);
@@ -349,7 +368,7 @@
     uint32_t* counts = two ? cur2 : cur1;
     if (need_off) {
         ProfScope ps(ctx, "k_win_place", 0);
-        hipLaunchKernelGGL(k_win_offsets, dim3(1), dim3(1024), 0, ctx->stream, counts, (uint32_t)nwin_total, off);
+        hipLaunchKernelGGL(k_win_offsets, dim3(1), dim3(1024), 0, ctx->stream, counts, (uint32_t)nwin_total, off, plan, n);
     }
     {
         const size_t lds = (size_t)kWinSlots * sizeof(uint32_t);
@@ -357,7 +376,7 @@
         ProfScope ps(ctx, "k_win_place", 16.0 * (double)n);
         hipLaunchKernelGGL(k_win_place, dim3((unsigned)nwin_total), dim3(kPlaceThreads), lds, ctx->stream, two ? ent2.as<uint64_t>() : ent1.as<uint64_t>(),
                            counts, need_off ? off : nullptr, n, perm_out, sorted_out, flag, cur1, two ? (uint32_t)nb1 : 0u,
-                           static_cast<uint2*>(ranktab), (uint32_t)rank_blocks);
+                           static_cast<uint2*>(ranktab), (uint32_t)rank_blocks, plan);
     }
     CPH_HIP_TRY(hipGetLastError());
     finished = true;
@@ -380,6 +399,15 @@
     CPH_TRY(ws.add(ctx, nullptr, 0, n, flag, keys, &ap));
     return ws.finish(ctx, perm_out, sorted_out, flag, ranktab, rank_blocks);
 }
+Status direct_sort_windows_spec(cph_ctx* ctx, const uint64_t* keys, const SpecPlan* plan, uint64_t n, uint32_t* perm_out, uint32_t* sorted_out,
+                                uint32_t* flag, void* ranktab) {
+    if (n == 0) return {};
+    WindowSort ws;
+    CPH_TRY(ws.begin(ctx, n, 2 * n, plan));
+    ArithPlan none{};
+    CPH_TRY(ws.add(ctx, nullptr, 0, n, flag, keys, &none));
+    return ws.finish(ctx, perm_out, sorted_out, flag, ranktab, 0);
+}
 
 }
 
```

Result: no change. 133.4 billion rows/s (median of 2 runs) (+0.7%).
